# fdaPDE/fdaPDE-core

Hardware: AMD Instinct MI355X
Metric: DOF/s assemble+solve, 3D P1 Laplacian; SpMV achieved HBM GB/s vs peak (higher is better)
Workload: dtype f64

## Files before the change

fdapde-core_amd/capi.py:

```python
from __future__ import annotations

import ctypes as C
import os

import numpy as np

_HERE = os.path.dirname(os.path.abspath(__file__))
LIB_PATH = os.environ.get("FDAPDE_HIP_LIB") or os.path.join(_HERE, "lib", "libfdapde_hip.so")

OK, EINVAL, ENOMEM, ENODEVICE, EHIP, ENOTINIT, ENOCONV, EUNSUPPORTED, ERCCL = range(9)
LAPLACIAN, DIFFUSION, ADVECTION, REACTION, DT = range(5)
SOLVER_AUTO, SOLVER_CG, SOLVER_BICGSTAB, SOLVER_CG_SR, SOLVER_CG_FUSED, SOLVER_GMRES, SOLVER_DENSE, SOLVER_PMG, SOLVER_AMG = range(9)
ASSEMBLY_ROWS, ASSEMBLY_ATOMIC, ASSEMBLY_COLOURED, ASSEMBLY_PARTITIONED, ASSEMBLY_WAVE = range(5)
MAT_STIFF, MAT_MASS = 0, 1


class Term(C.Structure):
    _fields_ = [("kind", C.c_int32), ("space_varying", C.c_int32), ("coef", C.c_double), ("cst", C.c_double * 9),
                ("data", C.POINTER(C.c_double))]


class Options(C.Structure):
    _fields_ = [("method", C.c_int32), ("maxit", C.c_int32), ("rtol", C.c_double), ("assembly", C.c_int32),
                ("check_every", C.c_int32), ("time_spmv", C.c_int32)]


class Info(C.Structure):
    _fields_ = [("iters", C.c_int32), ("converged", C.c_int32), ("relres", C.c_double), ("t_assemble_ms", C.c_double),
                ("t_solve_ms", C.c_double), ("t_setup_ms", C.c_double), ("spmv_avg_ms", C.c_double), ("spmv_timed", C.c_int32),
                ("method_used", C.c_int32), ("persistent", C.c_int32), ("gather_avg_ms", C.c_double), ("update_avg_ms", C.c_double),
                ("spmv_mean_ms", C.c_double), ("launch_ms", C.c_double)]


SYMBOLS = [
    "fdapde_abi_version", "fdapde_device_count", "fdapde_ctx_create", "fdapde_ctx_destroy", "fdapde_last_error",
    "fdapde_status_string", "fdapde_mesh_upload", "fdapde_dofs_build", "fdapde_dofs_get", "fdapde_dofs_set_boundary", "fdapde_sizes",
    "fdapde_pattern_get", "fdapde_quadrature_nodes", "fdapde_set_operator", "fdapde_set_forcing", "fdapde_set_dirichlet",
    "fdapde_init", "fdapde_assemble_operator", "fdapde_solver_prepare", "fdapde_solve", "fdapde_matrix_values", "fdapde_lump", "fdapde_force", "fdapde_solution",
    "fdapde_info_get", "fdapde_spmv", "fdapde_bench_spmv", "fdapde_tune", "fdapde_stream", "fdapde_synchronize",
    "fdapde_comm_unique_id", "fdapde_comm_init", "fdapde_halo_setup", "fdapde_solve_parabolic",
    "fdapde_lin_compute", "fdapde_lin_solve", "fdapde_eval_pointwise", "fdapde_cell_integrals", "fdapde_comm_init_callback", "fdapde_comm_set_exchange_callback", "fdapde_halo_setup_peers",
    "fdapde_solver_layout", "fdapde_topology_build", "fdapde_topology_get", "fdapde_comm_allreduce", "fdapde_comm_library", "fdapde_solver_layout_kind", "fdapde_solver_layout_partition", "fdapde_rowdist_setup", "fdapde_ctx_clone", "fdapde_comm_count",
    "fdapde_ctx_create_multi", "fdapde_ctx_devices", "fdapde_partition_build", "fdapde_partition_sizes", "fdapde_partition_get", "fdapde_partition_whole",
    "fdapde_partition_peers",
]
PARTITION_ROWDIST, PARTITION_ELEMENTS = 0, 1

_lib = None


def load() -> C.CDLL:
    global _lib
    if _lib is None:
        if not os.path.exists(LIB_PATH):
            raise ImportError(f"{LIB_PATH} is missing: build it with __graft_entry__.build() or `make -C fdapde-core_amd/csrc`. "
                              "There is no CPU fallback.")
        lib = C.CDLL(LIB_PATH)
        lib.fdapde_last_error.restype = C.c_char_p
        lib.fdapde_status_string.restype = C.c_char_p
        lib.fdapde_stream.restype = C.c_void_p
        lib.fdapde_comm_library.restype = C.c_char_p
        lib.fdapde_ctx_destroy.restype = None
        _lib = lib
    return _lib


class FdapdeError(RuntimeError):
    def __init__(self, status, msg):
        super().__init__(f"[status {status}] {msg}")
        self.status = status


def _dp(a):
    return a.ctypes.data_as(C.POINTER(C.c_double))


def _ip(a):
    return a.ctypes.data_as(C.POINTER(C.c_int32))


def _bp(a):
    return a.ctypes.data_as(C.POINTER(C.c_uint8))


class Operator:

    def __init__(self, terms=None):
        self.terms = list(terms or [])

    def __neg__(self):
        return Operator([(k, -c, cst, d) for (k, c, cst, d) in self.terms])

    def __add__(self, o):
        return Operator(self.terms + o.terms)

    def __sub__(self, o):
        return Operator(self.terms + (-o).terms)

    def __rmul__(self, s):
        return Operator([(k, float(s) * c, cst, d) for (k, c, cst, d) in self.terms])

    @property
    def is_symmetric(self):
        return all(k != ADVECTION for (k, _, _, _) in self.terms)

    def c_terms(self):
        arr = (Term * len(self.terms))()
        keep = []
        for t, (k, c, cst, d) in zip(arr, self.terms):
            t.kind, t.coef, t.space_varying = k, c, 0 if d is None else 1
            if cst is not None:
                for i, v in enumerate(np.asarray(cst, dtype=float).reshape(-1)):
                    t.cst[i] = v
            if d is not None:
                dd = np.ascontiguousarray(d, dtype=float)
                keep.append(dd)
                t.data = _dp(dd)
        return arr, keep


def laplacian():
    return Operator([(LAPLACIAN, 1.0, None, None)])


def diffusion(K):
# ... 249 lines not shown
        flat = np.ascontiguousarray(locs.T).reshape(-1)
        cells = np.zeros(nl, dtype=np.int32)
        vals = np.zeros((nl, s["n_basis"]))
        self._check(self.lib.fdapde_eval_pointwise(self._ctx, C.c_int64(nl), _dp(flat), _ip(cells), _dp(vals)))
        dofs, _, _ = self.dofs_get()
        ok = cells >= 0
        rows = np.repeat(np.nonzero(ok)[0], s["n_basis"])
        cols = dofs[cells[ok]].reshape(-1)
        psi = sp.csr_matrix((vals[ok].reshape(-1), (rows, cols)), shape=(nl, s["n_dofs"]))
        return psi, np.ones(nl), cells

    def eval_areal(self, incidence):
        import scipy.sparse as sp

        inc = sp.csr_matrix(np.asarray(incidence) == 1, dtype=float)
        s = self.sizes()
        meas = np.zeros(self.n_cells)
        pint = np.zeros((self.n_cells, s["n_basis"]))
        self._check(self.lib.fdapde_cell_integrals(self._ctx, _dp(meas), _dp(pint)))
        dofs, _, _ = self.dofs_get()
        D = inc @ meas
        nb = s["n_basis"]
        cellmat = sp.csr_matrix((pint.reshape(-1), (np.repeat(np.arange(self.n_cells), nb), dofs.reshape(-1))),
                                shape=(self.n_cells, s["n_dofs"]))
        psi = sp.diags(1.0 / D) @ (inc @ cellmat)
        return psi.tocsr(), D

    def info(self):
        info = Info()
        self._check(self.lib.fdapde_info_get(self._ctx, C.byref(info)))
        return info

    def matrix_values(self, which=MAT_STIFF):
        out = np.zeros(self.sizes()["nnz"])
        self._check(self.lib.fdapde_matrix_values(self._ctx, which, _dp(out)))
        return out

    def lump(self, which=MAT_MASS):
        out = np.zeros(self.sizes()["n_dofs"])
        self._check(self.lib.fdapde_lump(self._ctx, which, _dp(out)))
        return out

    def force(self, ncols=None):
        have = getattr(self, "_force_cols", 1)
        if ncols is None:
            ncols = have
        if ncols < have:
            raise ValueError(f"force(): the context holds {have} forcing columns, a buffer for {ncols} was asked for")
        out = np.zeros(self.sizes()["n_dofs"] * ncols)
        self._check(self.lib.fdapde_force(self._ctx, _dp(out)))
        return out

    def solution(self):
        out = np.zeros(self.sizes()["n_dofs"])
        self._check(self.lib.fdapde_solution(self._ctx, _dp(out)))
        return out

    def spmv(self, which, x):
        x = np.ascontiguousarray(x, dtype=float)
        y = np.zeros_like(x)
        self._check(self.lib.fdapde_spmv(self._ctx, which, _dp(x), _dp(y)))
        return y

    def bench_spmv(self, reps=50):
        ms, by = C.c_double(), C.c_double()
        self._check(self.lib.fdapde_bench_spmv(self._ctx, reps, C.byref(ms), C.byref(by)))
        return ms.value, by.value

    def solver_layout(self, with_dirichlet=True):
        ni, nz, by = C.c_int64(), C.c_int64(), C.c_double()
        self._check(self.lib.fdapde_solver_layout(self._ctx, 1 if with_dirichlet else 0, C.byref(ni), C.byref(nz), C.byref(by)))
        return ni.value, nz.value, by.value

    def solver_layout_kind(self, with_dirichlet=True):
        k, sy, g, r = C.c_int32(), C.c_int32(), C.c_int32(), C.c_int32()
        self._check(self.lib.fdapde_solver_layout_kind(self._ctx, 1 if with_dirichlet else 0, C.byref(k), C.byref(sy), C.byref(g), C.byref(r)))
        return dict(kind=k.value, sym=sy.value, workgroups=g.value, rows_per_thread=r.value)

    def solver_layout_partition(self, with_dirichlet=True):
        p = C.c_int32()
        self._check(self.lib.fdapde_solver_layout_partition(self._ctx, 1 if with_dirichlet else 0, C.byref(p)))
        return p.value

    @staticmethod
    def comm_unique_id() -> bytes:
        buf = C.create_string_buffer(128)
        rc = load().fdapde_comm_unique_id(buf)
        if rc != OK:
            raise FdapdeError(rc, "fdapde_comm_unique_id failed (RCCL not loadable?)")
        return buf.raw

    def comm_init(self, world, rank, unique_id: bytes):
        self._check(self.lib.fdapde_comm_init(self._ctx, int(world), int(rank), C.c_char_p(unique_id)))

    def rowdist_setup(self, dof_key, dof_owner):
        k = np.ascontiguousarray(dof_key, dtype=np.int64)
        o = np.ascontiguousarray(dof_owner, dtype=np.int32)
        self._check(self.lib.fdapde_rowdist_setup(self._ctx, k.ctypes.data_as(C.POINTER(C.c_int64)), _ip(o)))

    def comm_allreduce(self, values, op="sum"):
        a = np.ascontiguousarray(np.asarray(values, dtype=float)).copy()
        self._check(self.lib.fdapde_comm_allreduce(self._ctx, _dp(a), int(a.size), 0 if op == "sum" else 1))
        return a

    def comm_count(self):
        n = C.c_int32(0)
        self._check(self.lib.fdapde_comm_count(self._ctx, C.byref(n)))
        return int(n.value)

    @staticmethod
    def comm_library():
        return (load().fdapde_comm_library() or b"").decode()

    def comm_init_callback(self, world, rank, allreduce):
        proto = C.CFUNCTYPE(C.c_int, C.c_void_p, C.POINTER(C.c_double), C.c_int64)

        def _cb(user, ptr, count):
            try:
                allreduce(np.ctypeslib.as_array(ptr, shape=(count,)))
                return 0
            except Exception:
                return 1

        self._ar_cb = proto(_cb)
        self._check(self.lib.fdapde_comm_init_callback(self._ctx, int(world), int(rank), self._ar_cb, None))

    def halo_setup(self, n_if_global, local_dof, if_index, owned):
        local_dof = np.ascontiguousarray(local_dof, dtype=np.int32)
        if_index = np.ascontiguousarray(if_index, dtype=np.int32)
        owned = np.ascontiguousarray(owned, dtype=np.uint8)
        self._check(self.lib.fdapde_halo_setup(self._ctx, C.c_int64(int(n_if_global)), C.c_int64(local_dof.size), _ip(local_dof),
                                               _ip(if_index), _bp(owned)))

    def comm_set_exchange_callback(self, exchange):
        proto = C.CFUNCTYPE(C.c_int, C.c_void_p, C.c_int32, C.POINTER(C.c_int32), C.POINTER(C.c_int64), C.POINTER(C.c_double), C.POINTER(C.c_double))

        def _cb(user, n_peers, ranks, offs, send, recv):
            try:
                off = np.ctypeslib.as_array(offs, shape=(n_peers + 1,))
                n = int(off[-1])
                exchange(np.ctypeslib.as_array(ranks, shape=(n_peers,)), off, np.ctypeslib.as_array(send, shape=(n,)),
                         np.ctypeslib.as_array(recv, shape=(n,)))
                return 0
            except Exception:
                return 1

        self._xchg_cb = proto(_cb)
        self._check(self.lib.fdapde_comm_set_exchange_callback(self._ctx, self._xchg_cb, None))

    def halo_setup_peers(self, peer_rank, peer_off, peer_dof, owned):
        peer_rank = np.ascontiguousarray(peer_rank, dtype=np.int32)
        peer_off = np.ascontiguousarray(peer_off, dtype=np.int64)
        peer_dof = np.ascontiguousarray(peer_dof, dtype=np.int32)
        owned = np.ascontiguousarray(owned, dtype=np.uint8)
        self._check(self.lib.fdapde_halo_setup_peers(self._ctx, C.c_int32(peer_rank.size), _ip(peer_rank),
                                                     peer_off.ctypes.data_as(C.POINTER(C.c_int64)), _ip(peer_dof), _bp(owned)))

    def tune(self, key, value):
        self._check(self.lib.fdapde_tune(self._ctx, key.encode(), int(value)))

    def stream(self):
        return self.lib.fdapde_stream(self._ctx)

    def synchronize(self):
        self._check(self.lib.fdapde_synchronize(self._ctx))
```

fdapde-core_amd/csrc/capi.hip:

```cpp
#include <algorithm>
#include <chrono>
#include <cmath>
#include <cstdio>
#include <cstdlib>
#include <cstring>
#include <new>

#include <dlfcn.h>
#include <hip/hip_ext.h>
#include <rccl/rccl.h>

#include "context.h"
#include "engine.h"

using namespace fdapde_engine;

extern "C" {

int fdapde_abi_version(void) { return FDAPDE_ABI_VERSION; }

int fdapde_device_count(void) {
    int n = 0;
    if (hipGetDeviceCount(&n) != hipSuccess) return 0;
    return n;
// ... 1 lines not shown

const char* fdapde_status_string(int s) {
    switch (s) {
    case FDAPDE_OK: return "ok";
    case FDAPDE_EINVAL: return "invalid argument";
    case FDAPDE_ENOMEM: return "out of memory";
    case FDAPDE_ENODEVICE: return "no HIP device";
    case FDAPDE_EHIP: return "HIP runtime error";
    case FDAPDE_ENOTINIT: return "solver must be initialized first!";
    case FDAPDE_ENOCONV: return "Krylov solve did not converge";
    case FDAPDE_EUNSUPPORTED: return "unsupported configuration";
    case FDAPDE_ERCCL: return "RCCL error";
    }
    return "unknown status";
}

int fdapde_ctx_create(int device, fdapde_ctx** out) {
    if (!out) return FDAPDE_EINVAL;
    *out = nullptr;
    fdapde_ctx* c = new (std::nothrow) fdapde_ctx();
    if (!c) return FDAPDE_ENOMEM;
    if (device >= 0) {
        int n = 0;
        if (hipGetDeviceCount(&n) != hipSuccess || device >= n) {
            delete c;
            return FDAPDE_ENODEVICE;
        }
        if (hipSetDevice(device) != hipSuccess || hipStreamCreateWithFlags(&c->stream, hipStreamNonBlocking) != hipSuccess ||
            hipEventCreate(&c->ev0) != hipSuccess || hipEventCreate(&c->ev1) != hipSuccess ||
            hipEventCreate(&c->ev_p0) != hipSuccess || hipEventCreate(&c->ev_p1) != hipSuccess ||
            hipHostMalloc(reinterpret_cast<void**>(&c->h_ctl), 8 * sizeof(int32_t)) != hipSuccess ||
            hipHostMalloc(reinterpret_cast<void**>(&c->h_sc), 16 * sizeof(double)) != hipSuccess) {
            delete c;
            return FDAPDE_EHIP;
        }
        c->device = device, c->has_device = true;
        preload_assembly(), preload_solve(), preload_dist(), preload_persist();
        preload_setup_async(device);
        if (hipDeviceGetAttribute(&c->n_cu, hipDeviceAttributeMultiprocessorCount, device) != hipSuccess) c->n_cu = 0;
    }
    *out = c;
    return FDAPDE_OK;
}

void fdapde_ctx_destroy(fdapde_ctx* c) {
    if (!c) return;
    if (c->group) fdapde_engine::g_destroy(c);
    fdapde_engine::pmg_release(c);
    fdapde_engine::amg_release(c);
    if (c->has_device) {
        (void)hipSetDevice(c->device);
        fdapde_engine::partition_free(c);
        (void)hipSetDevice(c->device);
        (void)hipStreamSynchronize(c->stream);
        drop_graph(c);
        for (DBuf<int32_t>* b : {&c->cverts, &c->cdofs, &c->adj, &c->rowptr, &c->colidx, &c->diag, &c->slot_i2e, &c->dof_i2e,
                                 &c->dof_e2i, &c->cell_i2e, &c->rb_row, &c->colour_cells, &c->ctl, &c->rowptr_e, &c->colidx_e, &c->dofs_e})
            b->release();
        for (DBuf<double>* b : {&c->vcoords, &c->vals[0], &c->vals[1], &c->force, &c->fq, &c->g, &c->sval, &c->scale, &c->gt,
                                &c->x, &c->r, &c->p, &c->y, &c->s, &c->t, &c->r0, &c->u, &c->part_a, &c->part_b, &c->sc,
                                &c->tmp_e, &c->tmp_i, &c->tmp_v, &c->lin_rhs, &c->cols_b, &c->cols_r, &c->cols_x, &c->cols_sc, &c->cols_part})
            b->release();
        c->cols_ctl.release(), c->eval_grid.release(), c->eval_locs.release(), c->eval_vals.release(), c->eval_out.release();
        for (auto& b : c->coef) b.release();
        c->slotw.release(), c->sl_off.release(), c->lane_row.release(), c->fq_blk.release(), c->bnd.release(), c->tables.release(), c->reftab.release(), c->reftab_sym.release(), c->lin_sq.release();
        c->bc_off.release(), c->bn_off.release(), c->bc_cell.release(), c->bn_node.release(), c->bc_vert.release();
        c->halo_dof.release(), c->halo_pos.release(), c->owned.release(), c->hbuf.release(), c->sbuf.release();
        c->halo_inv.release(), c->if_slot.release();
        c->peer_send_dof.release(), c->peer_src_off.release(), c->peer_src.release(), c->peer_sendbuf.release(), c->peer_recvbuf.release();
        c->xd.remote[0].release(), c->xd.remote[1].release(), c->xd.slots.release(), c->xd.slot_ptr.release();
        release_rowdist(c);
        if (c->comm) (void)g_rccl.CommDestroy(c->comm);
        c->mesh_nodes.release(), c->mesh_cells.release(), c->mesh_nbnd.release();
        c->gm_V.release(), c->gm_b.release(), c->gm_s.release(), c->gm_part.release();
        c->lin_dense.X.release(), c->step_dense.X.release(), c->solve_dense.X.release(), c->dn_b.release(), c->dn_x.release(), c->dn_r.release(), c->dn_cnt.release();
        c->lin_mat.release(), c->stiff_stat.release(), c->ar_dev.release(), c->persist_stats.release(), c->persist_x.release(), c->persist_xs.release(), c->coords_e.release();
        dev_topology_release(&c->topo);
        c->part_cells.release(), c->part_off.release(), c->part_slots.release(), c->wave_slots.release(), c->part_shared.release();
        for (auto& bk : c->bk)
            bk.slot_dof.release(), bk.sl_off.release(), bk.ell_src.release(), bk.imp_off.release(), bk.imp_dof.release(), bk.drop_dof.release(), bk.ell_off.release(),
              bk.ell_code.release(), bk.ell_val.release();
        for (auto& ps : c->ps)
            ps.slot_dof.release(), ps.sl_off.release(), ps.ell_src.release(), ps.exp_off.release(), ps.imp_off.release(),
              ps.imp_pos.release(), ps.ell_off.release(), ps.ell_code.release(), ps.exp_slot.release(), ps.ell_val.release(), ps.board.release(), ps.board_cols.release(), ps.amax.release(), ps.wg_late.release(), ps.ell_col.release();
        for (int v = 0; v < 2; ++v)
            c->sp_rowptr[v].release(), c->sp_colidx[v].release(), c->sp_map[v].release(), c->sp_tbase[v].release(), c->sp_col16[v].release(),
              c->sp_vrow[v].release();
        if (c->h_io) (void)hipHostFree(c->h_io);
        if (c->h_ctl) (void)hipHostFree(c->h_ctl);
        if (c->h_sc) (void)hipHostFree(c->h_sc);
        (void)hipEventDestroy(c->ev0), (void)hipEventDestroy(c->ev1), (void)hipEventDestroy(c->ev_p0), (void)hipEventDestroy(c->ev_p1);
        for (hipEvent_t e : c->ev_spmv) (void)hipEventDestroy(e);
        (void)hipStreamDestroy(c->stream);
    }
    delete c->lin_state;
    delete c;
}

int fdapde_ctx_clone(const fdapde_ctx* src, fdapde_ctx** out) {
    if (!src || !out) return FDAPDE_EINVAL;
    *out = nullptr;
    if (src->group) return fdapde_engine::g_clone(src, out);
    fdapde_ctx* c = nullptr;
    if (int rc = fdapde_ctx_create(src->has_device ? src->device : -1, &c)) return rc;
    const int rc = fdapde_engine::e_ctx_clone(src, c);
    if (rc != FDAPDE_OK) {
        const_cast<fdapde_ctx*>(src)->err = "fdapde_ctx_clone: " + c->err;
        fdapde_ctx_destroy(c);
        return rc;
    }
    *out = c;
    return FDAPDE_OK;
}

const char* fdapde_last_error(const fdapde_ctx* c) { return c ? c->err.c_str() : "null context"; }

int fdapde_mesh_upload(fdapde_ctx* c, int M, int N, int64_t n_nodes, const double* nodes, int64_t n_cells,
                       const int32_t* cells, const uint8_t* bnd) {
    if (!c) return FDAPDE_EINVAL;
    if (c->group && M == 2 && N == 3)
        return fail(c, FDAPDE_EUNSUPPORTED, "fdapde_mesh_upload: a surface mesh (Triangulation<2,3>) takes a one-GPU context; the multi-device partitioner "
                                            "and its ranks are built for planar and volume meshes");
    if (c->group && M == 1)
        return fail(c, FDAPDE_EUNSUPPORTED, "fdapde_mesh_upload: a 1-D mesh (interval or linear network, Triangulation<1,N>) takes a one-GPU context; the "
                                            "multi-device partitioner and its ranks are built for planar and volume meshes");
    c->space_ready = c->dev_ready = c->colour_ready = c->fq_blk_ready = c->fq_bc_ready = c->stiff_stat_valid = false;
    c->assembled[0] = c->assembled[1] = c->force_ready = c->solved = c->dirichlet_applied = false;
    c->op.clear(), c->coef_of_op = false, c->fq_i.clear(), c->fq_cols = 0, c->g_i.clear(), c->have_g = false;
    if (c->topo_ready) dev_topology_release(&c->topo), c->topo_ready = false;
    c->mesh_on_dev = false;
    if (int rc = host_set_mesh(c->hs, M, N, n_nodes, nodes, n_cells, cells, bnd, c->err)) return rc;
    if (c->has_device) {
        const HostSpace& hs = c->hs;
        if (hipSetDevice(c->device) != hipSuccess || c->mesh_nodes.upload(hs.nodes.data(), hs.nodes.size(), c->stream) != hipSuccess ||
            c->mesh_cells.upload(hs.cells.data(), hs.cells.size(), c->stream) != hipSuccess ||
            c->mesh_nbnd.upload(hs.node_bnd.data(), hs.node_bnd.size(), c->stream) != hipSuccess || hipStreamSynchronize(c->stream) != hipSuccess) {
            c->mesh_nodes.release(), c->mesh_cells.release(), c->mesh_nbnd.release();
            c->err = "fdapde_mesh_upload: copying the mesh to the device failed";
            return FDAPDE_EHIP;
        }
        c->mesh_on_dev = true;
    }
    fdapde_engine::partition_free(c);
    if (c->group) fdapde_engine::g_mesh_changed(c);
    return FDAPDE_OK;
}

int fdapde_sizes(const fdapde_ctx* c, int64_t* n_dofs, int64_t* nnz, int32_t* n_basis, int32_t* n_quadrature, int64_t* n_edges) {
    if (!c || !c->space_ready) return FDAPDE_ENOTINIT;
    if (n_dofs) *n_dofs = c->hs.n_dofs;
    if (nnz) *nnz = c->hs.nnz;
    if (n_basis) *n_basis = c->hs.nb;
    if (n_quadrature) *n_quadrature = c->hs.nq;
    if (n_edges) *n_edges = c->hs.n_edges;
    return FDAPDE_OK;
}

int fdapde_dofs_build(fdapde_ctx* c, int order, int64_t* n_dofs) {
    if (!c) return FDAPDE_EINVAL;
    if (c->group) return fdapde_engine::g_dofs_build(c, order, n_dofs);
    return fdapde_engine::e_dofs_build(c, order, n_dofs);
}
int fdapde_topology_build(fdapde_ctx* c, int64_t* n_facets, int64_t* n_edges) {
    if (!c) return FDAPDE_EINVAL;
    return fdapde_engine::e_topology_build(c, n_facets, n_edges);
}
int fdapde_topology_get(fdapde_ctx* c, int32_t* neighbors, int32_t* cell_facets, int32_t* facet_nodes, int32_t* facet_cells, uint8_t* facet_boundary, int32_t* edge_nodes, uint8_t* edge_boundary, int32_t* face_edges) {
    if (!c) return FDAPDE_EINVAL;
    return fdapde_engine::e_topology_get(c, neighbors, cell_facets, facet_nodes, facet_cells, facet_boundary, edge_nodes, edge_boundary, face_edges);
}
int fdapde_dofs_set_boundary(fdapde_ctx* c, const uint8_t* bnd) {
    if (!c) return FDAPDE_EINVAL;
    if (c->group) return fdapde_engine::g_dofs_set_boundary(c, bnd);
    return fdapde_engine::e_dofs_set_boundary(c, bnd);
}
int fdapde_dofs_get(const fdapde_ctx* c, int32_t* dofs, uint8_t* bnd, double* coords) {
    if (!c) return FDAPDE_EINVAL;
    return fdapde_engine::e_dofs_get(c, dofs, bnd, coords);
}
int fdapde_pattern_get(const fdapde_ctx* c, int32_t* rowptr, int32_t* colidx) {
    if (!c) return FDAPDE_EINVAL;
    return fdapde_engine::e_pattern_get(c, rowptr, colidx);
}
int fdapde_quadrature_nodes(fdapde_ctx* c, double* out) {
    if (!c) return FDAPDE_EINVAL;
    return fdapde_engine::e_quadrature_nodes(c, out);
}
int fdapde_set_operator(fdapde_ctx* c, int32_t n_terms, const fdapde_term* terms) {
    if (!c) return FDAPDE_EINVAL;
    if (c->group) return fdapde_engine::g_set_operator(c, n_terms, terms);
    return fdapde_engine::e_set_operator(c, n_terms, terms);
}
int fdapde_set_forcing(fdapde_ctx* c, const double* f_q, int32_t n_cols) {
    if (!c) return FDAPDE_EINVAL;
    if (c->group) return fdapde_engine::g_set_forcing(c, f_q, n_cols);
    return fdapde_engine::e_set_forcing(c, f_q, n_cols);
}
int fdapde_set_dirichlet(fdapde_ctx* c, const double* g) {
    if (!c) return FDAPDE_EINVAL;
    if (c->group) return fdapde_engine::g_set_dirichlet(c, g);
    return fdapde_engine::e_set_dirichlet(c, g);
}
int fdapde_assemble_operator(fdapde_ctx* c, int32_t which, int32_t n_terms, const fdapde_term* terms, int32_t assembly) {
    if (!c) return FDAPDE_EINVAL;
    if (c->group) return fdapde_engine::g_assemble_operator(c, which, n_terms, terms, assembly);
    return fdapde_engine::e_assemble_operator(c, which, n_terms, terms, assembly);
}
int fdapde_init(fdapde_ctx* c, const fdapde_options* opt) {
    if (!c) return FDAPDE_EINVAL;
    if (c->group) return fdapde_engine::g_init(c, opt);
    return fdapde_engine::e_init(c, opt);
}
int fdapde_eval_pointwise(fdapde_ctx* c, int64_t n_locs, const double* locs_colmajor, int32_t* cell_ids, double* values) {
    if (!c) return FDAPDE_EINVAL;
    return fdapde_engine::e_eval_pointwise(c, n_locs, locs_colmajor, cell_ids, values);
}
int fdapde_cell_integrals(fdapde_ctx* c, double* measure, double* psi_int) {
    if (!c) return FDAPDE_EINVAL;
    return fdapde_engine::e_cell_integrals(c, measure, psi_int);
}
int fdapde_solver_prepare(fdapde_ctx* c, int32_t with_dirichlet) {
    if (!c) return FDAPDE_EINVAL;
    if (c->group) return fdapde_engine::g_solver_prepare(c, with_dirichlet);
    return fdapde_engine::e_solver_prepare(c, with_dirichlet);
}
int fdapde_solver_layout(fdapde_ctx* c, int32_t with_dirichlet, int64_t* n_interior, int64_t* nnz_interior, double* streamed_bytes) {
    if (!c) return FDAPDE_EINVAL;
    if (c->group) return fdapde_engine::g_layout_kind(c, with_dirichlet, nullptr, nullptr, nullptr, nullptr);
    return fdapde_engine::e_solver_layout(c, with_dirichlet, n_interior, nnz_interior, streamed_bytes);
}
int fdapde_solver_layout_kind(fdapde_ctx* c, int32_t with_dirichlet, int32_t* kind, int32_t* symmetric_storage, int32_t* workgroups, int32_t* rows_per_thread) {
    if (!c) return FDAPDE_EINVAL;
    if (c->group) return fdapde_engine::g_layout_kind(c, with_dirichlet, kind, symmetric_storage, workgroups, rows_per_thread);
    return fdapde_engine::e_solver_layout_kind(c, with_dirichlet, kind, symmetric_storage, workgroups, rows_per_thread);
}
int fdapde_solver_layout_partition(fdapde_ctx* c, int32_t with_dirichlet, int32_t* partition) {
    int32_t kind = 0;
    if (int rc = fdapde_solver_layout_kind(c, with_dirichlet, &kind, nullptr, nullptr, nullptr)) return rc;
    const fdapde_ctx::Persist& ps = c->ps[with_dirichlet ? 1 : 0];
    if (partition) *partition = (kind == 2 || kind == 3) && ps.ok ? (ps.meta.bisect ? 1 : 0) : -1;
    return FDAPDE_OK;
}
int fdapde_solve(fdapde_ctx* c, const fdapde_options* opt, fdapde_info* info) {
    if (!c) return FDAPDE_EINVAL;
    if (c->group && opt && opt->method == FDAPDE_SOLVER_AMG) return fdapde_engine::fail(c, FDAPDE_EUNSUPPORTED, "FDAPDE_SOLVER_AMG takes one-GPU contexts, not a multi-device context");
    if (c->group) return fdapde_engine::g_solve(c, opt, info);
    return fdapde_engine::e_solve(c, opt, info);
}
int fdapde_solve_parabolic(fdapde_ctx* c, const fdapde_options* opt, int32_t n_times, double delta_t, const double* initial_condition, const double* dirichlet, double* solution, fdapde_info* info) {
    if (!c) return FDAPDE_EINVAL;
    if (c->group && opt && opt->method == FDAPDE_SOLVER_AMG) return fdapde_engine::fail(c, FDAPDE_EUNSUPPORTED, "FDAPDE_SOLVER_AMG takes one-GPU contexts, not a multi-device context");
    if (c->group) return fdapde_engine::g_solve_parabolic(c, opt, n_times, delta_t, initial_condition, dirichlet, solution, info);
    return fdapde_engine::e_solve_parabolic(c, opt, n_times, delta_t, initial_condition, dirichlet, solution, info);
}
int fdapde_lin_compute(fdapde_ctx* c, int32_t which, const double* values, int32_t symmetric) {
    if (!c) return FDAPDE_EINVAL;
    if (c->group) return fdapde_engine::g_lin_compute(c, which, values, symmetric);
    return fdapde_engine::e_lin_compute(c, which, values, symmetric);
}
int fdapde_lin_solve(fdapde_ctx* c, const fdapde_options* opt, const double* b, int32_t n_rhs, double* x, fdapde_info* info) {
    if (!c) return FDAPDE_EINVAL;
    if (c->group && opt && opt->method == FDAPDE_SOLVER_AMG) return fdapde_engine::fail(c, FDAPDE_EUNSUPPORTED, "FDAPDE_SOLVER_AMG takes one-GPU contexts, not a multi-device context");
    if (c->group) return fdapde_engine::g_lin_solve(c, opt, b, n_rhs, x, info);
    return fdapde_engine::e_lin_solve(c, opt, b, n_rhs, x, info);
}
int fdapde_matrix_values(fdapde_ctx* c, int32_t which, double* values) {
    if (!c) return FDAPDE_EINVAL;
    if (c->group) return fdapde_engine::g_matrix_values(c, which, values);
    return fdapde_engine::e_matrix_values(c, which, values);
}
int fdapde_lump(fdapde_ctx* c, int32_t which, double* diag) {
    if (!c) return FDAPDE_EINVAL;
    if (c->group) return fdapde_engine::g_lump(c, which, diag);
    return fdapde_engine::e_lump(c, which, diag);
}
int fdapde_force(fdapde_ctx* c, double* force) {
    if (!c) return FDAPDE_EINVAL;
    if (c->group) return fdapde_engine::g_force(c, force);
    return fdapde_engine::e_force(c, force);
}
int fdapde_solution(fdapde_ctx* c, double* solution) {
    if (!c) return FDAPDE_EINVAL;
    if (c->group) return fdapde_engine::g_solution(c, solution);
    return fdapde_engine::e_solution(c, solution);
}
int fdapde_spmv(fdapde_ctx* c, int32_t which, const double* x, double* y) {
    if (!c) return FDAPDE_EINVAL;
    if (c->group) return fdapde_engine::g_spmv(c, which, x, y);
    return fdapde_engine::e_spmv(c, which, x, y);
}
int fdapde_bench_spmv(fdapde_ctx* c, int32_t reps, double* avg_ms, double* algorithmic_bytes) {
    if (!c) return FDAPDE_EINVAL;
    if (c->group) return fail(c, FDAPDE_EUNSUPPORTED, "fdapde_bench_spmv: a multi-device context wires its own ranks");
    return fdapde_engine::e_bench_spmv(c, reps, avg_ms, algorithmic_bytes);
}
int fdapde_comm_unique_id(void* out128) {
    return fdapde_engine::e_comm_unique_id(out128);
}
int fdapde_comm_init(fdapde_ctx* c, int32_t world, int32_t rank, const void* unique_id128) {
    if (!c) return FDAPDE_EINVAL;
    if (c->group) return fail(c, FDAPDE_EUNSUPPORTED, "fdapde_comm_init: a multi-device context wires its own ranks");
    return fdapde_engine::e_comm_init(c, world, rank, unique_id128);
}
int fdapde_comm_allreduce(fdapde_ctx* c, double* host_inout, int32_t n, int32_t op) {
    if (!c) return FDAPDE_EINVAL;
    if (c->group) return fail(c, FDAPDE_EUNSUPPORTED, "fdapde_comm_allreduce: a multi-device context wires its own ranks");
    return fdapde_engine::e_comm_allreduce(c, host_inout, n, op);
}
int fdapde_comm_count(fdapde_ctx* c, int32_t* ranks) {
    if (!c) return FDAPDE_EINVAL;
    return fdapde_engine::e_comm_count(c, ranks);
}
int fdapde_comm_init_callback(fdapde_ctx* c, int32_t world, int32_t rank, fdapde_allreduce_fn fn, void* user) {
    if (!c) return FDAPDE_EINVAL;
    if (c->group) return fail(c, FDAPDE_EUNSUPPORTED, "fdapde_comm_init_callback: a multi-device context wires its own ranks");
    return fdapde_engine::e_comm_init_callback(c, world, rank, fn, user);
}
// ... 61 lines not shown
    if (c->group) return fdapde_engine::g_tune(c, key, value);
    const std::string k(key);
    drop_graph(c);
    if (k == "spmv_variant" && value >= 0 && value <= 2) c->spmv_variant = value;
    else if (k == "spmv_team" && (value == 2 || value == 4 || value == 8 || value == 16 || value == 32 || value == 64)) {
        if (value != c->spmv_team) c->sp_built[0] = c->sp_built[1] = false, c->sp_cur = -1, c->solved = false, c->scaled_owner = fdapde_ctx::kScaledNone;
        c->spmv_team = value;
    }
    else if (k == "spmv_unroll" && value >= 1 && value <= 8) c->spmv_unroll = value;
    else if (k == "spmv_ablate") c->spmv_ablate = value;
    else if (k == "spmv_c16" && (value == 0 || value == 1)) c->spmv_c16 = value;
    else if (k == "spmv_deep" && (value == 0 || value == 1)) c->spmv_deep = value;
    else if (k == "cgf_split" && (value == 0 || value == 1)) c->cgf_split = value;
    else if (k == "cgf_v" && (value == 1 || value == 2 || value == 4 || value == 8)) c->cgf_v = value;
    else if (k == "use_graph" && (value == 0 || value == 1)) c->use_graph = value;
    else if (k == "cgf_band" && (value == 0 || value == 1)) c->cgf_band = value;
    else if (k == "cgf_nt" && value >= 0 && value <= 15) c->cgf_nt = value;
    else if (k == "cgf_lazy" && (value == 0 || value == 1)) c->cgf_lazy = value;
    else if (k == "multi_rhs" && (value == 0 || value == 1)) c->multi_rhs = value;
    else if (k == "asm_fq_block" && (value == 0 || value == 1)) c->asm_fq_block = value;
    else if (k == "asm_fuse_mass" && value >= 0 && value <= 3) c->asm_fuse_mass = value;
    else if (k == "asm_items" && (value == 0 || value == 1)) c->asm_items = value;
    else if (k == "asm_items_fuse" && (value == 0 || value == 1)) c->asm_items_fuse = value;
    else if (k == "bicg_restart" && (value == 0 || value == 1)) c->bicg_restart = value;
    else if (k == "bicg_shadow" && value >= 0 && value <= 2) c->bicg_shadow = value;
    else if (k == "gmres_m" && value >= 2 && value <= 200) c->gmres_m = value;
    else if (k == "persist_exp_lds" && (value == 0 || value == 1)) {
        c->persist_exp_lds = value;
        c->ps[0].tried = c->ps[0].ok = c->ps[1].tried = c->ps[1].ok = false, c->scaled_owner = fdapde_ctx::kScaledNone;
        fdapde_engine::drop_graph(c);
    }
    else if (k == "dense_rows" && value >= 0 && value <= 8192) c->dense_rows = value, c->lin_dense.ready = false, c->lin_dense.failed = false;
    else if (k == "dense_after" && value >= 0) c->dense_after = value;
    else if (k == "dense_block" && (value == 0 || value == 1)) c->dense_block = value;
    else if (k == "dense_direct" && (value == 0 || value == 1)) c->dense_direct = value;
    else if (k == "dense_fold" && (value == 0 || value == 1)) c->dense_fold = value;
    else if (k == "dense_multi" && (value == 0 || value == 1)) c->dense_multi = value;
    else if (k == "pmg_inner_tol_exp" && value >= 1 && value <= 12) c->pmg_inner_rtol = std::pow(10.0, -(double)value);
    else if (k == "pmg_inner_maxit" && value >= 1) c->pmg_inner_maxit = value;
    else if (k == "pmg_auto" && (value == 0 || value == 1)) c->pmg_auto = value;
    else if (k == "pmg_blocked" && (value == 0 || value == 1)) c->pmg_blocked = value;
    else if (k == "pmg_smooth" && (value == 0 || value == 1)) c->pmg_smooth = value;
    else if (k == "pmg_setup_check" && (value == 0 || value == 1)) c->pmg_setup_check = value;
    else if (k == "amg_coarse_rows" && value >= 1 && value <= 8192) c->amg_coarse_rows = value;
    else if (k == "amg_setup_check" && (value == 0 || value == 1)) c->amg_setup_check = value;
    else if (k == "pmg_restart" && value >= 2 && value <= 50) c->pmg_restart = (int)value;
    else if (k == "pmg_outer" && (value == 0 || value == 1)) c->pmg_outer = value;
    else if (k == "pmg_auto_rows" && value >= 0) c->pmg_auto_rows = value;
    else if (k == "pmg_auto_first_rows" && value >= 0) c->pmg_auto_first_rows = value;
    else if (k == "dense_bulk" && (value == 0 || value == 1)) c->dense_bulk = value;
    else if (k == "dense_hostb" && (value == 0 || value == 1)) c->dense_hostb = value;
    else if (k == "small_rows" && value >= 0) c->small_rows = value;
    else if (k == "small_front_rows" && value >= 0) c->small_front_rows = value;
    else if (k == "auto_gmres" && (value == 0 || value == 1)) c->auto_gmres = value;
    else if (k == "asm_split_varying" && (value == 0 || value == 1)) c->asm_split_varying = value;
    else if (k == "asm_row_stat" && (value == 0 || value == 1)) c->asm_row_stat = value, c->stiff_stat_valid = false;
    else if (k == "asm_fq_bc" && (value == 0 || value == 1)) c->asm_fq_bc = value, c->fq_bc_ready = c->fq_bc_ready && value;
    else if (k == "persist" && (value == 0 || value == 1)) c->persist = value, c->persist_broken = false;
    else if (k == "persist_time" && (value == 0 || value == 1)) c->persist_time = value;
    else if (k == "persist_coop" && (value == 0 || value == 1)) c->persist_coop = value;
    else if (k == "persist_bicg" && (value == 0 || value == 1)) c->persist_bicg = value;
    else if (k == "persist_fill_fused" && (value == 0 || value == 1)) c->persist_fill_fused = value;
    else if (k == "persist_prefetch" && (value == 0 || value == 1)) c->persist_prefetch = value;
    else if (k == "persist_cols" && (value == 0 || value == 1)) c->persist_cols = value;
    else if (k == "persist_direct" && (value == 0 || value == 1)) c->persist_direct = value;
    else if (k == "persist_wide_gj" && (value == 4 || value == 6 || value == 12)) {
        c->persist_wide_gj = value;
        for (auto& ps : c->ps) ps.attr_set = nullptr;
    }
    else if ((k == "persist_wide" && (value == 0 || value == 1)) || (k == "persist_max_wg" && value >= 0)) {
        if (k == "persist_wide") c->persist_wide = value;
        else c->persist_max_wg = value;
        for (auto& ps : c->ps) ps.tried = ps.ok = ps.filled = false;
    }
    else if (k == "persist_direct_spin_us" && value >= 0 && value <= 1000000) c->persist_direct_spin_us = value;
    else if (k == "persist_single_rows" && value >= 0 && value <= 8192) {
        c->persist_single_rows = value;
        for (auto& ps : c->ps) ps.tried = ps.ok = ps.filled = false;
    }
    else if (k == "persist_partition" && value >= 0 && value <= 2) {
        c->persist_partition = value;
        for (auto& ps : c->ps) ps.tried = ps.ok = ps.filled = false;
    }
    else if (k == "persist_late" && (value == 0 || value == 1)) {
        c->persist_late = value;
        for (auto& ps : c->ps) ps.tried = ps.ok = ps.filled = false;
    }
    else if (k == "rowdist_max_wg" && value >= 0) {
        c->rd.max_wg = value;
        for (auto& L : c->rd.lay) L.tried = L.ok = false;
    } else if (k == "rowdist_share" && value >= 1) {
        c->rd.max_wg = std::max(1, c->n_cu / value);
        for (auto& L : c->rd.lay) L.tried = L.ok = false;
    } else if (k == "rowdist_timeout_first_ms" && value >= 1) c->rd.timeout_first_ms = value;
    else if (k == "rowdist_flat_gather" && value >= -1 && value <= 1) c->rd.flat_gather = value;
    else if (k == "persist_timeout_us" && value >= 100 && value <= 10000000) c->persist_timeout_us = value;
    else if (k == "persist_debug_stall" && value >= 0) c->persist_debug_stall = value;
    else if (k == "persist_retry" && value == 1) c->persist_broken = false, c->persist_retry_in = 0, c->persist_backoff = 8;
    else if (k == "blocked" && value >= 0 && value <= 2) c->blocked = value;
    else if (k == "persist_gather_waves" && (value == 1 || value == 4)) c->persist_gather_waves = value;
    else if (k == "persist_poll_sleep" && value >= 0 && value <= 3) c->persist_poll_sleep = value;
    else if (k == "persist_balance" && (value == 0 || value == 1)) {
        c->persist_balance = value;
        for (auto& ps : c->ps) ps.tried = ps.ok = ps.filled = false;
    } else if (k == "persist_sym" && value >= 0 && value <= 2) {
        c->persist_sym = value;
        for (auto& ps : c->ps) ps.tried = ps.ok = ps.filled = false;
    }
    else if (k == "spmv_ntv" && value >= -1 && value <= 1) c->spmv_ntv = value;
    else if (k == "spmv_bpx" && value >= 1 && value <= 1024) {
        c->spmv_grid = 8 * value;
        HIPCHK(c, hipSetDevice(c->device));
        HIPCHK(c, hipStreamSynchronize(c->stream));
        HIPCHK(c, c->part_a.alloc(2 * (size_t)c->spmv_grid));
    } else return fail(c, FDAPDE_EINVAL, "unknown tuning key or value out of range");
    return FDAPDE_OK;
}

void* fdapde_stream(fdapde_ctx* c) { return c ? (void*)c->stream : nullptr; }

int fdapde_synchronize(fdapde_ctx* c) {
    if (!c) return FDAPDE_EINVAL;
    if (int rc = need_device(c)) return rc;
    if (c->group)
        if (int rc = fdapde_engine::g_synchronize(c)) return rc;
    HIPCHK(c, hipSetDevice(c->device));
    HIPCHK(c, hipStreamSynchronize(c->stream));
    HIPCHK(c, hipDeviceSynchronize());
    return FDAPDE_OK;
}

}
```

fdapde-core_amd/csrc/context.h:

```cpp
#ifndef FDAPDE_CONTEXT_H
#define FDAPDE_CONTEXT_H

#include <cstdint>
#include <memory>
#include <functional>
#include <string>
#include <vector>

#include <dlfcn.h>
#include <hip/hip_ext.h>
#include <hip/hip_runtime.h>
#include <rccl/rccl.h>

#include "../../include/fdapde_hip.h"
#include "dev_persist.h"
#include "dev_setup.h"
#include "dev_topology.h"
#include "internal.h"

namespace fdapde_engine {
struct Group;
struct AmgHierarchy;
}
namespace fdapde_hip {
// ... 85 lines not shown
        GetUniqueId = reinterpret_cast<decltype(GetUniqueId)>(dlsym(handle, "ncclGetUniqueId"));
        CommInitRank = reinterpret_cast<decltype(CommInitRank)>(dlsym(handle, "ncclCommInitRank"));
        CommDestroy = reinterpret_cast<decltype(CommDestroy)>(dlsym(handle, "ncclCommDestroy"));
        CommCount = reinterpret_cast<decltype(CommCount)>(dlsym(handle, "ncclCommCount"));
        AllReduce = reinterpret_cast<decltype(AllReduce)>(dlsym(handle, "ncclAllReduce"));
        GetErrorString = reinterpret_cast<decltype(GetErrorString)>(dlsym(handle, "ncclGetErrorString"));
        Send = reinterpret_cast<decltype(Send)>(dlsym(handle, "ncclSend"));
        Recv = reinterpret_cast<decltype(Recv)>(dlsym(handle, "ncclRecv"));
        GroupStart = reinterpret_cast<decltype(GroupStart)>(dlsym(handle, "ncclGroupStart"));
        GroupEnd = reinterpret_cast<decltype(GroupEnd)>(dlsym(handle, "ncclGroupEnd"));
        if (!GetUniqueId || !CommInitRank || !CommDestroy || !AllReduce || !GetErrorString || !Send || !Recv || !GroupStart || !GroupEnd) {
            err = "librccl lacks a required symbol";
            return false;
        }
        return true;
    }
};
inline RcclApi g_rccl;

struct HostTerm {
    fdapde_term t;
    std::vector<double> data_i;
    std::shared_ptr<DBuf<double>> data_dev;
    bool field_nonsym = false;
};

}
using namespace fdapde_detail;

constexpr int64_t kNtValsRows = 2000000;
constexpr int kTimeStride = 8, kTimePhase = 3;

struct GraphKey {
    const void* sval;
    const void* rowptr;
    int64_t n;
    double tol2;
    int chunk, v, grid, team, ablate, c16, deep, unroll, sp_cur, bk_cur, bk_G;
    const void* bk_val;
};

struct SolveState {
    bool dist = false, diag_positive = true;
    bool symmetric = true;
    bool rowdist = false;
    const uint8_t* owned = nullptr;
    int use_bnd = 0;
    bool diag_deferred = false;
    mutable bool front_pending = false;
    const double* front_A = nullptr;
};
struct SolveStateHolder {
    SolveState ss;
};

struct fdapde_ctx {
    int device = -1;
    bool has_device = false;
    hipStream_t stream = nullptr;
    hipEvent_t ev0 = nullptr, ev1 = nullptr, ev_p0 = nullptr, ev_p1 = nullptr;
    std::vector<hipEvent_t> ev_spmv;
    std::string err;
    HostSpace hs;
    BasisTables tb;
    bool space_ready = false, dev_ready = false, colour_ready = false;
    bool assembled[2] = {false, false};
    bool force_ready = false, solved = false, dirichlet_applied = false;
    std::vector<HostTerm> op;
    bool op_symmetric = true;
    std::vector<double> fq_i;
    int fq_cols = 0;
    std::vector<double> g_i;
    bool have_g = false, g_zero = false;
    fdapde_info info{};
    DBuf<int32_t> cverts, cdofs, adj, rowptr, colidx, diag, slot_i2e, dof_i2e, dof_e2i, cell_i2e, rb_row, colour_cells;
    DBuf<int32_t> rowptr_e, colidx_e;
    DBuf<int32_t> dofs_e;
    DBuf<double> coords_e;
    DBuf<double> mesh_nodes;
    DBuf<int32_t> mesh_cells;
    DBuf<uint8_t> mesh_nbnd;
    bool mesh_on_dev = false;
    DBuf<double> gm_V, gm_b, gm_s, gm_part;
    int persist_exp_lds = 1;
    int gmres_m = 50;
    int auto_gmres = 1;
    bool dev_built = false;
    DBuf<uint32_t> slotw;
    DBuf<int64_t> bc_off, bn_off;
    DBuf<int32_t> bc_cell, bn_node;
    DBuf<uint16_t> bc_vert;
    DBuf<int64_t> sl_off;
    DBuf<int32_t> lane_row;
    DBuf<double> stiff_stat;
    bool stiff_stat_valid = false, asm_all_in_lds = false;
    int asm_row_stat = 1;
    DBuf<double> fq_blk;
    bool fq_blk_ready = false;
    DBuf<double> fq_bc;
    bool fq_bc_ready = false;
    bool cg_broke_down = false;
    int bicg_shadow = 0;
    int bicg_restart = 1;
    int asm_split_varying = 1;
    int asm_items = 1;
    int32_t asm_max_visits = -1;
    int asm_fuse_mass = 1;
    int asm_items_fuse = 1;
    int asm_fq_bc = 1;
    int asm_fq_block = 0;
    DBuf<double> vcoords, vals[2], force, fq, g, sval, scale, gt, x, r, p, y, s, t, r0, u, part_a, part_b, sc, tmp_e,
      tmp_i, tmp_v, restart_u, lin_rhs;
    DBuf<uint8_t> bnd;
    DBuf<DevTables> tables;
    DBuf<DevRefTensors> reftab;
    DBuf<DevRefTensorsSym> reftab_sym;
    DBuf<int32_t> ctl;
    DBuf<double> coef[kMaxTerms];
    bool coef_of_op = false;
    double* h_io = nullptr;
    size_t h_io_cap = 0;
    int persist_direct = 1;
    int persist_direct_spin_us = 2000;
    int32_t* h_ctl = nullptr;
    double* h_sc = nullptr;
    int spmv_grid = 0, rb_per_band = 0, vec_grid = 0, n_rb = 0, cg_grid = 0;
    int spmv_variant = 2;
    int spmv_team = 16, spmv_unroll = 4, spmv_ablate = 0;
    int lds_limit = 96 * 1024;
    DBuf<int32_t> sp_rowptr[2], sp_colidx[2], sp_map[2], sp_tbase[2], sp_vrow[2];
    int64_t sp_nv[2] = {0, 0};
    int sval_layout = -2;
    DBuf<uint16_t> sp_col16[2];
    int64_t sp_wide[2] = {0, 0};
    int spmv_ntv = -1;
    int sp_team = 0;
    int spmv_c16 = 1;
    int use_graph = 0;
    hipGraphExec_t cg_graph_exec = nullptr;
    GraphKey cg_graph_key{};
    int cgf_lazy = 1;
    int cgf_nt = 7;
    int cgf_band = 1;
    int cgf_split = 0;
    int cgf_v = 8;
    int spmv_deep = 0;
    int64_t sp_nnz[2] = {0, 0};
    bool sp_built[2] = {false, false};
    int sp_cur = -1;
    bool sval_stale = false;
    const double* sval_A = nullptr;
    int persist_fill_fused = 0;
    enum { kScaledNone = 0, kScaledSolve, kScaledParabolic, kScaledLin, kScaledPmg };
    int scaled_owner = kScaledNone;
    ncclComm_t comm = nullptr;
    fdapde_allreduce_fn ar_fn = nullptr;
    void* ar_user = nullptr;
    std::vector<double> ar_host;
    DBuf<double> ar_dev;
    int world = 1, rank = 0;
    bool halo_ready = false;
    int64_t n_if = 0, n_loc_if = 0;
    DBuf<int32_t> halo_dof, halo_pos;
    DBuf<int32_t> halo_inv, if_slot;
    DBuf<uint8_t> owned;
    DBuf<double> hbuf, sbuf;
    bool peer_mode = false;
    fdapde_exchange_fn xchg_fn = nullptr;
    void* xchg_user = nullptr;
    std::vector<int32_t> peer_rank;
    std::vector<int64_t> peer_off;
    DBuf<int32_t> peer_send_dof;
    DBuf<int32_t> peer_src_off, peer_src;
    DBuf<double> peer_sendbuf, peer_recvbuf;
    std::vector<double> xchg_send_h, xchg_recv_h;
    struct PeerDirect {
        bool on = false;
        int (*arrive)(void*) = nullptr;
        void* user = nullptr;
        int parity = 0, ar_parity = 0;
        int64_t n_send = 0;
        DBuf<const double*> remote[2];
        DBuf<double> slots;
        DBuf<const double*> slot_ptr;
    } xd;
    static constexpr int kSlotDoubles = 64;
    DBuf<double> lin_mat;
    bool lin_ready = false, lin_symmetric = false;
    DBuf<double> lin_sq;
    bool lin_sq_ready = false;
    int multi_rhs = 1;
    SolveStateHolder* lin_state = nullptr;
    int n_cu = 0;
    int persist = 1;
    int persist_time = 1;
    int persist_balance = 1;
    int persist_sym = 2;
    int persist_gather_waves = 4, persist_poll_sleep = 2;
    bool persist_broken = false;
    int persist_retry_in = 0, persist_backoff = 8;
    struct Persist {
        bool tried = false, ok = false;
        PersistLayout meta;
        int32_t lds_cap = 0, imp_cap = 0;
        size_t lds_bytes = 0;
        DBuf<int32_t> slot_dof, sl_off, ell_src, exp_off, imp_off, imp_pos;
        DBuf<int32_t> ell_col;
        bool stream = false;
        bool exp_lds = false;
        DBuf<int64_t> ell_off;
        DBuf<uint16_t> ell_code, exp_slot;
        DBuf<double> ell_val;
        DBuf<unsigned long long> amax;
        DBuf<uint8_t> wg_late;
        DBuf<unsigned long long> board;
        DBuf<unsigned long long> board_cols;
        int per_cu = 0;
        bool filled = false;
        uint32_t epoch_next = 0;
        const void* attr_set = nullptr;
        bool built_plain = false;
    } ps[2];
    struct RowDist {
        bool ready = false;
        std::vector<int32_t> owner_i;
        std::vector<int64_t> key_i;
        DBuf<uint8_t> owned;
        int max_wg = 0;
        int flat_gather = -1;
        int timeout_first_ms = 2000;
        struct Layout {
            bool tried = false, ok = false;
            Persist ps;
            int32_t n_ghost = 0, G_tot = 0, g_base = 0;
            DBuf<int32_t> rexp_off, rexp_peer, rexp_pos;
            DBuf<uint16_t> rexp_slot;
            DBuf<uint8_t> wg_late;
            DBuf<unsigned long long> rboard;
            DBuf<unsigned long long*> peer_pboard, peer_dboard;
            std::vector<void*> ipc_opened;
            std::vector<int32_t> x_rank;
            std::vector<int64_t> x_soff, x_roff;
            DBuf<int32_t> x_send_dof, x_recv_dof;
            DBuf<double> x_sendbuf, x_recvbuf;
        } lay[2];
    } rd;
    DBuf<double> persist_stats;
    DBuf<double> persist_x;
    DBuf<double> persist_xs;
    int persist_wide_gj = 12;
    int persist_wide = 1;
    int persist_max_wg = 0;
    double persist_launch_ms = 0;
    int persist_host_below = 32768;
    int persist_cols = 1;
    DBuf<double> cols_b, cols_r, cols_x, cols_sc, cols_part;
    DBuf<int32_t> cols_ctl;
    struct EvalGrid {
        bool ready = false;
        DBuf<int32_t> ptr, cells, dims;
        DBuf<double> lo, invh;
        void release() { ptr.release(), cells.release(), dims.release(), lo.release(), invh.release(), ready = false; }
    } eval_grid;
    DBuf<double> eval_locs, eval_vals;
    DBuf<int32_t> eval_out;
    std::function<int()> persist_tail;
    int h_ctl_seen = 4;
    bool ev1_at_end = false;
    int64_t small_rows = 8192;
    int64_t small_front_rows = 2048;
    bool front_used = false;
    bool tail_in_launch = false;
    bool defer_end_sync = false;
    int persist_single_rows = 2048;
    int persist_prefetch = 1;
    int persist_partition = 2;
    int persist_late = 0;
    int persist_plain = 0;
    int persist_bicg = 1;
    int persist_coop = 0;
    int persist_timeout_us = 5000;
    int persist_debug_stall = 0;
    struct Blocked {
        bool tried = false, ok = false, filled = false;
        PersistLayout meta;
        int32_t imp_cap = 0;
        size_t lds_bytes = 0;
        DBuf<int32_t> slot_dof, sl_off, ell_src, imp_off, imp_dof, drop_dof;
        DBuf<int64_t> ell_off;
        DBuf<uint16_t> ell_code;
        DBuf<double> ell_val;
    } bk[2];
    int bk_cur = -1;
    int blocked = 1;
    DevTopology topo;
    bool topo_ready = false;
// ... 78 lines not shown
```

fdapde-core_amd/csrc/eng_solve.hip:

```cpp
#include <algorithm>
#include <chrono>
#include <cmath>
#include <cstdio>
#include <cstdlib>
#include <cstring>
#include <new>

#include <dlfcn.h>
#include <hip/hip_ext.h>
#include <rccl/rccl.h>

#include "context.h"
#include "engine.h"
#include "kernels.h"

namespace fdapde_engine {

constexpr int64_t kBlockedShortRowsAbove = 3200000;

void drop_graph(fdapde_ctx* c) {
    if (c->cg_graph_exec) (void)hipGraphExecDestroy(c->cg_graph_exec);
    c->cg_graph_exec = nullptr;
}

// ... 794 lines not shown
    int rc = solve_run(c, ss, A, f_dev, g_dev, u0_dev, method, rtol, maxit, check_every, n_timed);
    int total = c->info.iters;
    const bool may_restart = method == FDAPDE_SOLVER_BICGSTAB || method == FDAPDE_SOLVER_AUTO;
    for (int k = 0; k < kBicgRestarts && may_restart && rc == FDAPDE_ENOCONV && c->h_ctl[2] != 0 && c->info.method_used == FDAPDE_SOLVER_BICGSTAB &&
                    total < maxit && std::isfinite(c->info.relres) && c->info.relres < 1e3 && c->bicg_restart;
         ++k) {
        if (ss.rowdist)
            if (int rc2 = rowdist_import_ghosts(c, ss.use_bnd ? 1 : 0, c->u.p)) return rc2;
        HIPCHK(c, c->restart_u.alloc((size_t)n));
        HIPCHK(c, hipMemcpyAsync(c->restart_u.p, c->u.p, sizeof(double) * (size_t)n, hipMemcpyDeviceToDevice, c->stream));
        rc = solve_run(c, ss, A, f_dev, g_dev, c->restart_u.p, FDAPDE_SOLVER_BICGSTAB, rtol, maxit - total, check_every, 0);
        total += c->info.iters;
    }
    c->info.iters = total;
    if (gmres_budget >= 0 && (gmres_budget > 0 || maxit - total > 0) && rc == FDAPDE_ENOCONV && c->info.method_used == FDAPDE_SOLVER_BICGSTAB && !ss.dist && !ss.rowdist &&
        dense_eligible(c)) {
        bool solved = false;
        if (int rc2 = dense_direct(c, A, ss.use_bnd, f_dev, g_dev, &solved)) return rc2;
        if (solved) {
            c->info.method_used = FDAPDE_SOLVER_DENSE, c->info.converged = 1, c->info.relres = c->solve_dense.check, c->info.persistent = 0;
            c->h_ctl[0] = 1, c->h_ctl[2] = 0;
            c->err.clear();
            if (c->ev1_at_end) HIPCHK(c, hipEventRecord(c->ev1, c->stream));
            return FDAPDE_OK;
        }
    }
    const int gm_maxit = gmres_budget > 0 ? gmres_budget : maxit - total;
    if (gmres_budget >= 0 && gm_maxit > 0 && c->auto_gmres && rc == FDAPDE_ENOCONV && c->info.method_used == FDAPDE_SOLVER_BICGSTAB && !ss.dist && !ss.rowdist) {
        const bool warm = std::isfinite(c->info.relres) && c->info.relres < 1.0;
        if (warm) {
            HIPCHK(c, c->restart_u.alloc((size_t)n));
            HIPCHK(c, hipMemcpyAsync(c->restart_u.p, c->u.p, sizeof(double) * (size_t)n, hipMemcpyDeviceToDevice, c->stream));
        }
        rc = solve_run(c, ss, A, f_dev, g_dev, warm ? c->restart_u.p : u0_dev, FDAPDE_SOLVER_GMRES, rtol, gm_maxit, check_every, 0);
        c->info.iters += total;
    }
    return rc;
}

int e_solver_prepare(fdapde_ctx* c, int32_t with_dirichlet) {
    if (!c) return FDAPDE_EINVAL;
    if (int rc = need_device(c)) return rc;
    if (!c->dev_ready) return fail(c, FDAPDE_ENOTINIT, "call fdapde_dofs_build first");
    HIPCHK(c, hipSetDevice(c->device));
    if (c->spmv_variant != 2) return FDAPDE_OK;
    const int v = with_dirichlet ? 1 : 0;
    if (c->persist && !c->persist_broken && c->comm == nullptr && c->ar_fn == nullptr && (c->op_symmetric || c->persist_bicg)) {
        c->persist_plain = c->op_symmetric ? 0 : 1;
        if (int rc = build_persist(c, v)) return rc;
        if (c->ps[v].ok && (c->op_symmetric || (!c->ps[v].meta.sym && c->ps[v].meta.R <= 8))) return FDAPDE_OK;
    }
    if (c->blocked && c->comm == nullptr && c->ar_fn == nullptr &&
        ((double)c->hs.nnz >= 20.0 * (double)c->hs.n_dofs || c->blocked == 2 || c->hs.n_dofs > kBlockedShortRowsAbove)) {
        if (int rc = build_blocked(c, v)) return rc;
        if (c->bk[v].ok) return FDAPDE_OK;
    }
    return build_solver_pattern(c, v);
}

int e_solver_layout(fdapde_ctx* c, int32_t with_dirichlet, int64_t* n_interior, int64_t* nnz_interior, double* streamed_bytes) {
    if (!c) return FDAPDE_EINVAL;
    if (int rc = need_device(c)) return rc;
    if (!c->dev_ready) return fail(c, FDAPDE_ENOTINIT, "call fdapde_dofs_build first");
    HIPCHK(c, hipSetDevice(c->device));
    const int v = with_dirichlet ? 1 : 0;
    const bool persist = c->persist && !c->persist_broken && c->ps[v].tried && c->ps[v].ok;
    const bool blocked = !persist && c->bk[v].tried && c->bk[v].ok;
    if (c->spmv_variant == 2 && !persist && !blocked)
        if (int rc = build_solver_pattern(c, v)) return rc;
    if (int rc = ensure_host(c, kHostPattern)) return rc;
    const HostSpace& hs = c->hs;
    int64_t ni = 0, nz = 0;
    for (int64_t i = 0; i < hs.n_dofs; ++i) {
        if (v && hs.dof_bnd_i[(size_t)i]) continue;
        ++ni;
        for (int32_t k = hs.rowptr_i[(size_t)i]; k < hs.rowptr_i[(size_t)i + 1]; ++k)
            if (!(v && hs.dof_bnd_i[(size_t)hs.colidx_i[(size_t)k]])) ++nz;
    }
    if (n_interior) *n_interior = ni;
    if (nnz_interior) *nnz_interior = nz;
    if (streamed_bytes) {
        if (persist) {
            *streamed_bytes = 10.0 * (double)c->ps[v].meta.n_entries + 32.0 * (double)c->ps[v].meta.n_board +
                              (c->ps[v].meta.R > kPersistRmax ? 16.0 * (double)c->ps[v].meta.n_int : 0.0);
        } else if (blocked) {
            *streamed_bytes = 10.0 * (double)c->bk[v].meta.n_entries + 8.0 * (double)(c->bk[v].meta.n_int + c->bk[v].meta.n_imp) + 8.0 * (double)c->bk[v].meta.n_int;
        } else if (c->spmv_variant == 2 && c->sp_built[v]) {
            const int64_t n_csr = c->sp_nv[v] > 0 ? c->sp_nv[v] : hs.n_dofs;
            *streamed_bytes = 10.0 * (double)c->sp_nnz[v] + 4.0 * (double)(n_csr + 1) + 16.0 * (double)((n_csr + kCodeRows - 1) / kCodeRows) +
                              (c->sp_nv[v] > 0 ? 8.0 * (double)n_csr : 0.0) + 16.0 * (double)hs.n_dofs +
                              4.0 * (double)c->sp_wide[v] * kCodeRows * ((double)c->sp_nnz[v] / (double)(n_csr > 0 ? n_csr : 1));
        } else
            *streamed_bytes = 12.0 * (double)hs.nnz + 4.0 * (double)(hs.n_dofs + 1) + 16.0 * (double)hs.n_dofs;
    }
    return FDAPDE_OK;
}

int e_solver_layout_kind(fdapde_ctx* c, int32_t with_dirichlet, int32_t* kind, int32_t* symmetric_storage, int32_t* workgroups,
                              int32_t* rows_per_thread) {
    if (!c) return FDAPDE_EINVAL;
    if (!c->dev_ready) return fail(c, FDAPDE_ENOTINIT, "call fdapde_dofs_build first");
    const int v = with_dirichlet ? 1 : 0;
    const bool persist = c->persist && !c->persist_broken && c->ps[v].tried && c->ps[v].ok;
    const bool blocked = !persist && c->bk[v].tried && c->bk[v].ok;
    if (kind) *kind = persist ? (c->ps[v].stream ? 2 : 3) : blocked ? 1 : 0;
    if (symmetric_storage) *symmetric_storage = persist && c->ps[v].meta.sym ? 1 : 0;
    if (workgroups) *workgroups = persist ? c->ps[v].meta.G : blocked ? c->bk[v].meta.G : 0;
    if (rows_per_thread) *rows_per_thread = persist ? c->ps[v].meta.R : blocked ? c->bk[v].meta.R : 0;
    return FDAPDE_OK;
}

int e_solve(fdapde_ctx* c, const fdapde_options* opt, fdapde_info* info) {
    if (!c) return FDAPDE_EINVAL;
    if (int rc = need_device(c)) return rc;
    if (!c->dev_ready || !c->assembled[0] || !c->force_ready)
        return fail(c, FDAPDE_ENOTINIT, "solver must be initialized first!");
    HIPCHK(c, hipSetDevice(c->device));
    const int64_t n = c->hs.n_dofs;
    const double rtol = (opt && opt->rtol > 0) ? opt->rtol : 1e-10;
    const int maxit = (opt && opt->maxit > 0) ? opt->maxit : default_maxit(c, n);
    const int check_every = (opt && opt->check_every > 0) ? opt->check_every : 32;
    const double* A = c->vals[FDAPDE_MAT_STIFF].p;
    HIPCHK(c, hipEventRecord(c->ev0, c->stream));
    if (opt && opt->method == FDAPDE_SOLVER_PMG) return e_solve_pmg(c, opt, info);
    if (opt && opt->method == FDAPDE_SOLVER_AMG) return e_solve_amg(c, opt, info);
    if (opt && opt->method == FDAPDE_SOLVER_DENSE) {
        if (!dense_eligible(c))
            return fail(c, FDAPDE_EUNSUPPORTED, "FDAPDE_SOLVER_DENSE takes one-GPU systems of up to `dense_rows` (at most 8192) DOFs");
        bool solved = false;
        c->scaled_owner = fdapde_ctx::kScaledNone;
        if (int rc = dense_direct(c, A, c->have_g ? 1 : 0, c->force.p, c->g.p, &solved)) return rc;
        HIPCHK(c, hipEventRecord(c->ev1, c->stream));
        HIPCHK(c, hipEventSynchronize(c->ev1));
        float ms = 0;
        HIPCHK(c, hipEventElapsedTime(&ms, c->ev0, c->ev1));
        const double t_asm = c->info.t_assemble_ms;
        c->info = fdapde_info{};
        c->info.t_assemble_ms = t_asm;
        c->info.method_used = FDAPDE_SOLVER_DENSE, c->info.converged = solved ? 1 : 0, c->info.relres = c->solve_dense.check, c->info.t_solve_ms = ms;
        c->solved = solved, c->dirichlet_applied = c->have_g;
        if (info) *info = c->info;
        if (!solved) {
            c->err = "FDAPDE_SOLVER_DENSE: the matrix is singular to working precision (no usable pivot, or max |I - A X| beyond 1e-6)";
            return FDAPDE_ENOCONV;
        }
        return FDAPDE_OK;
    }
    if ((!opt || opt->method == FDAPDE_SOLVER_AUTO) && c->pmg_auto && n >= c->pmg_auto_rows &&
        (n >= c->pmg_auto_first_rows || c->pmg.ready || c->open_solves >= 1) && pmg_eligible(c)) {
        fdapde_options po{};
        po.method = FDAPDE_SOLVER_PMG, po.rtol = rtol, po.maxit = (opt && opt->maxit > 0) ? std::min(opt->maxit, 60) : 60;
        const int rc = e_solve_pmg(c, &po, info);
        if (rc == FDAPDE_OK) {
            ++c->open_solves;
            return rc;
        }
        if (rc != FDAPDE_ENOCONV && rc != FDAPDE_EUNSUPPORTED) return rc;
        c->err.clear();
        HIPCHK(c, hipEventRecord(c->ev0, c->stream));
    }
    SolveState ss;
    c->scaled_owner = fdapde_ctx::kScaledSolve;
    DebugClock clk;
    const bool open_method = !opt || opt->method == FDAPDE_SOLVER_AUTO;
    const bool skip_cg = open_method && c->cg_broke_down;
    const int gm_budget = !open_method ? -1 : ((opt && opt->maxit > 0) ? 0 : default_maxit(c, n));
    if (int rc = solve_prepare(c, A, c->have_g ? 1 : 0, &ss, c->op_symmetric && !skip_cg, true)) return rc;
// ... 436 lines not shown
    struct KrylovClock {
        fdapde_ctx* c;
        std::chrono::steady_clock::time_point t0 = std::chrono::steady_clock::now();
        ~KrylovClock() { c->lin_krylov_ms += std::chrono::duration<double, std::milli>(std::chrono::steady_clock::now() - t0).count(); }
    } krylov_clock{c};
    if (c->scaled_owner != fdapde_ctx::kScaledLin) {
        c->scaled_owner = fdapde_ctx::kScaledNone;
        if (int rc = solve_prepare(c, c->lin_mat.p, 0, &c->lin_state->ss, c->lin_symmetric)) return rc;
        c->scaled_owner = fdapde_ctx::kScaledLin;
    }
    c->solved = false;
    DBuf<double>& rhs = c->lin_rhs;
    HIPCHK(c, rhs.alloc((size_t)n));
    DebugClock clk;
    HIPCHK(c, hipEventRecord(c->ev0, st));
    int total = 0, rc_all = FDAPDE_OK;
    double worst = 0;
    int32_t j0 = 0;
    bool breakdown = false;
    auto retry_as_bicgstab = [&]() -> int {
        c->lin_symmetric = false, c->scaled_owner = fdapde_ctx::kScaledNone;
        if (int rc = solve_prepare(c, c->lin_mat.p, 0, &c->lin_state->ss, false)) return rc;
        c->scaled_owner = fdapde_ctx::kScaledLin, c->lin_sq_ready = false;
        const int spent = total;
        c->lin_cols -= n_rhs;
        const int rc = e_lin_solve(c, opt, b, n_rhs, x, info);
        c->info.iters += spent;
        if (info) info->iters = c->info.iters;
        return rc;
    };
    const bool may_retry = c->lin_symmetric && (!opt || opt->method == FDAPDE_SOLVER_AUTO) && method == FDAPDE_SOLVER_CG_FUSED &&
                           !c->lin_state->ss.dist && !c->lin_state->ss.rowdist;
    const bool persist_cols = c->persist && !c->persist_broken && c->ps[0].ok && c->ps[0].filled && c->ps[0].meta.R <= kPersistRmax;
    const bool batched = c->multi_rhs && n_rhs >= 4 && method == FDAPDE_SOLVER_CG_FUSED && !c->lin_state->ss.dist && !c->lin_state->ss.rowdist && !persist_cols;
    if (batched) {
        if (!c->lin_sq_ready) {
            HIPCHK(c, c->lin_sq.alloc((size_t)hs.nnz + 2));
            hipLaunchKernelGGL(k_scale_matrix, dim3(g1(n * 16)), dim3(256), 0, st, n, c->rowptr.p, c->colidx.p, c->lin_mat.p, c->scale.p,
                               c->lin_sq.p);
            c->lin_sq_ready = true;
        }
        while (n_rhs - j0 >= 4) {
            const int q = n_rhs - j0 >= 8 ? 8 : 4;
            int its = 0, rc = FDAPDE_OK;
            double rel = 0;
            bool ok = true;
            if (q == 8) rc = lin_solve_batch<8>(c, b + (size_t)j0 * n, x + (size_t)j0 * n, rtol, maxit, check_every, &its, &rel, &ok);
            else rc = lin_solve_batch<4>(c, b + (size_t)j0 * n, x + (size_t)j0 * n, rtol, maxit, check_every, &its, &rel, &ok);
            if (rc != FDAPDE_OK) return rc;
            if (!ok) rc_all = FDAPDE_ENOCONV, breakdown = breakdown || c->h_ctl[2] != 0;
            total += its, worst = rel > worst ? rel : worst;
            c->info.method_used = method;
            j0 += q;
        }
    }
    if (n_rhs == 1 && persist_cols && c->persist_cols && c->persist_direct && method == FDAPDE_SOLVER_CG_FUSED && !c->lin_state->ss.dist &&
        !c->lin_state->ss.rowdist && !c->lin_state->ss.use_bnd && c->ps[0].meta.G == 1) {
        bool ran = false;
        const double tol2 = rtol * rtol;
        if (int rc = run_persist_direct(c, 0, tol2, maxit, b, x, &ran)) return rc;
        if (ran) {
            const double bb = c->h_sc[0], rr = c->h_sc[3];
            c->info.iters = c->h_ctl[1], c->info.relres = bb > 0 ? sqrt(rr / bb) : 0.0;
            c->info.converged = (rr <= tol2 * bb && c->h_ctl[2] == 0) ? 1 : 0;
            c->info.method_used = method, c->info.persistent = 1, c->info.launch_ms = 0.0, c->info.t_solve_ms = 0.0;
            c->info.spmv_avg_ms = 0, c->info.spmv_timed = 0;
            if (info) *info = c->info;
            if (!c->info.converged) {
                if (c->h_ctl[2] && may_retry) {
                    total = c->info.iters;
                    return retry_as_bicgstab();
                }
                c->err = c->h_ctl[2] ? "Krylov breakdown (operator not SPD for CG)" : "maxit reached";
                return FDAPDE_ENOCONV;
            }
            return FDAPDE_OK;
        }
    }
    const bool cols_bicg = method == FDAPDE_SOLVER_BICGSTAB && c->persist_bicg && !c->ps[0].meta.sym && c->ps[0].meta.R <= 8;
    if (persist_cols && c->persist_cols && (method == FDAPDE_SOLVER_CG_FUSED || cols_bicg) && !c->lin_state->ss.dist && !c->lin_state->ss.rowdist &&
        !c->lin_state->ss.use_bnd) {
        fdapde_ctx::Persist& ps = c->ps[0];
        const int G = ps.meta.G;
        const int cap = (ps.per_cu > 0 ? ps.per_cu : 1) * c->n_cu / (G > 0 ? G : 1);
        const double tol2 = rtol * rtol;
        const int np = c->vec_grid;
        while (n_rhs - j0 >= 1 && cap >= 1) {
            const int Q = std::min(std::min<int>(n_rhs - j0, cap), 64);
            const size_t qn = (size_t)Q * (size_t)n;
            HIPCHK(c, c->cols_b.alloc(qn));
            HIPCHK(c, c->cols_r.alloc(qn));
            HIPCHK(c, c->cols_x.alloc(qn));
            HIPCHK(c, c->cols_sc.alloc(4 * (size_t)Q));
            HIPCHK(c, c->cols_ctl.alloc(4 * (size_t)Q));
            HIPCHK(c, c->cols_part.alloc(2 * (size_t)np * Q));
            HIPCHK(c, hipMemcpyAsync(c->cols_b.p, b + (size_t)j0 * n, sizeof(double) * qn, hipMemcpyHostToDevice, st));
            hipLaunchKernelGGL(k_cols_init, dim3(np, Q), dim3(256), 0, st, n, c->cols_b.p, c->dof_i2e.p, c->scale.p, c->cols_r.p, c->cols_part.p);
            hipLaunchKernelGGL(k_cols_init_fin, dim3(Q), dim3(256), 0, st, c->cols_part.p, np, c->cols_sc.p, c->cols_ctl.p);
            HIPCHK(c, hipGetLastError());
            std::vector<int32_t> h_ctl(4 * (size_t)Q);
            std::vector<double> h_sc(4 * (size_t)Q);
            bool ran = false;
            if (int rc = run_persist_cols(c, 0, tol2, maxit, Q, c->cols_r.p, c->cols_x.p, c->cols_sc.p, c->cols_ctl.p, h_ctl.data(), h_sc.data(), &ran, cols_bicg))
                return rc;
            if (!ran) break;
            if (cols_bicg && c->bicg_restart) {
                bool broke = false;
                for (int k = 0; k < Q; ++k) broke = broke || h_ctl[4 * (size_t)k + 2] != 0;
                if (broke) break;
            }
            hipLaunchKernelGGL(k_cols_finish, dim3(g1(n), Q), dim3(256), 0, st, n, c->cols_x.p, c->scale.p, c->dof_i2e.p, c->cols_b.p);
            HIPCHK(c, hipGetLastError());
            HIPCHK(c, hipMemcpyAsync(x + (size_t)j0 * n, c->cols_b.p, sizeof(double) * qn, hipMemcpyDeviceToHost, st));
            for (int k = 0; k < Q; ++k) {
                const double bb = h_sc[4 * (size_t)k], rr = h_sc[4 * (size_t)k + 3];
                const double rel = bb > 0 ? sqrt(rr / bb) : 0.0;
                if (!(rr <= tol2 * bb && h_ctl[4 * (size_t)k + 2] == 0)) rc_all = FDAPDE_ENOCONV;
                breakdown = breakdown || h_ctl[4 * (size_t)k + 2] != 0;
                total += h_ctl[4 * (size_t)k + 1], worst = rel > worst ? rel : worst;
            }
            c->info.method_used = method, c->info.persistent = 1, c->info.launch_ms = c->persist_launch_ms;
            j0 += Q;
        }
    }
    for (int32_t j = j0; j < n_rhs; ++j) {
        HIPCHK(c, hipMemcpyAsync(c->tmp_e.p, b + (size_t)j * n, sizeof(double) * (size_t)n, hipMemcpyHostToDevice, st));
        hipLaunchKernelGGL(k_gather_f64, dim3(g1(n)), dim3(256), 0, st, n, c->dof_i2e.p, c->tmp_e.p, rhs.p);
        clk.mark("lin_solve: upload + gather issued");
        c->defer_end_sync = true;
        const int rc = solve_run_restarting(c, c->lin_state->ss, c->lin_mat.p, rhs.p, c->g.p, nullptr, method, rtol, maxit, check_every, 0,
                                            !(!opt || opt->method == FDAPDE_SOLVER_AUTO) ? -1 : ((opt && opt->maxit > 0) ? 0 : default_maxit(c, n)));
        c->defer_end_sync = false;
        clk.mark("lin_solve: solve_run");
        if (rc != FDAPDE_OK && rc != FDAPDE_ENOCONV) return rc;
        if (rc == FDAPDE_ENOCONV) rc_all = rc, breakdown = breakdown || (c->h_ctl[2] != 0 && is_cg_method(c->info.method_used));
        total += c->info.iters, worst = c->info.relres > worst ? c->info.relres : worst;
        hipLaunchKernelGGL(k_scatter_f64, dim3(g1(n)), dim3(256), 0, st, n, c->dof_i2e.p, c->u.p, c->tmp_e.p);
        HIPCHK(c, hipMemcpyAsync(x + (size_t)j * n, c->tmp_e.p, sizeof(double) * (size_t)n, hipMemcpyDeviceToHost, st));
        clk.mark("lin_solve: solution download issued");
    }
    HIPCHK(c, hipEventRecord(c->ev1, st));
    HIPCHK(c, hipEventSynchronize(c->ev1));
    if (rc_all == FDAPDE_ENOCONV && breakdown && may_retry) return retry_as_bicgstab();
    float ms = 0;
    HIPCHK(c, hipEventElapsedTime(&ms, c->ev0, c->ev1));
    c->info.t_solve_ms = ms, c->info.iters = total, c->info.relres = worst, c->info.converged = rc_all == FDAPDE_OK ? 1 : 0;
    if (rc_all == FDAPDE_ENOCONV)
        c->err = breakdown ? "Krylov breakdown in at least one column (matrix not positive definite for CG, or BiCGStab rho / omega = 0)" : "maxit reached in at least one column";
    if (info) *info = c->info;
    return rc_all;
}

int e_matrix_values(fdapde_ctx* c, int32_t which, double* values) {
    if (!c || !values || which < 0 || which > 1) return FDAPDE_EINVAL;
    if (int rc = need_device(c)) return rc;
    if (!c->dev_ready || !c->assembled[which]) return fail(c, FDAPDE_ENOTINIT, "matrix not assembled");
    HIPCHK(c, hipSetDevice(c->device));
    const HostSpace& hs = c->hs;
    const int zero_rows = (which == FDAPDE_MAT_STIFF && c->dirichlet_applied) ? 1 : 0;
    hipLaunchKernelGGL(k_export_values, dim3(g1(hs.n_dofs * 16)), dim3(256), 0, c->stream, hs.n_dofs, c->rowptr.p, c->colidx.p,
                       c->vals[which].p, c->slot_i2e.p, c->bnd.p, zero_rows, c->tmp_v.p);
    HIPCHK(c, hipGetLastError());
    HIPCHK(c, hipMemcpyAsync(values, c->tmp_v.p, sizeof(double) * (size_t)hs.nnz, hipMemcpyDeviceToHost, c->stream));
    HIPCHK(c, hipStreamSynchronize(c->stream));
    return FDAPDE_OK;
}

// ... 145 lines not shown
```

fdapde-core_amd/csrc/host_persist.cpp:

```cpp
#include <algorithm>
#include <cstddef>
#include <cstdint>
#include <numeric>
#include <thread>
#include <vector>

#include "internal.h"

namespace fdapde_hip {

namespace {

template <typename F> void for_each_wg(int G, F&& fn) {
    unsigned nt = std::thread::hardware_concurrency();
    nt = nt < 1 ? 1 : (nt > 16 ? 16 : nt);
    if ((unsigned)G < nt) nt = (unsigned)G;
    if (nt <= 1) {
        for (int g = 0; g < G; ++g) fn(g);
        return;
    }
    std::vector<std::thread> th;
    for (unsigned t = 0; t < nt; ++t)
        th.emplace_back([&, t] {
            for (int g = (int)t; g < G; g += (int)nt) fn(g);
// ... 177 lines not shown
    if (ghost_order != nullptr) {
        for (int64_t d = 0; d < nd; ++d)
            if (ghost(d) && is_exp[(size_t)d]) pl.ghost_needed.push_back((int32_t)d);
        std::sort(pl.ghost_needed.begin(), pl.ghost_needed.end(), [&](int32_t a, int32_t b) { return ghost_order[(size_t)a] < ghost_order[(size_t)b]; });
        for (size_t k = 0; k < pl.ghost_needed.size(); ++k) board_of[(size_t)pl.ghost_needed[k]] = (int32_t)(pl.n_board + (int64_t)k);
    }
    pl.imp_off.assign((size_t)G + 1, 0);
    pl.max_imp = 0;
    for (int g = 0; g < G; ++g) {
        std::vector<int32_t>& imp = imports[(size_t)g];
        std::sort(imp.begin(), imp.end(), [&](int32_t a, int32_t b) { return board_of[(size_t)a] < board_of[(size_t)b]; });
        pl.imp_off[(size_t)g + 1] = pl.imp_off[(size_t)g] + (int32_t)imp.size();
        pl.max_imp = std::max(pl.max_imp, (int32_t)imp.size());
    }
    if (S + pl.max_imp > 65535) return FDAPDE_EUNSUPPORTED;
    pl.imp_pos.resize((size_t)pl.imp_off[(size_t)G]);
    pl.n_imp = pl.imp_off[(size_t)G];
    for (int g = 0; g < G; ++g)
        for (size_t h = 0; h < imports[(size_t)g].size(); ++h)
            pl.imp_pos[(size_t)pl.imp_off[(size_t)g] + h] = board_of[(size_t)imports[(size_t)g][h]];

    pl.sl_off.assign((size_t)G * (nsl + 1), 0);
    pl.ell_off.assign((size_t)G + 1, 0);
    for (int g = 0; g < G; ++g) {
        int32_t off = 0;
        for (int q = 0; q < nsl; ++q) {
            int32_t w = 0;
            for (int l = 0; l < 64; ++l) {
                const int32_t d = pl.slot_dof[(size_t)g * S + (size_t)q * 64 + l];
                if (d >= 0) w = std::max(w, row_len[(size_t)d]);
            }
            pl.sl_off[(size_t)g * (nsl + 1) + q] = off;
            off += (w + 1) / 2;
        }
        pl.sl_off[(size_t)g * (nsl + 1) + nsl] = off;
        pl.ell_off[(size_t)g + 1] = pl.ell_off[(size_t)g] + (int64_t)off * 128;
    }
    pl.n_entries = pl.ell_off[(size_t)G];
    pl.ell_code.assign((size_t)pl.n_entries, 0);
    pl.ell_src.assign((size_t)pl.n_entries, -1);
    std::vector<int64_t> nnz_wg((size_t)G, 0);
    for_each_wg(G, [&](int g) {
        const std::vector<int32_t>& imp = imports[(size_t)g];
        std::vector<int32_t> by_dof(imp.size());
        std::iota(by_dof.begin(), by_dof.end(), 0);
        std::sort(by_dof.begin(), by_dof.end(), [&](int32_t a, int32_t b) { return imp[(size_t)a] < imp[(size_t)b]; });
        auto import_index = [&](int32_t dof) {
            size_t lo = 0, hi = by_dof.size();
            while (lo < hi) {
                const size_t mid = (lo + hi) / 2;
                if (imp[(size_t)by_dof[mid]] < dof) lo = mid + 1;
                else hi = mid;
            }
            return by_dof[lo];
        };
        int64_t nz = 0;
        for (int s = 0; s < S; ++s) {
            const int32_t d = pl.slot_dof[(size_t)g * S + s];
            if (d < 0 && !sym) continue;
            const int q = s / 64, l = s % 64;
            const int64_t base = pl.ell_off[(size_t)g] + (int64_t)pl.sl_off[(size_t)g * (nsl + 1) + q] * 128 + 2 * l;
            int32_t e = 0;
            for (int32_t k = d < 0 ? 0 : hs.rowptr_i[(size_t)d]; k < (d < 0 ? 0 : hs.rowptr_i[(size_t)d + 1]); ++k) {
                const int32_t c = hs.colidx_i[(size_t)k];
                if (!kept(d, c)) continue;
                if (sym && wg_of[(size_t)c] == g && !own[(size_t)k]) continue;
                const int64_t at = base + (int64_t)(e / 2) * 128 + (e & 1);
                pl.ell_src[(size_t)at] = k;
                pl.ell_code[(size_t)at] = (uint16_t)(wg_of[(size_t)c] == g ? slot_of[(size_t)c] : S + import_index(c));
                ++e, ++nz;
            }
            if (sym) {
                const int32_t e1 = 2 * (pl.sl_off[(size_t)g * (nsl + 1) + q + 1] - pl.sl_off[(size_t)g * (nsl + 1) + q]);
                for (; e < e1; ++e) pl.ell_code[(size_t)(base + (int64_t)(e / 2) * 128 + (e & 1))] = (uint16_t)s;
            }
        }
        nnz_wg[(size_t)g] = nz;
    });
    pl.nnz = std::accumulate(nnz_wg.begin(), nnz_wg.end(), (int64_t)0);
    if (ghost_order != nullptr) pl.wg_of = std::move(wg_of), pl.slot_of = std::move(slot_of);
    return FDAPDE_OK;
}

}
```

fdapde-core_amd/csrc/internal.h:

```cpp
#ifndef FDAPDE_INTERNAL_H
#define FDAPDE_INTERNAL_H

#include <cmath>
#include <cstdint>
#include <memory>
#include <new>
#include <string>
#include <utility>
#include <vector>

#include "../../include/fdapde_hip.h"

namespace fdapde_hip {

template <class T> struct NoInitAlloc : std::allocator<T> {
    template <class U> struct rebind { using other = NoInitAlloc<U>; };
    NoInitAlloc() = default;
    template <class U> NoInitAlloc(const NoInitAlloc<U>&) noexcept {}
    template <class U> void construct(U* p) noexcept { ::new (static_cast<void*>(p)) U; }
    template <class U, class... A> void construct(U* p, A&&... a) { ::new (static_cast<void*>(p)) U(std::forward<A>(a)...); }
};
template <class T> using hvec = std::vector<T, NoInitAlloc<T>>;

constexpr int kMaxBasis = 10;
// ... 64 lines not shown
int host_build_colouring(HostSpace& hs, std::string& err);
int host_build_solver_pattern_seg(const HostSpace& hs, bool use_bnd, int seg, int wrows, std::vector<int32_t>& rowptr_v,
                                  std::vector<int32_t>& colidx_s, std::vector<int32_t>& full2s, std::vector<int32_t>& vrow);
constexpr int kCodeRows = 32, kCodeWindow = 1 << 14;
int host_build_col16(int64_t n, const std::vector<int32_t>& rowptr, const std::vector<int32_t>& colidx, std::vector<uint16_t>& code,
                     std::vector<int32_t>& tbase, int64_t* n_wide);
int host_build_solver_pattern(const HostSpace& hs, bool use_bnd, std::vector<int32_t>& rowptr_s, std::vector<int32_t>& colidx_s,
                              std::vector<int32_t>& full2s);


struct CellPartitions {
    int32_t cells_per_part = 0, max_colours = 0;
    int64_t n_parts = 0;
    std::vector<int32_t> cell_list;
    std::vector<int32_t> colour_off;
    std::vector<uint8_t> dof_shared;
    std::vector<int32_t> slot_map;
};
int host_build_cell_partitions(const HostSpace& hs, int cells_per_part, CellPartitions& cp, std::string& err);
void host_build_slot_map(const HostSpace& hs, const int32_t* list, int64_t n, std::vector<int32_t>& out);

constexpr int kPersistT = 512;
constexpr int kPersistRmax = 16;
constexpr int kPersistRwide = 24;
inline int persist_rows_per_thread(int64_t rpw, int64_t max_halo, bool halo_free, bool sym) {
    constexpr int64_t T = kPersistT;
    int R = 2;
    while (R <= kPersistRmax && ((int64_t)R * T < rpw || (!halo_free && (int64_t)(R / 2) * T < max_halo))) R *= 2;
    if (R <= kPersistRmax) return R;
    if (!sym && (int64_t)kPersistRwide * T >= rpw && (halo_free || (int64_t)(kPersistRwide / 2) * T >= max_halo)) return kPersistRwide;
    return 0;
}
#ifdef __HIPCC__
__host__ __device__
#endif
inline bool persist_sym_owner(int32_t row, int32_t col) {
    const uint32_t lo = (uint32_t)(row < col ? row : col), hi = (uint32_t)(row < col ? col : row);
    const bool low_owns = ((((lo * 2654435761u) ^ (hi * 2246822519u)) >> 16) & 1u) != 0;
    return (low_owns ? lo : hi) == (uint32_t)row;
}
inline int64_t persist_want_workgroups(int64_t n_int, int64_t nnz_kept, int lds_entries, int32_t single_rows) {
    if (n_int <= single_rows) return 1;
    int64_t want = (n_int + 2047) / 2048;
    if (lds_entries > 0) {
        const int64_t fit = (nnz_kept + nnz_kept / 16 + lds_entries - 1) / lds_entries;
        if (fit > want) want = fit;
    }
    return want;
}
inline bool persist_want_sym(int sym_mode, int64_t nnz_kept, int G, int64_t rows_per_wg) {
    const bool plain_streams = 10.6 * (double)nnz_kept / (double)G + 16.0 * (double)rows_per_wg > 150e3;
    return sym_mode == 1 || (sym_mode == 2 && rows_per_wg > 2048 && plain_streams) || (sym_mode == 3 && plain_streams);
}
struct PersistLayout {
    int32_t single_rows = 2048;
    bool sym = false;
    bool bisect = false;
    int G = 0, R = 0, nsl = 0;
    int64_t n_int = 0;
    int64_t n_entries = 0;
    int64_t nnz = 0;
    int64_t nnz_full = 0;
    int64_t n_board = 0;
    int64_t n_imp = 0;
    int64_t n_drop = 0;
    int32_t max_imp = 0, max_exp = 0;
    int64_t max_block = 0;
    std::vector<int32_t> slot_dof;
    std::vector<int64_t> ell_off;
    std::vector<int32_t> sl_off;
    std::vector<uint16_t> ell_code;
    std::vector<int32_t> ell_src;
    std::vector<int32_t> exp_off;
    std::vector<uint16_t> exp_slot;
    std::vector<int32_t> imp_off;
    std::vector<int32_t> imp_pos;
    std::vector<int32_t> ghost_needed;
    std::vector<int32_t> wg_of, slot_of;
    std::vector<uint8_t> wg_late;
};
int host_build_persist_layout(const HostSpace& hs, bool use_bnd, int n_wg, int lds_entries, PersistLayout& pl, const int32_t* block_rows = nullptr,
                              int sym_mode = 0, bool balance = false, const int32_t* ghost_order = nullptr, bool allow_late = false);

inline double persist_bisect_span(int M, int N, int64_t n) {
    const double key_span = (double)((uint64_t(1) << (N == 3 ? 21 : 31)) - 1);
    double levels = std::floor(std::pow((double)(n > 1 ? n : 1), 1.0 / (double)(M >= 1 ? M : 1)) + 0.5) - 1.0;
    return levels < 1.0 ? 1.0 : (levels > key_span ? key_span : levels);
}
void host_bisect_quantise(int N, int64_t n, const double* pts_colmajor, const int32_t* i2e, double span, std::vector<uint32_t>& q);
int host_bisect_partition(int64_t n_int, const int32_t* cost, const uint32_t* qx, const uint32_t* qy, const uint32_t* qz, int G, std::vector<int32_t>& perm,
                          std::vector<int32_t>& block_rows);
int host_build_persist_layout_bisect(const HostSpace& hs, bool use_bnd, int G, int lds_entries, PersistLayout& pl, int sym_mode, const uint32_t* q,
                                     std::vector<int32_t>* perm_out = nullptr, std::vector<int32_t>* rows_out = nullptr);

}
#endif
```

fdapde-core_amd/csrc/kernels_persist.h:

```cpp
#ifndef FDAPDE_KERNELS_PERSIST_H
#define FDAPDE_KERNELS_PERSIST_H

#include <hip/hip_runtime.h>

#include <type_traits>

#include "internal.h"

#ifndef FDAPDE_SYM_U8
#define FDAPDE_SYM_U8 1
#endif
#ifndef FDAPDE_SYM_NT_V
#define FDAPDE_SYM_NT_V 0
#endif
#ifndef FDAPDE_SYM_NT_C
#define FDAPDE_SYM_NT_C 0
#endif
#ifndef FDAPDE_SYM_U
#define FDAPDE_SYM_U 1
#endif

namespace fdapde_hip {

#ifdef FDAPDE_DOT_STRIDE6
constexpr int kDotStride = 6;
#else
constexpr int kDotStride = 8;
#endif
#ifdef FDAPDE_GATHER_3BAR
constexpr bool kGather3 = true;
#else
constexpr bool kGather3 = false;
#endif

struct PersistArgs {
    int32_t G, nsl, maxit, imp_cap;
    int32_t lds_cap;
    int32_t time_phases;
    int32_t gather_waves, poll_sleep;
    uint32_t epoch0;
    int32_t timeout_ticks;
    int32_t debug_stall_it;
    int32_t n_cols;
    int64_t col_stride, board_stride;
    int32_t direct;
    const double* b_ext;
    double* x_ext;
    double* rec;
    int32_t exp_lds;
    double* hrec;
    double* u_out;
    const int32_t* i2e;
    const double* scale;
    int32_t pf_steps;
    double tol2;
    const int32_t* slot_dof;
    const int64_t* ell_off;
    const int32_t* sl_off;
    const uint16_t* ell_code;
    const double* ell_val;
    const int32_t* exp_off;
    const uint16_t* exp_slot;
    const int32_t* imp_off;
    const int32_t* imp_pos;
    unsigned long long* pboard;
    unsigned long long* dboard;
    const unsigned long long* amax_bits;
    int32_t max_len;
    const double* r_in;
    const double* x;
    double* x_slots;
    double* x_out;
    double* sc;
    int32_t* ctl;
    double* stats;
    int32_t world, rank, n_board_local;
    int32_t flat_gather, g_base, G_tot;
    int32_t timeout_first_ticks;
    const int32_t* rexp_off;
    const uint16_t* rexp_slot;
    const int32_t* rexp_peer;
    const int32_t* rexp_pos;
    const uint8_t* wg_late;
    unsigned long long* rboard;
    unsigned long long* const* peer_pboard;
    unsigned long long* const* peer_dboard;
};

typedef __attribute__((address_space(1))) unsigned long long pg_u64;

__device__ __forceinline__ void granule_store(unsigned long long* p, unsigned epoch, unsigned payload) {
    __hip_atomic_store((pg_u64*)p, ((unsigned long long)epoch << 32) | payload, __ATOMIC_RELAXED,
                       __HIP_MEMORY_SCOPE_AGENT);
}
__device__ __forceinline__ unsigned long long granule_load(const unsigned long long* p) {
    return __hip_atomic_load((const pg_u64*)p, __ATOMIC_RELAXED, __HIP_MEMORY_SCOPE_AGENT);
}
typedef unsigned long long pg_v2u64 __attribute__((ext_vector_type(2)));
typedef unsigned int pg_u32x4 __attribute__((ext_vector_type(4)));
__device__ __forceinline__ pg_v2u64 granule_load2(const unsigned long long* p) {
    pg_v2u64 v;
    asm volatile("global_load_dwordx4 %0, %1, off sc1\n\ts_waitcnt vmcnt(0)" : "=v"(v) : "v"(p) : "memory");
    return v;
}
__device__ __forceinline__ void granule_load6(const unsigned long long* p, pg_v2u64& a, pg_v2u64& b, pg_v2u64& c) {
    asm volatile("global_load_dwordx4 %0, %3, off sc1\n\tglobal_load_dwordx4 %1, %3, off offset:16 sc1\n\t"
                 "global_load_dwordx4 %2, %3, off offset:32 sc1\n\ts_waitcnt vmcnt(0)"
                 : "=&v"(a), "=&v"(b), "=&v"(c) : "v"(p) : "memory");
}
__device__ __forceinline__ bool granule_pair_ok(pg_v2u64 v, unsigned epoch) {
    return (unsigned)(v.x >> 32) == epoch && (unsigned)(v.y >> 32) == epoch;
}
__device__ __forceinline__ double granule_pair_f64(pg_v2u64 v) {
    return __longlong_as_double((long long)((v.y << 32) | (v.x & 0xffffffffull)));
}
__device__ __forceinline__ void publish_f64(unsigned long long* g2, unsigned epoch, double v) {
    const unsigned long long b = (unsigned long long)__double_as_longlong(v);
    granule_store(g2, epoch, (unsigned)b);
    granule_store(g2 + 1, epoch, (unsigned)(b >> 32));
}
__device__ __forceinline__ void publish_f64_x4(unsigned long long* g2, unsigned epoch, double v) {
    const unsigned long long b = (unsigned long long)__double_as_longlong(v);
    pg_u32x4 q;
    q.x = (unsigned)b, q.y = epoch, q.z = (unsigned)(b >> 32), q.w = epoch;
    asm volatile("global_store_dwordx4 %0, %1, off sc1" ::"v"(g2), "v"(q) : "memory");
}
__device__ __forceinline__ void granule_load2x4(const unsigned long long* p0, const unsigned long long* p1, const unsigned long long* p2,
                                                const unsigned long long* p3, pg_v2u64& a, pg_v2u64& b, pg_v2u64& c, pg_v2u64& d) {
    asm volatile("global_load_dwordx4 %0, %4, off sc1\n\tglobal_load_dwordx4 %1, %5, off sc1\n\t"
                 "global_load_dwordx4 %2, %6, off sc1\n\tglobal_load_dwordx4 %3, %7, off sc1\n\ts_waitcnt vmcnt(0)"
                 : "=&v"(a), "=&v"(b), "=&v"(c), "=&v"(d) : "v"(p0), "v"(p1), "v"(p2), "v"(p3) : "memory");
}
__device__ __forceinline__ void publish_f64_x4_sys(unsigned long long* g2, unsigned epoch, double v) {
    const unsigned long long b = (unsigned long long)__double_as_longlong(v);
    pg_u32x4 q;
    q.x = (unsigned)b, q.y = epoch, q.z = (unsigned)(b >> 32), q.w = epoch;
    asm volatile("global_store_dwordx4 %0, %1, off sc0 sc1" ::"v"(g2), "v"(q) : "memory");
}
__device__ __forceinline__ pg_v2u64 granule_load2_sys(const unsigned long long* p) {
    pg_v2u64 v;
    asm volatile("global_load_dwordx4 %0, %1, off sc0 sc1\n\ts_waitcnt vmcnt(0)" : "=v"(v) : "v"(p) : "memory");
    return v;
}
__device__ __forceinline__ void granule_load6_sys(const unsigned long long* p, pg_v2u64& a, pg_v2u64& b, pg_v2u64& c) {
    asm volatile("global_load_dwordx4 %0, %3, off sc0 sc1\n\tglobal_load_dwordx4 %1, %3, off offset:16 sc0 sc1\n\t"
                 "global_load_dwordx4 %2, %3, off offset:32 sc0 sc1\n\ts_waitcnt vmcnt(0)"
                 : "=&v"(a), "=&v"(b), "=&v"(c) : "v"(p) : "memory");
}
__device__ __forceinline__ void granule_load2x4_sys(const unsigned long long* p0, const unsigned long long* p1, const unsigned long long* p2,
                                                    const unsigned long long* p3, pg_v2u64& a, pg_v2u64& b, pg_v2u64& c, pg_v2u64& d) {
    asm volatile("global_load_dwordx4 %0, %4, off sc0 sc1\n\tglobal_load_dwordx4 %1, %5, off sc0 sc1\n\t"
                 "global_load_dwordx4 %2, %6, off sc0 sc1\n\tglobal_load_dwordx4 %3, %7, off sc0 sc1\n\ts_waitcnt vmcnt(0)"
                 : "=&v"(a), "=&v"(b), "=&v"(c), "=&v"(d) : "v"(p0), "v"(p1), "v"(p2), "v"(p3) : "memory");
}
__device__ __forceinline__ void touch_line(const void* p, unsigned lds_dump) {
    unsigned m0_saved;
    asm volatile("s_mov_b32 %0, m0\n\ts_mov_b32 m0, %2\n\tglobal_load_lds_dword %1, off\n\ts_mov_b32 m0, %0" : "=&s"(m0_saved) : "v"(p), "s"(lds_dump) : "memory");
}
template <int RI, int W>
__device__ __forceinline__ void touch_first_step(const int32_t* slo, const void* gv, const void* gc, int wave, int lane, unsigned lds_dump) {
    constexpr int per_wave = RI * 10, total = 2 * per_wave;
    if (wave < W / 2) return;
#pragma unroll
    for (int t = 0; t * 64 < total; ++t) {
        int idx = min(t * 64 + lane, total - 1);
        asm volatile("" : "+v"(idx));
        const int half = idx / per_wave, rem = idx - half * per_wave;
        const int j = rem / 10, k = rem - j * 10;
        const int tw = (wave - W / 2) + half * (W / 2);
        const int o = slo[j * W + tw], wj = slo[j * W + tw + 1] - o;
        const char* line = k < 8 ? static_cast<const char*>(gv) + (size_t)o * 1024 + k * 128 : static_cast<const char*>(gc) + (size_t)o * 256 + (k - 8) * 128;
        if (t * 64 + lane < total && wj > 0) touch_line(line, lds_dump);
    }
}
template <int CTRL> __device__ __forceinline__ double persist_dpp_f64(double v) {
    const long long b = __double_as_longlong(v);
    const int lo = __builtin_amdgcn_update_dpp(0, (int)(b & 0xffffffffll), CTRL, 0xf, 0xf, false);
    const int hi = __builtin_amdgcn_update_dpp(0, (int)(b >> 32), CTRL, 0xf, 0xf, false);
    return __longlong_as_double(((long long)hi << 32) | (unsigned int)lo);
}
template <int O> __device__ __forceinline__ double persist_swap_sum(double v) {
    const long long b = __double_as_longlong(v);
    const unsigned l = (unsigned)(b & 0xffffffffll), h = (unsigned)(b >> 32);
    const auto lo = O == 32 ? __builtin_amdgcn_permlane32_swap(l, l, false, false) : __builtin_amdgcn_permlane16_swap(l, l, false, false);
    const auto hi = O == 32 ? __builtin_amdgcn_permlane32_swap(h, h, false, false) : __builtin_amdgcn_permlane16_swap(h, h, false, false);
    return __longlong_as_double(((long long)hi[0] << 32) | lo[0]) + __longlong_as_double(((long long)hi[1] << 32) | lo[1]);
}
__device__ __forceinline__ double wave_max64(double v) {
#ifdef FDAPDE_WAVE_SUM_SHFL
#pragma unroll
    for (int o = 32; o > 0; o >>= 1) v = fmax(v, __shfl_xor(v, o));
    return v;
#endif
    const long long b = __double_as_longlong(v);
    const unsigned l = (unsigned)(b & 0xffffffffll), h = (unsigned)(b >> 32);
    const auto lo = __builtin_amdgcn_permlane32_swap(l, l, false, false), hi = __builtin_amdgcn_permlane32_swap(h, h, false, false);
    v = fmax(__longlong_as_double(((long long)hi[0] << 32) | lo[0]), __longlong_as_double(((long long)hi[1] << 32) | lo[1]));
    const long long b2 = __double_as_longlong(v);
    const unsigned l2 = (unsigned)(b2 & 0xffffffffll), h2 = (unsigned)(b2 >> 32);
    const auto lo2 = __builtin_amdgcn_permlane16_swap(l2, l2, false, false), hi2 = __builtin_amdgcn_permlane16_swap(h2, h2, false, false);
    v = fmax(__longlong_as_double(((long long)hi2[0] << 32) | lo2[0]), __longlong_as_double(((long long)hi2[1] << 32) | lo2[1]));
    v = fmax(v, persist_dpp_f64<0x128>(v));
    v = fmax(v, persist_dpp_f64<0x124>(v));
    v = fmax(v, persist_dpp_f64<0x4E>(v));
    v = fmax(v, persist_dpp_f64<0xB1>(v));
    return v;
}
__device__ __forceinline__ double wave_sum64(double v) {
#ifdef FDAPDE_WAVE_SUM_SHFL
#pragma unroll
    for (int o = 32; o > 0; o >>= 1) v += __shfl_xor(v, o);
    return v;
#endif
    v = persist_swap_sum<32>(v);
    v = persist_swap_sum<16>(v);
    v += persist_dpp_f64<0x128>(v);
    v += persist_dpp_f64<0x124>(v);
    v += persist_dpp_f64<0x4E>(v);
    v += persist_dpp_f64<0xB1>(v);
    return v;
}


template <int R, bool STREAM, bool SYM, bool DIST = false, int WIDE_GJ = 12>
static __global__ __launch_bounds__(kPersistT) void k_cg_persist(PersistArgs a) {
    constexpr int T = kPersistT, W = T / 64, S = R * T, RI = R / 2;
    constexpr bool WIDE = R > kPersistRmax;
    constexpr bool PLDS = SYM || WIDE;
    static_assert(!WIDE || (STREAM && !SYM && !DIST), "the wide form is the plain streaming storage on one GPU");
    extern __shared__ __attribute__((aligned(128))) double lds[];
    __shared__ double red[W][3], red2[W][3];
    __shared__ double tot[3];
    __shared__ double pmax_w[W];
    __shared__ int32_t fail_flag;
    const int g = blockIdx.x, tid = threadIdx.x, lane = tid & 63, wave = tid >> 6;
    if constexpr (!DIST) {
        if (a.n_cols > 1) {
            const size_t col = blockIdx.y;
            a.r_in += col * a.col_stride, a.x_out += col * a.col_stride, a.sc += 4 * col, a.ctl += 4 * col;
            if (a.x != nullptr) a.x += col * a.col_stride;
            a.pboard += col * a.board_stride, a.dboard += col * a.board_stride;
        }
    }
    const int nsl = a.nsl;
    const int H = a.imp_off[g + 1] - a.imp_off[g], exp0 = a.exp_off[g], E = a.exp_off[g + 1] - exp0;
    unsigned long long* const exp_board = a.pboard + 2 * (size_t)exp0;
    double* p_tab = lds;
    long long* y_tab = reinterpret_cast<long long*>(p_tab + (S + a.imp_cap));
    double2* ev = reinterpret_cast<double2*>(y_tab + (SYM ? S : 0));
    uint32_t* ec = reinterpret_cast<uint32_t*>(ev + a.lds_cap / 2);
    int32_t* impl_l = reinterpret_cast<int32_t*>(ec + a.lds_cap / 2);
    uint16_t* expl_l = reinterpret_cast<uint16_t*>(impl_l + a.imp_cap);
    const int64_t e0 = a.ell_off[g];
    const double2* gv = reinterpret_cast<const double2*>(a.ell_val + e0);
    const uint32_t* gc = reinterpret_cast<const uint32_t*>(a.ell_code + e0);
    const int64_t e_left = a.ell_off[a.G] + 256 - e0;
    const __amdgpu_buffer_rsrc_t rs_v = __builtin_amdgcn_make_buffer_rsrc(const_cast<double2*>(gv), 0, (int)min(e_left * 8, (int64_t)0x7fffffff), 0x00020000);
    const __amdgpu_buffer_rsrc_t rs_c = __builtin_amdgcn_make_buffer_rsrc(const_cast<uint32_t*>(gc), 0, (int)min(e_left * 2, (int64_t)0x7fffffff), 0x00020000);
    const int lane16 = lane * 16, lane4 = lane * 4;
    const int32_t* impl = PLDS ? a.imp_pos + a.imp_off[g] : impl_l;
    const uint16_t* expl = PLDS ? a.exp_slot + a.exp_off[g] : expl_l;
    bool expl_in_lds = !PLDS;
    if constexpr (SYM && STREAM && !DIST) {
        if (a.exp_lds) {
            uint16_t* expl_s = reinterpret_cast<uint16_t*>(y_tab + S);
            for (int i = tid; i < E; i += T) expl_s[i] = a.exp_slot[exp0 + i];
            expl = expl_s;
            expl_in_lds = true;
        }
    }
    if constexpr (!PLDS) {
        for (int i = tid; i < H; i += T) impl_l[i] = a.imp_pos[a.imp_off[g] + i];
        for (int i = tid; i < E; i += T) expl_l[i] = a.exp_slot[a.exp_off[g] + i];
    } else if constexpr (SYM) {
#pragma unroll
        for (int j = 0; j < R; ++j) y_tab[j * T + tid] = 0;
    }
    int bexp = 0;
    if constexpr (SYM) {
        const double amax = __longlong_as_double((long long)*a.amax_bits);
        bexp = amax > 0.0 && amax < 1.7e308 ? ilogb(amax * (double)a.max_len) + 1 : 0;
    }
    if (tid == 0) fail_flag = 0;
    const int32_t* slo = a.sl_off + (size_t)g * (nsl + 1);
    if constexpr (!STREAM) {
        const int n_pairs = slo[nsl] * 64;
        for (int i = tid; i < n_pairs; i += T) ev[i] = gv[i], ec[i] = gc[i];
    }
    int o0[R], w[R];
#pragma unroll
    for (int j = 0; j < R; ++j) {
        o0[j] = __builtin_amdgcn_readfirstlane(slo[j * W + wave]);
        w[j] = __builtin_amdgcn_readfirstlane(slo[j * W + wave + 1]) - o0[j];
    }
    double xv[WIDE ? 1 : R], rv[R], pv[PLDS ? 1 : R];
    int32_t dof[PLDS ? 1 : R];
    double* const xs = WIDE ? a.x_slots + (size_t)g * S + tid : nullptr;
    double rr_part = 0;
    auto P = [&](int j) -> double {
        if constexpr (PLDS) return p_tab[j * T + tid];
        else return pv[j];
    };
#pragma unroll
    for (int j = 0; j < R; ++j) {
        const int32_t d = a.slot_dof[(size_t)g * S + j * T + tid];
        const bool on = d >= 0;
        if (!DIST && a.direct) rv[j] = on ? a.scale[d] * (a.b_ext[a.i2e[d]] - 0.0) : 0.0;
        else rv[j] = on ? a.r_in[d] : 0.0;
        const double x0 = on && a.x != nullptr ? a.x[d] : 0.0;
        if constexpr (WIDE) xs[j * T] = x0;
        else xv[j] = x0;
        if constexpr (PLDS) p_tab[j * T + tid] = rv[j];
        else pv[j] = rv[j], dof[j] = d;
        rr_part += rv[j] * rv[j];
    }
    double bb = (!DIST && a.direct) ? 0.0 : a.sc[0];
    const bool stamper = a.time_phases && tid == 0;
    long long t_spmv = 0, t_gather = 0, t_update = 0, n_stamped = 0;
    int it = 0, status = 0;
    double rr = 0;
    __shared__ unsigned pf_dump[64];
    [[maybe_unused]] auto prefetch_next = [&]() {
        if constexpr (STREAM)
            if (a.pf_steps != 0) touch_first_step<RI, W>(slo, gv, gc, wave, lane, (unsigned)(size_t)(__attribute__((address_space(3))) unsigned*)pf_dump);
    };
    __syncthreads();
    for (;;) {
        const unsigned epoch = a.epoch0 + (unsigned)it + 1u;
        const long long tmo = (DIST && it == 0) ? (long long)a.timeout_first_ticks : (long long)a.timeout_ticks;
        if (a.debug_stall_it > 0 && it == a.debug_stall_it && g == a.G - 1) {
            status = 3;
            break;
        }
        long long c0 = 0, c1 = 0, c2 = 0;
        if (stamper) c0 = wall_clock64();
        if constexpr (!PLDS) {
#pragma unroll
            for (int j = 0; j < R; ++j) p_tab[j * T + tid] = pv[j];
        }
        double tscale = 0, tinv = 0;
        if constexpr (SYM) {
            double m = 0;
#pragma unroll
            for (int j = 0; j < R; ++j) m = fmax(m, fabs(P(j)));
            m = wave_max64(m);
            if (lane == 0) pmax_w[wave] = m;
        }
        __syncthreads();
        if constexpr (SYM) {
            double m = 0;
#pragma unroll
            for (int ww = 0; ww < W; ++ww) m = fmax(m, pmax_w[ww]);
            const int ex = m > 0.0 && m < 1.7e308 ? min(max(61 - bexp - ilogb(m), -1000), 1000) : 0;
            tscale = ldexp(1.0, ex), tinv = ldexp(1.0, -ex);
        }
        constexpr bool PS_REG = SYM && R <= 8;
        double psj[PS_REG ? R : 1];
        if constexpr (PS_REG) {
#pragma unroll
            for (int j = 0; j < R; ++j) psj[j] = P(j) * tscale;
        }
        [[maybe_unused]] long long c_exp = 0, c_first = 0;
        {
            auto publish = [&](auto codes) {
                for (int i0 = tid; i0 < E; i0 += 4 * T) {
                    unsigned code[4];
                    double pe[4];
#pragma unroll
                    for (int k = 0; k < 4; ++k) code[k] = codes[min(i0 + k * T, E - 1)];
#pragma unroll
                    for (int k = 0; k < 4; ++k) pe[k] = p_tab[code[k]];
#pragma unroll
                    for (int k = 0; k < 4; ++k)
                        if (i0 + k * T < E) publish_f64_x4(exp_board + 2 * (size_t)(i0 + k * T), epoch, pe[k]);
                }
            };
            if (expl_in_lds) publish((const __attribute__((address_space(3))) uint16_t*)expl);
            else publish(expl);
            if constexpr (DIST) {
                const int re0 = a.rexp_off[g], RE = a.rexp_off[g + 1] - re0;
                for (int i = tid; i < RE; i += T) {
                    const unsigned slot = a.rexp_slot[re0 + i];
                    publish_f64_x4_sys(a.peer_pboard[a.rexp_peer[re0 + i]] + 2 * (size_t)a.rexp_pos[re0 + i], epoch, p_tab[slot]);
                }
            }
#ifdef FDAPDE_STAMP_EXPORT
            if (stamper) c_exp = wall_clock64();
#endif
        }
        double yv[R];
#pragma unroll
        for (int j = 0; j < R; ++j) yv[j] = P(j);
        auto product = [&](auto phase) {
            constexpr int J0 = decltype(phase)::value ? RI : 0, J1 = decltype(phase)::value ? R : RI, NJ = J1 - J0;
            int mw = 0;
#pragma unroll
            for (int j = J0; j < J1; ++j) mw = max(mw, w[j]);
            if constexpr (!SYM && STREAM) {
                constexpr int U = NJ >= 4 ? 1 : 8 / NJ;
                constexpr int GJ = NJ > 8 ? WIDE_GJ : NJ;
                static_assert(NJ % GJ == 0, "the passes of a phase in equal groups");
                for (int e = 0; e < mw; e += U) {
#pragma unroll
                    for (int jg = J0; jg < J1; jg += GJ) {
                        pg_u32x4 v[U][GJ];
                        uint32_t c[U][GJ];
#pragma unroll
                        for (int u = 0; u < U; ++u)
#pragma unroll
                            for (int j = jg; j < jg + GJ; ++j) {
                                if (e + u < w[j]) {
                                    const int row = o0[j] + e + u;
                                    v[u][j - jg] = __builtin_amdgcn_raw_buffer_load_b128(rs_v, lane16, row * 1024, 0);
                                    c[u][j - jg] = __builtin_amdgcn_raw_buffer_load_b32(rs_c, lane4, row * 256, 0);
                                }
                            }
#pragma unroll
                        for (int u = 0; u < U; ++u)
#pragma unroll
                            for (int j = jg; j < jg + GJ; ++j) {
                                if (e + u < w[j]) {
                                    const pg_u32x4 q = v[u][j - jg];
                                    const double vx = __hiloint2double((int)q.y, (int)q.x), vy = __hiloint2double((int)q.w, (int)q.z);
                                    yv[j] += vx * p_tab[c[u][j - jg] & 0xffffu] + vy * p_tab[c[u][j - jg] >> 16];
                                }
                            }
                    }
                }
            } else if constexpr (!SYM) {
                double2 vn[NJ];
                uint32_t cn[NJ];
                auto fetch = [&](int e) {
#pragma unroll
                    for (int j = J0; j < J1; ++j) {
                        const int ee = min(e, max(w[j] - 1, 0));
                        const int idx = (o0[j] + ee) * 64 + lane;
                        if constexpr (STREAM) vn[j - J0] = gv[idx], cn[j - J0] = gc[idx];
                        else vn[j - J0] = ev[idx], cn[j - J0] = ec[idx];
                    }
                };
                if (mw > 0) fetch(0);
                for (int e = 0; e < mw; ++e) {
                    double2 v[NJ];
                    double pa[NJ], pb[NJ];
#pragma unroll
                    for (int j = J0; j < J1; ++j) {
                        v[j - J0] = vn[j - J0];
                        pa[j - J0] = p_tab[cn[j - J0] & 0xffffu], pb[j - J0] = p_tab[cn[j - J0] >> 16];
                    }
                    if (e + 1 < mw) fetch(e + 1);
#pragma unroll
                    for (int j = J0; j < J1; ++j) {
                        const double t = v[j - J0].x * pa[j - J0] + v[j - J0].y * pb[j - J0];
                        yv[j] += e < w[j] ? t : 0.0;
                    }
                }
            } else {
                auto load = [&](auto& v, auto& c, int jg, int e) {
                    constexpr int GS = sizeof(c) / sizeof(c[0]);
#pragma unroll
                    for (int j = jg; j < jg + GS; ++j) {
                        if (e < w[j]) {
                            const int row = o0[j] + e;
                            if constexpr (STREAM) {
                                v[j - jg] = __builtin_amdgcn_raw_buffer_load_b128(rs_v, lane16, row * 1024, FDAPDE_SYM_NT_V);
                                c[j - jg] = __builtin_amdgcn_raw_buffer_load_b32(rs_c, lane4, row * 256, FDAPDE_SYM_NT_C);
                            } else v[j - jg] = reinterpret_cast<const pg_u32x4*>(ev)[row * 64 + lane], c[j - jg] = ec[row * 64 + lane];
                        }
                    }
                };
                auto compute = [&](const auto& v, const auto& c, int jg, int e) {
                    constexpr int GS = sizeof(c) / sizeof(c[0]);
#pragma unroll
                    for (int j = jg; j < jg + GS; ++j) {
                        if (e < w[j]) {
                            const unsigned c_lo = c[j - jg] & 0xffffu, c_hi = c[j - jg] >> 16;
                            const double vx = __hiloint2double((int)v[j - jg].y, (int)v[j - jg].x), vy = __hiloint2double((int)v[j - jg].w, (int)v[j - jg].z);
                            yv[j] += vx * p_tab[c_lo] + vy * p_tab[c_hi];
                            double ps;
                            if constexpr (PS_REG) ps = psj[j];
                            else ps = P(j) * tscale;
                            const long long q_lo = (long long)(vx * ps), q_hi = (long long)(vy * ps);
                            const bool t_lo = c_lo < (unsigned)S, t_hi = c_hi < (unsigned)S;
                            __hip_atomic_fetch_add(&y_tab[t_lo ? c_lo : (unsigned)(j * T + tid)], t_lo ? q_lo : 0ll, __ATOMIC_RELAXED, __HIP_MEMORY_SCOPE_WORKGROUP);
                            __hip_atomic_fetch_add(&y_tab[t_hi ? c_hi : (unsigned)(j * T + tid)], t_hi ? q_hi : 0ll, __ATOMIC_RELAXED, __HIP_MEMORY_SCOPE_WORKGROUP);
                        }
                    }
                };
                constexpr int U = !STREAM ? 1 : (NJ <= 4 ? FDAPDE_SYM_U : (NJ == 8 ? FDAPDE_SYM_U8 : 1));
                if constexpr (U == 1) {
                    for (int e = 0; e < mw; ++e) {
                        pg_u32x4 v[NJ];
                        uint32_t c[NJ];
                        load(v, c, J0, e);
                        compute(v, c, J0, e);
#ifdef FDAPDE_STAMP_EXPORT
                        if (stamper && e == 0 && J0 == 0) c_first = wall_clock64();
#endif
                    }
                } else {
                    for (int e = 0; e < mw; e += U) {
                        pg_u32x4 v[U][NJ];
                        uint32_t c[U][NJ];
#pragma unroll
                        for (int u = 0; u < U; ++u) load(v[u], c[u], J0, e + u);
#pragma unroll
                        for (int u = 0; u < U; ++u) compute(v[u], c[u], J0, e + u);
                    }
                }
            }
        };
        const bool late = a.wg_late != nullptr && a.wg_late[g] != 0;
        if (!late) product(std::integral_constant<int, 0>{});
        {
            bool fail = false;
            for (int hb = wave * 64; hb < H; hb += 4 * T) {
                const unsigned long long* gp[4];
                pg_v2u64 v[4];
                bool done[4];
                [[maybe_unused]] bool far[4];
#pragma unroll
                for (int k = 0; k < 4; ++k) {
                    const int h = hb + k * T + lane;
                    done[k] = h >= H;
                    const int32_t pos = impl[done[k] ? 0 : h];
                    if constexpr (DIST) {
                        far[k] = pos >= a.n_board_local;
                        gp[k] = far[k] ? a.rboard + 2 * (size_t)(pos - a.n_board_local) : a.pboard + 2 * (size_t)pos;
                    } else
                        gp[k] = a.pboard + 2 * (size_t)pos;
                }
                if constexpr (DIST) {
                    granule_load2x4(gp[0], gp[1], gp[2], gp[3], v[0], v[1], v[2], v[3]);
#pragma unroll
                    for (int k = 0; k < 4; ++k)
                        if (far[k]) v[k] = granule_load2_sys(gp[k]);
                } else
                    granule_load2x4(gp[0], gp[1], gp[2], gp[3], v[0], v[1], v[2], v[3]);
#pragma unroll
                for (int k = 0; k < 4; ++k) done[k] = done[k] || granule_pair_ok(v[k], epoch);
                long long t_wait = 0;
                for (unsigned spins = 0; !__all(done[0] && done[1] && done[2] && done[3]); ++spins) {
                    if ((spins & 63u) == 63u) {
                        const long long now = wall_clock64();
                        if (t_wait == 0) t_wait = now;
                        else if (now - t_wait > tmo) {
                            fail = true;
                            break;
                        }
                    }
                    __builtin_amdgcn_s_sleep(2);
#pragma unroll
                    for (int k = 0; k < 4; ++k)
                        if (!done[k]) {
                            if constexpr (DIST) v[k] = far[k] ? granule_load2_sys(gp[k]) : granule_load2(gp[k]);
                            else v[k] = granule_load2(gp[k]);
                            done[k] = granule_pair_ok(v[k], epoch);
                        }
                }
#pragma unroll
                for (int k = 0; k < 4; ++k) {
                    const int h = hb + k * T + lane;
                    if (h < H) p_tab[S + h] = granule_pair_f64(v[k]);
                }
                if (fail) break;
            }
            if (fail && lane == 0) fail_flag = 1;
        }
        const bool solo = !DIST && a.G == 1;
        if (!solo) {
            __syncthreads();
            if (fail_flag) {
                status = 3;
                break;
            }
        }
        if (late) product(std::integral_constant<int, 0>{});
        product(std::integral_constant<int, 1>{});
        if constexpr (SYM) {
            __syncthreads();
#pragma unroll
            for (int j = 0; j < R; ++j) {
                yv[j] += (double)y_tab[j * T + tid] * tinv;
                y_tab[j * T + tid] = 0;
            }
        }
        if (stamper) c1 = wall_clock64();
        double s0 = 0, s1 = 0;
#pragma unroll
        for (int j = 0; j < R; ++j) s0 += P(j) * yv[j], s1 += yv[j] * yv[j];
        s0 = wave_sum64(s0), s1 = wave_sum64(s1);
        const double s2 = wave_sum64(rr_part);
        if (lane == 0) red[wave][0] = s0, red[wave][1] = s1, red[wave][2] = s2;
        __syncthreads();
        double solo_tot[3] = {0.0, 0.0, 0.0};
        const bool flat = DIST && a.flat_gather != 0;
        if (flat) {
            if (tid < 3) {
                double v = 0;
#pragma unroll
                for (int ww = 0; ww < W; ++ww) v += red[ww][tid];
                tot[tid] = v;
            }
            __syncthreads();
            const size_t fbuf = (size_t)2 * a.world * 8 + (size_t)(it & 1) * a.G_tot * 8;
            if (tid < 3 * a.world) {
                const int k = tid % 3, q = tid / 3;
                publish_f64_x4_sys(a.peer_dboard[q] + fbuf + (size_t)(a.g_base + g) * 8 + 2 * k, epoch, tot[k]);
            }
            if (a.G_tot <= (W / 2) * 64) prefetch_next();
            double v0 = 0, v1 = 0, v2 = 0;
            bool fail = false;
            const int per_lane = (a.G_tot + T - 1) / T;
            if (wave * 64 < a.G_tot) {
                for (int rsel = 0; rsel < per_lane; ++rsel) {
                    const int w = rsel * T + tid;
                    const unsigned long long* gp = a.peer_dboard[a.rank] + fbuf + (size_t)(w < a.G_tot ? w : 0) * 8;
                    pg_v2u64 q0 = {0, 0}, q1 = {0, 0}, q2 = {0, 0};
                    bool done = w >= a.G_tot;
                    long long t_wait = 0;
                    for (unsigned spins = 0;; ++spins) {
                        if (!done) {
                            granule_load6_sys(gp, q0, q1, q2);
                            done = granule_pair_ok(q0, epoch) && granule_pair_ok(q1, epoch) && granule_pair_ok(q2, epoch);
                        }
                        if (__all(done)) break;
                        if ((spins & 63u) == 63u) {
                            const long long now = wall_clock64();
                            if (t_wait == 0) t_wait = now;
                            else if (now - t_wait > tmo) {
                                fail = true;
                                break;
                            }
                        }
                        __builtin_amdgcn_s_sleep(2);
                    }
                    if (w < a.G_tot && !fail) v0 += granule_pair_f64(q0), v1 += granule_pair_f64(q1), v2 += granule_pair_f64(q2);
                    if (fail) break;
                }
            }
            if (fail && lane == 0) fail_flag = 1;
            v0 = wave_sum64(v0), v1 = wave_sum64(v1), v2 = wave_sum64(v2);
            __syncthreads();
            if (lane == 0) red[wave][0] = v0, red[wave][1] = v1, red[wave][2] = v2;
            __syncthreads();
            if (tid < 3) {
                double v = 0;
#pragma unroll
                for (int ww = 0; ww < W; ++ww) v += red[ww][tid];
                tot[tid] = v;
            }
        } else if (!DIST && a.G == 1) {
#pragma unroll
            for (int ww = 0; ww < W; ++ww) solo_tot[0] += red[ww][0], solo_tot[1] += red[ww][1], solo_tot[2] += red[ww][2];
            prefetch_next();
        } else {
        unsigned long long* dslot = a.dboard + (size_t)(it & 1) * a.G * kDotStride;
        if (tid < 3) {
            double v = 0;
#pragma unroll
            for (int ww = 0; ww < W; ++ww) v += red[ww][tid];
            publish_f64_x4(dslot + (size_t)g * kDotStride + 2 * tid, epoch, v);
        }
        prefetch_next();
        {
            double v0 = 0, v1 = 0, v2 = 0;
            bool fail = false;
            const int per_lane = a.gather_waves == 1 ? (a.G + 63) / 64 : 1;
            if (a.gather_waves == 1 ? wave == 0 : wave * 64 < a.G) {
                for (int rsel = 0; rsel < per_lane; ++rsel) {
                    const int w = a.gather_waves == 1 ? rsel * 64 + lane : tid;
                    const unsigned long long* gp = dslot + (size_t)(w < a.G ? w : 0) * kDotStride;
                    pg_v2u64 q0 = {0, 0}, q1 = {0, 0}, q2 = {0, 0};
// ... 39 lines not shown
        if constexpr (DIST) {
            __syncthreads();
            const bool lfail = fail_flag != 0;
            const size_t rbuf = (size_t)(it & 1) * a.world * 8;
            if (g == 0 && !lfail && tid < 3 * a.world) {
                const int k = tid % 3, q = tid / 3;
                publish_f64_x4_sys(a.peer_dboard[q] + rbuf + (size_t)a.rank * 8 + 2 * k, epoch, tot[k]);
            }
            __syncthreads();
            if (wave == 0 && !lfail) {
                const unsigned long long* gp = a.peer_dboard[a.rank] + rbuf + (size_t)(lane < a.world ? lane : 0) * 8;
                pg_v2u64 q0 = {0, 0}, q1 = {0, 0}, q2 = {0, 0};
                bool done = lane >= a.world, fail = false;
                long long t_wait = 0;
                for (unsigned spins = 0;; ++spins) {
                    if (!done) {
                        granule_load6_sys(gp, q0, q1, q2);
                        done = granule_pair_ok(q0, epoch) && granule_pair_ok(q1, epoch) && granule_pair_ok(q2, epoch);
                    }
                    if (__all(done)) break;
                    if ((spins & 63u) == 63u) {
                        const long long now = wall_clock64();
                        if (t_wait == 0) t_wait = now;
                        else if (now - t_wait > tmo) {
                            fail = true;
                            break;
                        }
                    }
                    __builtin_amdgcn_s_sleep(1);
                }
                const bool on = lane < a.world && !fail;
                const double w0 = wave_sum64(on ? granule_pair_f64(q0) : 0.0), w1 = wave_sum64(on ? granule_pair_f64(q1) : 0.0),
                             w2 = wave_sum64(on ? granule_pair_f64(q2) : 0.0);
                if (lane == 0) {
                    tot[0] = w0, tot[1] = w1, tot[2] = w2;
                    if (fail) fail_flag = 1;
                }
            }
        }
        }
        if (!solo) {
            __syncthreads();
            if (fail_flag) {
                status = 3;
                break;
            }
            if constexpr (!DIST && !kGather3) {
#pragma unroll
                for (int ww = 0; ww < W; ++ww) solo_tot[0] += red2[ww][0], solo_tot[1] += red2[ww][1], solo_tot[2] += red2[ww][2];
            }
        }
        const bool own_tot = !DIST && (!kGather3 || solo);
        const double pAp = own_tot ? solo_tot[0] : tot[0], yy = own_tot ? solo_tot[1] : tot[1];
        rr = own_tot ? solo_tot[2] : tot[2];
        if (!DIST && a.direct && it == 0) bb = rr;
        if (stamper) c2 = wall_clock64();
        if (rr <= a.tol2 * bb) {
            status = 1;
            break;
        }
        if (!(pAp > 0.0)) {
            status = 2;
            break;
        }
        if (it >= a.maxit) break;
        const double alpha = rr / pAp;
        const double est = alpha * alpha * yy - rr;
        const double beta = (est > 0.0 && rr > 0.0) ? est / rr : 0.0;
        rr_part = 0;
        if constexpr (WIDE) {
#pragma unroll
            for (int j = 0; j < R; ++j) rv[j] -= alpha * yv[j], rr_part += rv[j] * rv[j];
#pragma unroll
            for (int j = 0; j < R; ++j) yv[j] = xs[j * T];
#pragma unroll
            for (int j = 0; j < R; ++j) {
                const double pj = P(j);
                xs[j * T] = yv[j] + alpha * pj;
                p_tab[j * T + tid] = rv[j] + beta * pj;
            }
        } else {
#pragma unroll
        for (int j = 0; j < R; ++j) {
            const double pj = P(j);
            xv[j] += alpha * pj;
            rv[j] -= alpha * yv[j];
            if constexpr (PLDS) p_tab[j * T + tid] = rv[j] + beta * pj;
            else pv[j] = rv[j] + beta * pj;
            rr_part += rv[j] * rv[j];
        }
        }
        ++it;
        if (stamper) {
            const long long c3 = wall_clock64();
#ifdef FDAPDE_STAMP_EXPORT
            t_spmv += c1 - c0, t_gather += c_exp - c0, t_update += (c_first > 0 ? c_first : c_exp) - c0, ++n_stamped;
            (void)c2, (void)c3;
#else
            t_spmv += c1 - c0, t_gather += c2 - c1, t_update += c3 - c2, ++n_stamped;
#endif
        }
    }
    if constexpr (STREAM) asm volatile("s_waitcnt vmcnt(0)" ::: "memory");
    if (status != 3) {
#pragma unroll
        for (int j = 0; j < R; ++j) {
            int32_t d;
            if constexpr (PLDS) d = a.slot_dof[(size_t)g * S + j * T + tid];
            else d = dof[j];
            double xj;
            if constexpr (WIDE) xj = xs[j * T];
            else xj = xv[j];
            if (!DIST && a.direct) {
                if (d >= 0) a.x_ext[a.i2e[d]] = a.scale[d] * xj + 0.0;
            } else if (d >= 0) {
                a.x_out[d] = xj;
                if (!DIST && a.u_out != nullptr) a.u_out[d] = a.scale[d] * xj + 0.0;
            }
        }
    }
    if (!DIST && a.direct) {
        asm volatile("s_waitcnt vmcnt(0)" ::: "memory");
        __syncthreads();
        if (tid == 0) {
            a.rec[0] = (double)it, a.rec[1] = rr, a.rec[2] = bb;
            __atomic_store_n(reinterpret_cast<volatile long long*>(a.rec + 3), (long long)(status + 1), __ATOMIC_RELEASE);
        }
    } else if (g == 0 && tid == 0 && status != 3) {
        a.sc[3] = rr;
        a.ctl[0] = status == 1 ? 1 : 0, a.ctl[1] = it, a.ctl[2] = status == 2 ? 1 : 0;
    }
    if constexpr (!DIST) {
        if (a.hrec != nullptr && g == 0 && tid == 0) {
            a.hrec[0] = status == 1 ? 1.0 : 0.0, a.hrec[1] = (double)it, a.hrec[2] = status == 2 ? 1.0 : 0.0, a.hrec[3] = status == 3 ? 1.0 : 0.0;
            a.hrec[4] = (double)a.ctl[4], a.hrec[5] = bb, a.hrec[6] = rr;
        }
    }
    if (stamper) {
        double* st = a.stats + 4 * (size_t)g;
        st[0] = (double)n_stamped, st[1] = (double)t_spmv, st[2] = (double)t_gather, st[3] = (double)t_update;
    }
    if (status == 3 && tid == 0 && !(!DIST && a.direct)) atomicExch(a.ctl + 3, 1);
}

struct BlockedSpmvArgs {
    int32_t G, nsl, imp_cap, dot2_ww;
    const int32_t* slot_dof;
    const int64_t* ell_off;
    const int32_t* sl_off;
    const uint16_t* ell_code;
    const double* ell_val;
    const int32_t* imp_off;
    const int32_t* imp_dof;
    const int32_t* drop_dof;
    int32_t n_drop;
    const double* x;
    double* y;
    const double* w;
    double* partial;
    const int32_t* stop;
};
template <int R>
static __global__ __launch_bounds__(kPersistT) void k_spmv_blocked(BlockedSpmvArgs a) {
    constexpr int T = kPersistT, W = T / 64, S = R * T;
    extern __shared__ __attribute__((aligned(128))) double lds[];
    __shared__ double red[W][2];
    if (a.stop && __syncthreads_or(*a.stop != 0)) return;
    const int g = blockIdx.x, tid = threadIdx.x, lane = tid & 63, wave = tid >> 6;
    const int nsl = a.nsl;
    double* p_tab = lds;
    const int H = a.imp_off[g + 1] - a.imp_off[g];
    const int64_t e0 = a.ell_off[g];
    const double2* gv = reinterpret_cast<const double2*>(a.ell_val + e0);
    const uint32_t* gc = reinterpret_cast<const uint32_t*>(a.ell_code + e0);
    const int64_t e_left = a.ell_off[a.G] + 256 - e0;
    const __amdgpu_buffer_rsrc_t rs_v = __builtin_amdgcn_make_buffer_rsrc(const_cast<double2*>(gv), 0, (int)min(e_left * 8, (int64_t)0x7fffffff), 0x00020000);
    const __amdgpu_buffer_rsrc_t rs_c = __builtin_amdgcn_make_buffer_rsrc(const_cast<uint32_t*>(gc), 0, (int)min(e_left * 2, (int64_t)0x7fffffff), 0x00020000);
    const int lane16 = lane * 16, lane4 = lane * 4;
    const int32_t* slo = a.sl_off + (size_t)g * (nsl + 1);
    int o0[R], w[R];
#pragma unroll
    for (int j = 0; j < R; ++j) {
        o0[j] = __builtin_amdgcn_readfirstlane(slo[j * W + wave]);
        w[j] = __builtin_amdgcn_readfirstlane(slo[j * W + wave + 1]) - o0[j];
    }
    double yv[R];
    int32_t dof[R];
#pragma unroll
    for (int j = 0; j < R; ++j) {
        dof[j] = a.slot_dof[(size_t)g * S + j * T + tid];
        yv[j] = dof[j] >= 0 ? a.x[dof[j]] : 0.0;
        p_tab[j * T + tid] = yv[j];
    }
    for (int h = tid; h < H; h += T) p_tab[S + h] = a.x[a.imp_dof[a.imp_off[g] + h]];
    __syncthreads();
    double wy = 0, second = 0;
    if (a.w != nullptr && a.dot2_ww) {
#pragma unroll
        for (int j = 0; j < R; ++j) {
            const double wv = (a.w == a.x) ? yv[j] : (dof[j] >= 0 ? a.w[dof[j]] : 0.0);
            second += wv * wv;
        }
    }
    auto product = [&](auto) {
        constexpr int J0 = 0, J1 = R;
        int mw = 0;
#pragma unroll
        for (int j = J0; j < J1; ++j) mw = max(mw, w[j]);
        constexpr int U = 2;
        for (int e = 0; e < mw; e += U) {
            pg_u32x4 v[U][J1 - J0];
            uint32_t c[U][J1 - J0];
#pragma unroll
            for (int u = 0; u < U; ++u)
#pragma unroll
                for (int j = J0; j < J1; ++j) {
                    if (e + u < w[j]) {
                        const int row = o0[j] + e + u;
                        v[u][j - J0] = __builtin_amdgcn_raw_buffer_load_b128(rs_v, lane16, row * 1024, 0);
                        c[u][j - J0] = __builtin_amdgcn_raw_buffer_load_b32(rs_c, lane4, row * 256, 0);
                    }
                }
#pragma unroll
            for (int u = 0; u < U; ++u)
#pragma unroll
// ... 118 lines not shown
```

fdapde-core_amd/csrc/persist_engine.hip:

```cpp
#include <algorithm>
#include <atomic>
#include <cstring>
#include <utility>

#include <unistd.h>

#include "engine.h"
#include "kernels_persist.h"
#include "kernels_persist_bicg.h"

static inline size_t dboard_offset(int64_t n_board) { return (2 * (size_t)n_board + 7) & ~(size_t)7; }

namespace fdapde_engine {

static int compare_dev_persist(fdapde_ctx* c, const PersistLayout& pl, const DevPersist& dp, const PersistLayout& ref);
int check_dev_persist(fdapde_ctx* c, int v, const PersistLayout& pl, const DevPersist& dp, const std::vector<int32_t>* block_rows, bool balance, int n_wg) {
    if (int rc = ensure_host(c, kHostPattern)) return rc;
    PersistLayout ref;
    ref.single_rows = pl.single_rows;
    if (host_build_persist_layout(c->hs, v == 1, n_wg, 12000, ref, block_rows ? block_rows->data() : nullptr,
                                  pl.sym ? 1 : 0, balance) != FDAPDE_OK) return fail(c, FDAPDE_EHIP, "set-up check: host persistent layout failed");
    return compare_dev_persist(c, pl, dp, ref);
}
int check_dev_persist_bisect(fdapde_ctx* c, int v, const PersistLayout& pl, const DevPersist& dp, const std::vector<int32_t>& perm, const std::vector<int32_t>& rows) {
    if (int rc = ensure_host(c, kHostPattern | kHostDofs)) return rc;
    std::vector<uint32_t> q;
    host_bisect_quantise(c->hs.N, c->hs.n_dofs, c->hs.dof_coords.data(), c->hs.dof_i2e.data(), persist_bisect_span(c->hs.M, c->hs.N, c->hs.n_dofs), q);
    PersistLayout ref;
    ref.single_rows = pl.single_rows;
    std::vector<int32_t> perm_h, rows_h;
    if (host_build_persist_layout_bisect(c->hs, v == 1, pl.G, 12000, ref, pl.sym ? 1 : 0, q.data(), &perm_h, &rows_h) != FDAPDE_OK)
        return fail(c, FDAPDE_EHIP, "set-up check: host bisection layout failed");
    const bool same_perm = perm == perm_h, same_rows = rows == rows_h;
    std::fprintf(stderr, "persist check %-9s: %s (%zu elements)\n", "bis_perm", same_perm ? "ok" : "MISMATCH", perm_h.size());
    std::fprintf(stderr, "persist check %-9s: %s (%zu elements)\n", "bis_rows", same_rows ? "ok" : "MISMATCH", rows_h.size());
    if (!same_perm || !same_rows) return fail(c, FDAPDE_EHIP, "FDAPDE_SETUP_CHECK: the device-built bisection differs from the host's (see stderr)");
    return compare_dev_persist(c, pl, dp, ref);
}
static int compare_dev_persist(fdapde_ctx* c, const PersistLayout& pl, const DevPersist& dp, const PersistLayout& ref) {
    int bad = 0;
    auto scalar = [&](const char* name, int64_t a, int64_t b) {
        if (a != b) std::fprintf(stderr, "persist check %-9s: MISMATCH %lld vs %lld\n", name, (long long)a, (long long)b), ++bad;
    };
    scalar("G", pl.G, ref.G), scalar("R", pl.R, ref.R), scalar("n_int", pl.n_int, ref.n_int), scalar("n_entries", pl.n_entries, ref.n_entries);
    scalar("nnz", pl.nnz, ref.nnz), scalar("n_board", pl.n_board, ref.n_board), scalar("max_imp", pl.max_imp, ref.max_imp), scalar("max_exp", pl.max_exp, ref.max_exp);
    auto cmp = [&](const char* name, const void* dev, const void* host, size_t bytes, size_t elem) {
        std::vector<unsigned char> tmp(bytes ? bytes : 1);
        if (bytes && hipMemcpy(tmp.data(), dev, bytes, hipMemcpyDeviceToHost) != hipSuccess) {
            ++bad;
            return;
        }
        size_t at = 0;
        while (at < bytes && tmp[at] == static_cast<const unsigned char*>(host)[at]) ++at;
        if (at < bytes) std::fprintf(stderr, "persist check %-9s: MISMATCH at element %zu of %zu\n", name, at / elem, bytes / elem), ++bad;
        else std::fprintf(stderr, "persist check %-9s: ok (%zu elements)\n", name, bytes / elem);
    };
    if (bad == 0) {
#define CMP(name, dptr, hvec_) cmp(name, dptr, (hvec_).data(), (hvec_).size() * sizeof((hvec_)[0]), sizeof((hvec_)[0]))
        CMP("slot_dof", dp.slot_dof, ref.slot_dof), CMP("ell_off", dp.ell_off, ref.ell_off), CMP("sl_off", dp.sl_off, ref.sl_off);
        CMP("ell_code", dp.ell_code, ref.ell_code), CMP("ell_src", dp.ell_src, ref.ell_src), CMP("exp_off", dp.exp_off, ref.exp_off);
        CMP("exp_slot", dp.exp_slot, ref.exp_slot), CMP("imp_off", dp.imp_off, ref.imp_off), CMP("imp_pos", dp.imp_pos, ref.imp_pos);
#undef CMP
    }
    if (bad) return fail(c, FDAPDE_EHIP, "FDAPDE_SETUP_CHECK: the device-built persistent layout differs from the host builder's (see stderr)");
    return FDAPDE_OK;
}

struct PersistNeeds {
    int S = 0, imp_cap = 0, exp_cap = 0;
    size_t fixed = 0;
    int64_t need = 0;
};
static PersistNeeds persist_needs(const PersistLayout& pl, bool host_built) {
    PersistNeeds n;
    n.S = pl.R * kPersistT;
    n.imp_cap = (pl.max_imp + 63) & ~63, n.exp_cap = (pl.max_exp + 63) & ~63;
    n.fixed = pl.sym ? 8 * (size_t)(n.S + n.imp_cap) + 8 * (size_t)n.S + 64 : 8 * (size_t)(n.S + n.imp_cap) + 4 * (size_t)n.imp_cap + 2 * (size_t)n.exp_cap + 64;
    if (pl.R > kPersistRmax) n.fixed = 8 * (size_t)(n.S + n.imp_cap) + 64;
    n.need = pl.max_block;
    for (int g = 0; g < pl.G && host_built; ++g) n.need = std::max<int64_t>(n.need, pl.ell_off[(size_t)g + 1] - pl.ell_off[(size_t)g]);
    n.need += 128;
    return n;
}

int build_persist_once(fdapde_ctx* c, int v, const std::vector<int32_t>* block_rows, bool balance) {
    fdapde_ctx::Persist& ps = c->ps[v];
    ps.ok = false;
    ps.ell_col.release();
    if (c->n_cu < 1) return FDAPDE_OK;
    const int32_t* brows = block_rows ? block_rows->data() : nullptr;
    const int n_wg = block_rows ? (int)block_rows->size() : (c->persist_max_wg > 0 ? std::min(c->persist_max_wg, c->n_cu) : c->n_cu);
    PersistLayout pl;
    DevPersist dp;
    DebugClock clk;
    const char* mode = std::getenv("FDAPDE_SETUP");
    bool on_device = !(mode && std::strcmp(mode, "host") == 0);
    if (c->hs.n_dofs <= c->persist_host_below && !(mode && std::strcmp(mode, "device") == 0)) on_device = false;
    double max_mb = 1024.0;
    if (const char* e = std::getenv("FDAPDE_PERSIST_MAX_MB")) max_mb = std::atof(e);
    const size_t lds_total = 160 * 1024 - 1024;
    size_t fixed = 0;
    int64_t need = 0;
    int imp_cap = 0, exp_cap = 0, S = 0;
    bool late_ok = c->persist_late != 0 && block_rows == nullptr;
    if (late_ok) on_device = false;
    int sym_mode = c->persist_sym == 2 ? 3 : c->persist_sym;
    if (c->persist_plain) sym_mode = 0;
    for (int attempt = 0; attempt < 2; ++attempt) {
        pl = PersistLayout{};
        pl.single_rows = c->persist_single_rows;
        int rc = FDAPDE_EUNSUPPORTED;
        if (on_device) {
            preload_wait(2);
            rc = dev_build_persist_layout(c->hs.n_dofs, c->hs.max_row, c->rowptr.p, c->colidx.p, c->bnd.p, v == 1, n_wg, 12000, 0, brows, sym_mode,
                                          balance, c->stream, pl, &dp, c->err);
            if (rc == FDAPDE_EUNSUPPORTED && c->hs.max_row > 255) on_device = false;
        }
        if (!on_device) {
            clk.mark("build_persist: (before ensure_host)");
            if (int rc2 = ensure_host(c, kHostPattern)) return rc2;
            clk.mark("build_persist: ensure_host");
            rc = host_build_persist_layout(c->hs, v == 1, n_wg, 12000, pl, brows, sym_mode, balance, nullptr, late_ok);
        }
        if (c->persist_plain && !late_ok && block_rows == nullptr && (rc == FDAPDE_EUNSUPPORTED || (rc == FDAPDE_OK && pl.R > 8)) &&
            (rc == FDAPDE_EUNSUPPORTED ? (c->hs.n_dofs + n_wg - 1) / n_wg <= 8 * kPersistT : (pl.n_int + pl.G - 1) / pl.G <= 8 * kPersistT) && attempt == 0) {
            dev_persist_release(&dp);
            late_ok = true, on_device = false;
            --attempt;
            continue;
        }
        if (rc == FDAPDE_EUNSUPPORTED && sym_mode != 0 && attempt == 0) {
            dev_persist_release(&dp);
            sym_mode = 0;
            continue;
        }
        if (rc == FDAPDE_EUNSUPPORTED) return FDAPDE_OK;
        if (rc) return rc;
        if (10.0 * (double)pl.n_entries > max_mb * 1e6) {
            dev_persist_release(&dp);
            return FDAPDE_OK;
        }
        {
            const PersistNeeds pn = persist_needs(pl, !on_device);
            S = pn.S, imp_cap = pn.imp_cap, exp_cap = pn.exp_cap, fixed = pn.fixed, need = pn.need;
        }
        if (pl.sym && fixed > lds_total && attempt == 0) {
            dev_persist_release(&dp);
            sym_mode = 0;
            continue;
        }
        if (c->persist_sym == 2 && pl.sym && attempt == 0 && pl.G == 1) {
            dev_persist_release(&dp);
            sym_mode = 0;
            continue;
        }
        if (c->persist_sym == 2 && pl.sym && attempt == 0) {
            const size_t fixed_plain = 8 * (size_t)(S + imp_cap) + 4 * (size_t)imp_cap + 2 * (size_t)exp_cap + 64;
            const size_t block_plain = (size_t)(1.03 * (double)pl.nnz_full / (double)pl.G) + 256;
            const bool plain_resident = pl.R < 16 && fixed_plain + 10 * block_plain <= lds_total;
            const bool sym_resident = fixed + 10 * (size_t)need <= lds_total;
            if (plain_resident || ((pl.n_int + pl.G - 1) / pl.G <= 2048 && !sym_resident)) {
                dev_persist_release(&dp);
                sym_mode = 0;
                continue;
            }
        }
        break;
    }
    clk.mark("build_persist: layout");
    ps.stream = fixed + 10 * (size_t)need > lds_total;
    if (fixed > lds_total || (pl.R >= 16 && !ps.stream) || (pl.R > kPersistRmax && (c->persist_plain || !c->persist_wide))) {
        dev_persist_release(&dp);
        return FDAPDE_OK;
    }
    const int part = c->persist_partition;
    const bool check = on_device && std::getenv("FDAPDE_SETUP_CHECK") != nullptr;
    if (check) {
        if (int rc2 = check_dev_persist(c, v, pl, dp, block_rows, balance, n_wg)) {
            dev_persist_release(&dp);
            return rc2;
        }
    }
    if (part != 0 && block_rows == nullptr && !late_ok && pl.G >= 2) {
        PersistLayout pl2;
        DevPersist dp2;
        pl2.single_rows = c->persist_single_rows;
        std::vector<int32_t> perm2, rows2;
        int rc2 = FDAPDE_EUNSUPPORTED;
        const size_t n_co = (size_t)c->hs.n_dofs * c->hs.N;
        if (on_device) {
            DBuf<double> coords_tmp;
            const double* coords = nullptr;
            if (c->hs.order == 1 && c->mesh_on_dev && c->mesh_nodes.n == n_co) coords = c->mesh_nodes.p;
            else if (c->coords_e.p && c->coords_e.n == n_co) coords = c->coords_e.p;
            else if (ensure_host(c, kHostDofs) == FDAPDE_OK && c->hs.dof_coords.size() == n_co &&
                     coords_tmp.upload(c->hs.dof_coords.data(), n_co, c->stream) == hipSuccess)
                coords = coords_tmp.p;
            if (coords)
                rc2 = dev_build_persist_layout_bisect(c->hs.n_dofs, c->hs.max_row, c->rowptr.p, c->colidx.p, c->bnd.p, v == 1, c->hs.M, c->hs.N, coords, c->dof_i2e.p, pl.G, 12000,
                                                      pl.sym ? 1 : 0, c->stream, pl2, &dp2, check ? &perm2 : nullptr, check ? &rows2 : nullptr, c->err);
            if (coords_tmp.p) (void)hipStreamSynchronize(c->stream);
        } else if (ensure_host(c, kHostPattern | kHostDofs) == FDAPDE_OK && c->hs.dof_coords.size() == n_co) {
            std::vector<uint32_t> q;
            host_bisect_quantise(c->hs.N, c->hs.n_dofs, c->hs.dof_coords.data(), c->hs.dof_i2e.data(), persist_bisect_span(c->hs.M, c->hs.N, c->hs.n_dofs), q);
            rc2 = host_build_persist_layout_bisect(c->hs, v == 1, pl.G, 12000, pl2, pl.sym ? 1 : 0, q.data());
        }
        if (rc2 != FDAPDE_OK) {
            (void)hipGetLastError();
            c->err.clear();
        }
        if (rc2 == FDAPDE_OK && check)
            if (int rc3 = check_dev_persist_bisect(c, v, pl2, dp2, perm2, rows2)) {
                dev_persist_release(&dp), dev_persist_release(&dp2);
                return rc3;
            }
        bool take = false;
        PersistNeeds pn2;
        bool stream2 = false;
        if (rc2 == FDAPDE_OK) {
            pn2 = persist_needs(pl2, !on_device);
            stream2 = pn2.fixed + 10 * (size_t)pn2.need > lds_total;
            auto bytes = [](const PersistLayout& l) {
                return 10.0 * (double)l.n_entries + 32.0 * (double)l.n_board + (l.R > kPersistRmax ? 16.0 * (double)l.n_int : 0.0);
            };
            const bool fits = 10.0 * (double)pl2.n_entries <= max_mb * 1e6 && pn2.fixed <= lds_total && !(pl2.R >= 16 && !stream2) &&
                              !(pl2.R > kPersistRmax && (c->persist_plain || !c->persist_wide));
            const bool same_form = pl2.sym == pl.sym && pl2.R <= pl.R && (!stream2 || ps.stream);
            take = fits && same_form && (part == 1 || bytes(pl2) < bytes(pl));
            if (std::getenv("FDAPDE_DEBUG_SETUP"))
                std::fprintf(stderr, "persistent CG layout %d: bisection %s: %.0f bytes per iteration against %.0f (entries %lld / %lld, board %lld / %lld, imports <= %d / %d, R %d / %d)\n",
                             v, take ? "taken" : "not taken", bytes(pl2), bytes(pl), (long long)pl2.n_entries, (long long)pl.n_entries, (long long)pl2.n_board,
                             (long long)pl.n_board, pl2.max_imp, pl.max_imp, pl2.R, pl.R);
        }
        if (take) {
            dev_persist_release(&dp);
            pl = std::move(pl2), dp = dp2;
            S = pn2.S, imp_cap = pn2.imp_cap, exp_cap = pn2.exp_cap, fixed = pn2.fixed, need = pn2.need, ps.stream = stream2;
            pl.bisect = true;
        } else
            dev_persist_release(&dp2);
        clk.mark("build_persist: bisection layout");
    }
    ps.lds_cap = ps.stream ? 0 : (int32_t)need, ps.imp_cap = imp_cap;
    ps.lds_bytes = fixed + (ps.stream ? 0 : 10 * (size_t)need);
    ps.exp_lds = pl.sym && ps.stream && pl.R <= kPersistRmax && ps.lds_bytes + 2 * (size_t)exp_cap + 1024 <= 160 * 1024 && c->persist_exp_lds;
    if (ps.exp_lds) ps.lds_bytes += 2 * (size_t)exp_cap;
    hipStream_t st = c->stream;
    if (on_device) {
        const size_t GS = (size_t)pl.G * S, n_alloc = (size_t)pl.n_entries + 256;
        adopt(ps.slot_dof, dp.slot_dof, GS), adopt(ps.ell_off, dp.ell_off, (size_t)pl.G + 1), adopt(ps.sl_off, dp.sl_off, (size_t)pl.G * (pl.nsl + 1));
        adopt(ps.ell_code, dp.ell_code, n_alloc), adopt(ps.ell_src, dp.ell_src, n_alloc), adopt(ps.exp_off, dp.exp_off, (size_t)pl.G + 1);
        adopt(ps.exp_slot, dp.exp_slot, (size_t)(pl.n_board ? pl.n_board : 1)), adopt(ps.imp_off, dp.imp_off, (size_t)pl.G + 1);
        adopt(ps.imp_pos, dp.imp_pos, (size_t)(pl.n_imp ? pl.n_imp : 1));
    } else {
        HIPCHK(c, ps.slot_dof.upload(pl.slot_dof.data(), pl.slot_dof.size(), st));
        HIPCHK(c, ps.ell_off.upload(pl.ell_off.data(), pl.ell_off.size(), st));
        HIPCHK(c, ps.sl_off.upload(pl.sl_off.data(), pl.sl_off.size(), st));
        HIPCHK(c, ps.ell_code.alloc(pl.ell_code.size() + 256));
        HIPCHK(c, hipMemsetAsync(ps.ell_code.p, 0, sizeof(uint16_t) * (pl.ell_code.size() + 256), st));
        HIPCHK(c, hipMemcpyAsync(ps.ell_code.p, pl.ell_code.data(), sizeof(uint16_t) * pl.ell_code.size(), hipMemcpyHostToDevice, st));
        HIPCHK(c, ps.ell_src.upload(pl.ell_src.data(), pl.ell_src.size(), st));
        HIPCHK(c, ps.exp_off.upload(pl.exp_off.data(), pl.exp_off.size(), st));
        HIPCHK(c, ps.exp_slot.upload(pl.exp_slot.data(), pl.exp_slot.size(), st));
        HIPCHK(c, ps.imp_off.upload(pl.imp_off.data(), pl.imp_off.size(), st));
        HIPCHK(c, ps.imp_pos.upload(pl.imp_pos.data(), pl.imp_pos.size(), st));
    }
    if (late_ok && !pl.wg_late.empty()) HIPCHK(c, ps.wg_late.upload(pl.wg_late.data(), pl.wg_late.size(), st));
    else ps.wg_late.release();
    HIPCHK(c, ps.ell_val.alloc((size_t)pl.n_entries + 256));
    HIPCHK(c, hipMemsetAsync(ps.ell_val.p, 0, sizeof(double) * ((size_t)pl.n_entries + 256), st));
    HIPCHK(c, ps.board.alloc(dboard_offset(pl.n_board) + 2 * (size_t)pl.G * 8 + 8));
    HIPCHK(c, hipMemsetAsync(ps.board.p, 0, sizeof(unsigned long long) * ps.board.n, st));
    ps.epoch_next = 0, ps.attr_set = nullptr;
    ps.board_cols.release();
    HIPCHK(c, ps.amax.alloc(1));
    HIPCHK(c, c->persist_stats.alloc(4 * 1024));
    HIPCHK(c, hipStreamSynchronize(st));
    clk.mark("build_persist: uploads + allocs");
    if (std::getenv("FDAPDE_DEBUG_SETUP"))
        std::fprintf(stderr, "persistent CG layout %d (%s-built): %d workgroups x %d rows/thread, %lld interior rows, %lld entries (%lld stored, %.1f %% padding), "
                     "LDS %zu B (%s%s, largest block %lld), imports <= %d, exports <= %d, board %lld\n", v, on_device ? "device" : "host", pl.G, pl.R,
                     (long long)pl.n_int, (long long)pl.n_entries, (long long)pl.nnz,
                     100.0 * (double)(pl.n_entries - pl.nnz) / (double)(pl.n_entries > 0 ? pl.n_entries : 1), ps.lds_bytes,
                     ps.stream ? "blocks stream" : "blocks resident", pl.sym ? (pl.bisect ? ", symmetric storage, bisection blocks" : ", symmetric storage") : (pl.bisect ? ", bisection blocks" : ""), (long long)need, pl.max_imp, pl.max_exp, (long long)pl.n_board);
    pl.slot_dof = {}, pl.ell_code = {}, pl.ell_src = {}, pl.exp_slot = {}, pl.imp_pos = {}, pl.sl_off = {}, pl.ell_off = {};
    ps.meta = std::move(pl);
    ps.filled = false, ps.ok = true;
    return FDAPDE_OK;
}

int launch_persist(fdapde_ctx* c, fdapde_ctx::Persist& ps, PersistArgs& a, bool dist = false, bool bicg = false) {
    hipStream_t st = c->stream;
    a.G = ps.meta.G, a.nsl = ps.meta.nsl, a.imp_cap = ps.imp_cap, a.lds_cap = ps.lds_cap;
    a.gather_waves = c->persist_gather_waves, a.poll_sleep = c->persist_poll_sleep;
    a.slot_dof = ps.slot_dof.p, a.ell_off = ps.ell_off.p, a.sl_off = ps.sl_off.p, a.ell_code = ps.ell_code.p;
    a.ell_val = ps.ell_val.p, a.exp_off = ps.exp_off.p, a.exp_slot = ps.exp_slot.p, a.imp_off = ps.imp_off.p, a.imp_pos = ps.imp_pos.p;
    if (!dist && a.n_cols <= 1) a.pboard = ps.board.p, a.dboard = ps.board.p + dboard_offset(ps.meta.n_board);
    if (!dist) a.wg_late = ps.wg_late.p;
    a.exp_lds = (!dist && !bicg && ps.exp_lds) ? 1 : 0;
    a.amax_bits = ps.amax.p, a.max_len = c->hs.max_row, a.stats = c->persist_stats.p;
    a.timeout_ticks = c->persist_timeout_us * 100, a.debug_stall_it = c->persist_debug_stall, a.pf_steps = c->persist_prefetch;
    if (!dist && ps.epoch_next > 0xC0000000u - 2u * (uint32_t)a.maxit) {
        HIPCHK(c, hipMemsetAsync(ps.board.p, 0, sizeof(unsigned long long) * ps.board.n, st));
        if (ps.board_cols.p) HIPCHK(c, hipMemsetAsync(ps.board_cols.p, 0, sizeof(unsigned long long) * ps.board_cols.n, st));
        ps.epoch_next = 0;
    }
    a.epoch0 = ps.epoch_next;
    if (a.time_phases) HIPCHK(c, hipMemsetAsync(c->persist_stats.p, 0, 4 * (size_t)a.G * sizeof(double), st));
    HIPCHK(c, hipEventRecord(c->ev_p0, st));
    void* kargs[] = {&a};
#define PERSIST_GO(R_, ST_, SY_) PERSIST_GO_D(R_, ST_, SY_, false)
#define PERSIST_GO_D(R_, ST_, SY_, DI_)                                                                                         \
    do {                                                                                                                        \
        const void* fn = reinterpret_cast<const void*>(&k_cg_persist<R_, ST_, SY_, DI_>);                                       \
        if (ps.attr_set != fn) {                                                                                                \
            DebugClock clk2;                                                                                                    \
            HIPCHK(c, hipFuncSetAttribute(fn, hipFuncAttributeMaxDynamicSharedMemorySize, (int)ps.lds_bytes));                  \
            clk2.mark("launch_persist: hipFuncSetAttribute");                                                                   \
            int per_cu = 0;                                                                                                     \
            HIPCHK(c, hipOccupancyMaxActiveBlocksPerMultiprocessor(&per_cu, fn, kPersistT, ps.lds_bytes));                      \
            clk2.mark("launch_persist: occupancy query");                                                                       \
            if ((int64_t)per_cu * c->n_cu < (int64_t)a.G) return FDAPDE_EUNSUPPORTED;    \
            ps.attr_set = fn, ps.per_cu = per_cu;                                                                               \
        }                                                                                                                       \
        const unsigned ncol = a.n_cols > 1 ? (unsigned)a.n_cols : 1u;                                                           \
        if ((int64_t)ps.per_cu * c->n_cu < (int64_t)a.G * ncol) return FDAPDE_EUNSUPPORTED;                                     \
        if (c->persist_coop) HIPCHK(c, hipLaunchCooperativeKernel(fn, dim3(a.G, ncol), dim3(kPersistT), kargs, (unsigned)ps.lds_bytes, st)); \
        else hipLaunchKernelGGL((k_cg_persist<R_, ST_, SY_, DI_>), dim3(a.G, ncol), dim3(kPersistT), ps.lds_bytes, st, a);      \
    } while (0)
#define PERSIST_GO2(R_, ST_)                                                                                                    \
    do {                                                                                                                        \
        if (ps.meta.sym) PERSIST_GO(R_, ST_, true);                                                                             \
        else PERSIST_GO(R_, ST_, false);                                                                                        \
    } while (0)
#define PERSIST_GOD(R_, ST_)                                                                                                    \
    do {                                                                                                                        \
        if (ps.meta.sym) PERSIST_GO_D(R_, ST_, true, true);                                                                     \
        else PERSIST_GO_D(R_, ST_, false, true);                                                                                \
    } while (0)
#define BICG_GO(R_, ST_, DI_)                                                                                                   \
    do {                                                                                                                        \
        const void* fn = reinterpret_cast<const void*>(&k_bicg_persist<R_, ST_, DI_>);                                          \
        if (ps.attr_set != fn) {                                                                                                \
            HIPCHK(c, hipFuncSetAttribute(fn, hipFuncAttributeMaxDynamicSharedMemorySize, (int)ps.lds_bytes));                  \
            int per_cu = 0;                                                                                                     \
            HIPCHK(c, hipOccupancyMaxActiveBlocksPerMultiprocessor(&per_cu, fn, kPersistT, ps.lds_bytes));                      \
            if ((int64_t)per_cu * c->n_cu < (int64_t)a.G) return FDAPDE_EUNSUPPORTED;                                           \
            ps.attr_set = fn, ps.per_cu = per_cu;                                                                               \
        }                                                                                                                       \
        const unsigned ncol = a.n_cols > 1 ? (unsigned)a.n_cols : 1u;                                                           \
        if ((int64_t)ps.per_cu * c->n_cu < (int64_t)a.G * ncol) return FDAPDE_EUNSUPPORTED;                                     \
        hipLaunchKernelGGL((k_bicg_persist<R_, ST_, DI_>), dim3(a.G, ncol), dim3(kPersistT), ps.lds_bytes, st, a);              \
    } while (0)
#define BICG_GO2(R_, ST_)                                                                                                       \
    do {                                                                                                                        \
        if (dist) BICG_GO(R_, ST_, true);                                                                                       \
        else BICG_GO(R_, ST_, false);                                                                                           \
    } while (0)
    if (bicg) {
        if (ps.meta.sym) return FDAPDE_EUNSUPPORTED;
        if (ps.stream) switch (ps.meta.R) {
            case 2: BICG_GO2(2, true); break;
            case 4: BICG_GO2(4, true); break;
            case 8: BICG_GO2(8, true); break;
            default: return FDAPDE_EUNSUPPORTED;
            }
        else switch (ps.meta.R) {
            case 2: BICG_GO2(2, false); break;
            case 4: BICG_GO2(4, false); break;
            case 8: BICG_GO2(8, false); break;
            default: return FDAPDE_EUNSUPPORTED;
            }
    } else if (dist) {
        if (ps.stream) switch (ps.meta.R) {
            case 2: PERSIST_GOD(2, true); break;
            case 4: PERSIST_GOD(4, true); break;
            case 8: PERSIST_GOD(8, true); break;
            case 16: PERSIST_GOD(16, true); break;
            default: return FDAPDE_EUNSUPPORTED;
            }
        else switch (ps.meta.R) {
            case 2: PERSIST_GOD(2, false); break;
            case 4: PERSIST_GOD(4, false); break;
            case 8: PERSIST_GOD(8, false); break;
            default: return FDAPDE_EUNSUPPORTED;
            }
    } else if (ps.stream) switch (ps.meta.R) {
        case 2: PERSIST_GO2(2, true); break;
        case 4: PERSIST_GO2(4, true); break;
        case 8: PERSIST_GO2(8, true); break;
        case 16: PERSIST_GO2(16, true); break;
        case kPersistRwide:
            if (ps.meta.sym || a.n_cols > 1 || a.direct) return FDAPDE_EUNSUPPORTED;
            if (c->persist_xs.n < (size_t)ps.meta.G * kPersistRwide * kPersistT) HIPCHK(c, c->persist_xs.alloc((size_t)ps.meta.G * kPersistRwide * kPersistT));
            a.x_slots = c->persist_xs.p;
            {
                const void* fn = c->persist_wide_gj == 12 ? reinterpret_cast<const void*>(&k_cg_persist<kPersistRwide, true, false, false, 12>)
                               : c->persist_wide_gj == 4  ? reinterpret_cast<const void*>(&k_cg_persist<kPersistRwide, true, false, false, 4>)
                                                          : reinterpret_cast<const void*>(&k_cg_persist<kPersistRwide, true, false, false, 6>);
                if (ps.attr_set != fn) {
                    HIPCHK(c, hipFuncSetAttribute(fn, hipFuncAttributeMaxDynamicSharedMemorySize, (int)ps.lds_bytes));
                    int per_cu = 0;
                    HIPCHK(c, hipOccupancyMaxActiveBlocksPerMultiprocessor(&per_cu, fn, kPersistT, ps.lds_bytes));
                    if ((int64_t)per_cu * c->n_cu < (int64_t)a.G) return FDAPDE_EUNSUPPORTED;
                    ps.attr_set = fn, ps.per_cu = per_cu;
                }
                if (c->persist_wide_gj == 12) hipLaunchKernelGGL((k_cg_persist<kPersistRwide, true, false, false, 12>), dim3(a.G), dim3(kPersistT), ps.lds_bytes, st, a);
                else if (c->persist_wide_gj == 4) hipLaunchKernelGGL((k_cg_persist<kPersistRwide, true, false, false, 4>), dim3(a.G), dim3(kPersistT), ps.lds_bytes, st, a);
                else hipLaunchKernelGGL((k_cg_persist<kPersistRwide, true, false, false, 6>), dim3(a.G), dim3(kPersistT), ps.lds_bytes, st, a);
            }
            break;
// ... 675 lines not shown
```

include/fdapde_hip.h:

```cpp
#ifndef FDAPDE_HIP_H
#define FDAPDE_HIP_H

#include <stdint.h>

#ifdef __cplusplus
extern "C" {
#endif

#define FDAPDE_ABI_VERSION 5

enum {
    FDAPDE_OK = 0,
    FDAPDE_EINVAL = 1,
    FDAPDE_ENOMEM = 2,
    FDAPDE_ENODEVICE = 3,
    FDAPDE_EHIP = 4,
    FDAPDE_ENOTINIT = 5,
    FDAPDE_ENOCONV = 6,
    FDAPDE_EUNSUPPORTED = 7,
    FDAPDE_ERCCL = 8
};

enum { FDAPDE_LAPLACIAN = 0, FDAPDE_DIFFUSION = 1, FDAPDE_ADVECTION = 2, FDAPDE_REACTION = 3, FDAPDE_DT = 4 };

// ... 20 lines not shown
    double rtol;
    int32_t assembly;
    int32_t check_every;
    int32_t time_spmv;
} fdapde_options;

typedef struct {
    int32_t iters;
    int32_t converged;
    double relres;
    double t_assemble_ms;
    double t_solve_ms;
    double t_setup_ms;
    double spmv_avg_ms;
    int32_t spmv_timed;
    int32_t method_used;
    int32_t persistent;
    double gather_avg_ms;
    double update_avg_ms;
    double spmv_mean_ms;
    double launch_ms;
} fdapde_info;

typedef struct fdapde_ctx fdapde_ctx;

int fdapde_abi_version(void);
int fdapde_device_count(void);
int fdapde_ctx_create(int device, fdapde_ctx **ctx);
void fdapde_ctx_destroy(fdapde_ctx *ctx);
int fdapde_ctx_clone(const fdapde_ctx *src, fdapde_ctx **out);
int fdapde_ctx_create_multi(const int32_t *devices, int32_t n_devices, fdapde_ctx **ctx);
int fdapde_ctx_devices(const fdapde_ctx *ctx, int32_t *n_devices, int32_t *devices, int32_t *form, double *t_partition_ms,
                       double *t_rank_setup_ms);
const char *fdapde_last_error(const fdapde_ctx *ctx);
const char *fdapde_status_string(int status);

int fdapde_mesh_upload(fdapde_ctx *ctx, int M, int N, int64_t n_nodes, const double *nodes_colmajor, int64_t n_cells,
                       const int32_t *cells_rowmajor, const uint8_t *boundary_nodes);

int fdapde_topology_build(fdapde_ctx *ctx, int64_t *n_facets, int64_t *n_edges);
int fdapde_topology_get(fdapde_ctx *ctx, int32_t *neighbors, int32_t *cell_facets, int32_t *facet_nodes, int32_t *facet_cells,
                        uint8_t *facet_boundary, int32_t *edge_nodes, uint8_t *edge_boundary, int32_t *face_edges);

int fdapde_dofs_build(fdapde_ctx *ctx, int order, int64_t *n_dofs);
int fdapde_dofs_get(const fdapde_ctx *ctx, int32_t *dofs_rowmajor, uint8_t *boundary_dofs, double *dof_coords_colmajor);
int fdapde_dofs_set_boundary(fdapde_ctx *ctx, const uint8_t *boundary_dofs);
int fdapde_sizes(const fdapde_ctx *ctx, int64_t *n_dofs, int64_t *nnz, int32_t *n_basis, int32_t *n_quadrature,
                 int64_t *n_edges);
int fdapde_pattern_get(const fdapde_ctx *ctx, int32_t *rowptr, int32_t *colidx);
int fdapde_quadrature_nodes(fdapde_ctx *ctx, double *out_colmajor);

int fdapde_set_operator(fdapde_ctx *ctx, int32_t n_terms, const fdapde_term *terms);
int fdapde_set_forcing(fdapde_ctx *ctx, const double *f_q, int32_t n_cols);
int fdapde_set_dirichlet(fdapde_ctx *ctx, const double *g);

int fdapde_init(fdapde_ctx *ctx, const fdapde_options *opt);
int fdapde_assemble_operator(fdapde_ctx *ctx, int32_t which, int32_t n_terms, const fdapde_term *terms, int32_t assembly);

int fdapde_solver_prepare(fdapde_ctx *ctx, int32_t with_dirichlet);
int fdapde_solve(fdapde_ctx *ctx, const fdapde_options *opt, fdapde_info *info);

int fdapde_solve_parabolic(fdapde_ctx *ctx, const fdapde_options *opt, int32_t n_times, double delta_t,
                           const double *initial_condition, const double *dirichlet, double *solution, fdapde_info *info);

int fdapde_lin_compute(fdapde_ctx *ctx, int32_t which, const double *values, int32_t symmetric);
int fdapde_lin_solve(fdapde_ctx *ctx, const fdapde_options *opt, const double *b, int32_t n_rhs, double *x, fdapde_info *info);

int fdapde_eval_pointwise(fdapde_ctx *ctx, int64_t n_locs, const double *locs_colmajor, int32_t *cell_ids, double *values);
int fdapde_cell_integrals(fdapde_ctx *ctx, double *measure, double *psi_int);

int fdapde_matrix_values(fdapde_ctx *ctx, int32_t which, double *values);
int fdapde_lump(fdapde_ctx *ctx, int32_t which, double *diag);
int fdapde_force(fdapde_ctx *ctx, double *force);
int fdapde_solution(fdapde_ctx *ctx, double *solution);
int fdapde_info_get(const fdapde_ctx *ctx, fdapde_info *info);

int fdapde_spmv(fdapde_ctx *ctx, int32_t which, const double *x, double *y);
int fdapde_bench_spmv(fdapde_ctx *ctx, int32_t reps, double *avg_ms, double *algorithmic_bytes);
int fdapde_solver_layout(fdapde_ctx *ctx, int32_t with_dirichlet, int64_t *n_interior, int64_t *nnz_interior,
                         double *streamed_bytes);
int fdapde_solver_layout_kind(fdapde_ctx *ctx, int32_t with_dirichlet, int32_t *kind, int32_t *symmetric_storage,
                              int32_t *workgroups, int32_t *rows_per_thread);
int fdapde_solver_layout_partition(fdapde_ctx *ctx, int32_t with_dirichlet, int32_t *partition);
typedef int (*fdapde_allreduce_fn)(void *user, double *host_buf, int64_t count);
int fdapde_comm_init_callback(fdapde_ctx *ctx, int32_t world, int32_t rank, fdapde_allreduce_fn fn, void *user);
int fdapde_comm_unique_id(void *out128);
int fdapde_comm_init(fdapde_ctx *ctx, int32_t world, int32_t rank, const void *unique_id128);
int fdapde_comm_allreduce(fdapde_ctx *ctx, double *host_inout, int32_t n, int32_t op);
int fdapde_comm_count(fdapde_ctx *ctx, int32_t *ranks);
const char *fdapde_comm_library(void);
int fdapde_halo_setup(fdapde_ctx *ctx, int64_t n_if_global, int64_t n_if_local, const int32_t *local_dof,
                      const int32_t *if_index, const uint8_t *owned);
typedef int (*fdapde_exchange_fn)(void *user, int32_t n_peers, const int32_t *peer_rank, const int64_t *peer_off, const double *send,
                                  double *recv);
int fdapde_comm_set_exchange_callback(fdapde_ctx *ctx, fdapde_exchange_fn fn, void *user);
int fdapde_halo_setup_peers(fdapde_ctx *ctx, int32_t n_peers, const int32_t *peer_rank, const int64_t *peer_off,
                            const int32_t *peer_dof, const uint8_t *owned);

int fdapde_rowdist_setup(fdapde_ctx *ctx, const int64_t *dof_key, const int32_t *dof_owner);

int fdapde_partition_build(fdapde_ctx *ctx, int32_t world, int32_t form);
int fdapde_partition_sizes(const fdapde_ctx *ctx, int32_t rank, int64_t *n_nodes, int64_t *n_cells);
int fdapde_partition_get(fdapde_ctx *ctx, int32_t rank, double *nodes_colmajor, int32_t *cells_rowmajor, uint8_t *boundary_nodes,
                         int64_t *node_ids, int64_t *cell_ids, int32_t *node_owner);
int fdapde_partition_whole(fdapde_ctx *ctx, int32_t *cell_rank, int32_t *node_owner, uint64_t *node_ranks);
int fdapde_partition_peers(fdapde_ctx *ctx, int32_t rank, int32_t *n_peers, int32_t *peer_rank, int64_t *peer_off, int32_t *peer_node,
                           uint8_t *owned, int64_t *n_shared);

int fdapde_tune(fdapde_ctx *ctx, const char *key, int32_t value);
void *fdapde_stream(fdapde_ctx *ctx);
int fdapde_synchronize(fdapde_ctx *ctx);

#ifdef __cplusplus
}
#endif
#endif
```

Baseline: 117.4 million.

## Keep head of streamed matrix blocks resident in spare LDS for persistent CG

Adds a residency plan that places the first records of each wave's streamed symmetric ELL values and codes into unused LDS (holes and spare capacity) of the persistent CG kernel. Those records are loaded once and reused across CG iterations instead of being re-streamed from HBM every SpMV. The kernel skips the resident depth when prefetching and streaming. The cost is larger dynamic LDS per workgroup, which may lower occupancy; the launcher falls back to the base layout if the grid no longer fits co-resident. A query API and a tune knob are added, with the feature on by default.

```diff
diff --git a/fdapde-core_amd/capi.py b/fdapde-core_amd/capi.py
--- a/fdapde-core_amd/capi.py
+++ b/fdapde-core_amd/capi.py
@@ -40,7 +40,7 @@
     "fdapde_info_get", "fdapde_spmv", "fdapde_bench_spmv", "fdapde_tune", "fdapde_stream", "fdapde_synchronize",
     "fdapde_comm_unique_id", "fdapde_comm_init", "fdapde_halo_setup", "fdapde_solve_parabolic",
     "fdapde_lin_compute", "fdapde_lin_solve", "fdapde_eval_pointwise", "fdapde_cell_integrals", "fdapde_comm_init_callback", "fdapde_comm_set_exchange_callback", "fdapde_halo_setup_peers",
-    "fdapde_solver_layout", "fdapde_topology_build", "fdapde_topology_get", "fdapde_comm_allreduce", "fdapde_comm_library", "fdapde_solver_layout_kind", "fdapde_solver_layout_partition", "fdapde_rowdist_setup", "fdapde_ctx_clone", "fdapde_comm_count",
+    "fdapde_solver_layout", "fdapde_topology_build", "fdapde_topology_get", "fdapde_comm_allreduce", "fdapde_comm_library", "fdapde_solver_layout_kind", "fdapde_solver_layout_partition", "fdapde_solver_layout_resident", "fdapde_rowdist_setup", "fdapde_ctx_clone", "fdapde_comm_count",
     "fdapde_ctx_create_multi", "fdapde_ctx_devices", "fdapde_partition_build", "fdapde_partition_sizes", "fdapde_partition_get", "fdapde_partition_whole",
     "fdapde_partition_peers",
 ]
@@ -456,6 +456,11 @@
         self._check(self.lib.fdapde_solver_layout_partition(self._ctx, 1 if with_dirichlet else 0, C.byref(p)))
         return p.value
 
+    def solver_layout_resident(self, with_dirichlet=True):
+        by, lo, hi = C.c_double(), C.c_int32(), C.c_int32()
+        self._check(self.lib.fdapde_solver_layout_resident(self._ctx, 1 if with_dirichlet else 0, C.byref(by), C.byref(lo), C.byref(hi)))
+        return dict(bytes=by.value, min_records=lo.value, max_records=hi.value)
+
     @staticmethod
     def comm_unique_id() -> bytes:
         buf = C.create_string_buffer(128)
diff --git a/fdapde-core_amd/csrc/capi.hip b/fdapde-core_amd/csrc/capi.hip
--- a/fdapde-core_amd/csrc/capi.hip
+++ b/fdapde-core_amd/csrc/capi.hip
@@ -107,7 +107,7 @@
               bk.ell_code.release(), bk.ell_val.release();
         for (auto& ps : c->ps)
             ps.slot_dof.release(), ps.sl_off.release(), ps.ell_src.release(), ps.exp_off.release(), ps.imp_off.release(),
-              ps.imp_pos.release(), ps.ell_off.release(), ps.ell_code.release(), ps.exp_slot.release(), ps.ell_val.release(), ps.board.release(), ps.board_cols.release(), ps.amax.release(), ps.wg_late.release(), ps.ell_col.release();
+              ps.imp_pos.release(), ps.ell_off.release(), ps.ell_code.release(), ps.exp_slot.release(), ps.ell_val.release(), ps.board.release(), ps.board_cols.release(), ps.amax.release(), ps.wg_late.release(), ps.ell_col.release(), ps.res_plan.release(), ps.res_depth.release();
         for (int v = 0; v < 2; ++v)
             c->sp_rowptr[v].release(), c->sp_colidx[v].release(), c->sp_map[v].release(), c->sp_tbase[v].release(), c->sp_col16[v].release(),
               c->sp_vrow[v].release();
@@ -258,6 +258,16 @@
     if (!c) return FDAPDE_EINVAL;
     if (c->group) return fdapde_engine::g_layout_kind(c, with_dirichlet, kind, symmetric_storage, workgroups, rows_per_thread);
     return fdapde_engine::e_solver_layout_kind(c, with_dirichlet, kind, symmetric_storage, workgroups, rows_per_thread);
+}
+int fdapde_solver_layout_resident(fdapde_ctx* c, int32_t with_dirichlet, double* resident_bytes, int32_t* min_records, int32_t* max_records) {
+    int32_t kind = 0;
+    if (int rc = fdapde_solver_layout_kind(c, with_dirichlet, &kind, nullptr, nullptr, nullptr)) return rc;
+    const fdapde_ctx::Persist& ps = c->ps[with_dirichlet ? 1 : 0];
+    const bool on = kind == 2 && ps.ok && ps.res_lds_bytes != 0;
+    if (resident_bytes) *resident_bytes = on ? (double)ps.res_bytes : 0.0;
+    if (min_records) *min_records = on ? ps.res_min : 0;
+    if (max_records) *max_records = on ? ps.res_max : 0;
+    return FDAPDE_OK;
 }
 int fdapde_solver_layout_partition(fdapde_ctx* c, int32_t with_dirichlet, int32_t* partition) {
     int32_t kind = 0;
@@ -485,6 +495,10 @@
         c->persist_partition = value;
         for (auto& ps : c->ps) ps.tried = ps.ok = ps.filled = false;
     }
+    else if (k == "persist_resident" && (value == 0 || value == 1)) {
+        c->persist_resident = value;
+        for (auto& ps : c->ps) ps.tried = ps.ok = ps.filled = false;
+    }
     else if (k == "persist_late" && (value == 0 || value == 1)) {
         c->persist_late = value;
         for (auto& ps : c->ps) ps.tried = ps.ok = ps.filled = false;
diff --git a/fdapde-core_amd/csrc/context.h b/fdapde-core_amd/csrc/context.h
--- a/fdapde-core_amd/csrc/context.h
+++ b/fdapde-core_amd/csrc/context.h
@@ -191,6 +191,7 @@
     DBuf<uint8_t> mesh_nbnd;
     bool mesh_on_dev = false;
     DBuf<double> gm_V, gm_b, gm_s, gm_part;
+    int persist_resident = 1;
     int persist_exp_lds = 1;
     int gmres_m = 50;
     int auto_gmres = 1;
@@ -321,6 +322,12 @@
         DBuf<uint16_t> ell_code, exp_slot;
         DBuf<double> ell_val;
         DBuf<unsigned long long> amax;
+        DBuf<uint32_t> res_plan;
+        DBuf<int32_t> res_depth;
+        size_t res_lds_bytes = 0;
+        int64_t res_bytes = 0;
+        int32_t res_min = 0, res_max = 0;
+        int per_cu_base = 0;
         DBuf<uint8_t> wg_late;
         DBuf<unsigned long long> board;
         DBuf<unsigned long long> board_cols;
diff --git a/fdapde-core_amd/csrc/eng_solve.hip b/fdapde-core_amd/csrc/eng_solve.hip
--- a/fdapde-core_amd/csrc/eng_solve.hip
+++ b/fdapde-core_amd/csrc/eng_solve.hip
@@ -900,7 +900,8 @@
     if (streamed_bytes) {
         if (persist) {
             *streamed_bytes = 10.0 * (double)c->ps[v].meta.n_entries + 32.0 * (double)c->ps[v].meta.n_board +
-                              (c->ps[v].meta.R > kPersistRmax ? 16.0 * (double)c->ps[v].meta.n_int : 0.0);
+                              (c->ps[v].meta.R > kPersistRmax ? 16.0 * (double)c->ps[v].meta.n_int : 0.0) -
+                              (c->ps[v].res_lds_bytes != 0 ? (double)c->ps[v].res_bytes : 0.0);
         } else if (blocked) {
             *streamed_bytes = 10.0 * (double)c->bk[v].meta.n_entries + 8.0 * (double)(c->bk[v].meta.n_int + c->bk[v].meta.n_imp) + 8.0 * (double)c->bk[v].meta.n_int;
         } else if (c->spmv_variant == 2 && c->sp_built[v]) {
@@ -1503,7 +1504,8 @@
         !c->lin_state->ss.use_bnd) {
         fdapde_ctx::Persist& ps = c->ps[0];
         const int G = ps.meta.G;
-        const int cap = (ps.per_cu > 0 ? ps.per_cu : 1) * c->n_cu / (G > 0 ? G : 1);
+        const int per_cu = std::max(ps.per_cu, ps.per_cu_base);
+        const int cap = (per_cu > 0 ? per_cu : 1) * c->n_cu / (G > 0 ? G : 1);
         const double tol2 = rtol * rtol;
         const int np = c->vec_grid;
         while (n_rhs - j0 >= 1 && cap >= 1) {
diff --git a/fdapde-core_amd/csrc/host_persist.cpp b/fdapde-core_amd/csrc/host_persist.cpp
--- a/fdapde-core_amd/csrc/host_persist.cpp
+++ b/fdapde-core_amd/csrc/host_persist.cpp
@@ -283,4 +283,120 @@
     return FDAPDE_OK;
 }
 
+int host_persist_resident_plan(const PersistLayout& pl, const uint8_t* hole_in, int imp_cap, size_t lds_used, size_t lds_budget, PersistResidentPlan& plan) {
+    constexpr int T = kPersistT, W = T / 64, REC = kPersistResRecord, VB = 1024, CB = 256;
+    plan = PersistResidentPlan{};
+    const int G = pl.G, R = pl.R, nsl = pl.nsl, S = R * T;
+    if (!pl.sym || G < 1 || R < 2 || R > kPersistRmax || nsl != R * W || pl.sl_off.size() != (size_t)G * (nsl + 1)) return FDAPDE_EINVAL;
+    if (hole_in == nullptr && pl.slot_dof.size() != (size_t)G * S) return FDAPDE_EINVAL;
+    plan.G = G, plan.R = R;
+    plan.words.assign((size_t)G * kPersistResWords, 0u);
+    plan.depth.assign((size_t)G * nsl, 0);
+    plan.rec_first.assign((size_t)G * W + 1, 0);
+    plan.hole.assign((size_t)G * nsl, 0);
+    const size_t spare0 = (lds_used + 255) & ~(size_t)255;
+    const size_t spare_bytes = lds_budget > spare0 ? ((lds_budget - spare0) / CB) * CB : 0;
+    plan.lds_bytes = spare_bytes > 0 ? spare0 + spare_bytes : lds_used;
+    const int64_t tab[2] = {0, 8 * (int64_t)(S + imp_cap)};
+    struct Range {
+        int64_t base, bytes;
+    };
+    for (int g = 0; g < G; ++g) {
+        uint8_t* hole = &plan.hole[(size_t)g * nsl];
+        for (int q = 0; q < nsl; ++q) {
+            if (hole_in) hole[q] = hole_in[(size_t)g * nsl + q] != 0;
+            else {
+                bool any = false;
+                for (int l = 0; l < 64 && !any; ++l) any = pl.slot_dof[(size_t)g * S + q * 64 + l] >= 0;
+                hole[q] = !any;
+            }
+        }
+        const int32_t* slo = &pl.sl_off[(size_t)g * (nsl + 1)];
+        for (int q = 0; q < nsl; ++q)
+            if (hole[q] && slo[q + 1] != slo[q]) return FDAPDE_EINVAL;
+        uint32_t* wd = &plan.words[(size_t)g * kPersistResWords];
+        for (int q = 0; q < nsl; ++q)
+            if (hole[q]) wd[q >> 5] |= 1u << (q & 31);
+        std::vector<Range> reg;
+        for (int t = 0; t < 2; ++t)
+            for (int q = 0; q < nsl;) {
+                if (!hole[q]) {
+                    ++q;
+                    continue;
+                }
+                int q1 = q;
+                while (q1 < nsl && hole[q1]) ++q1;
+                reg.push_back({tab[t] + (int64_t)512 * q, (int64_t)512 * (q1 - q)});
+                q = q1;
+            }
+        if (spare_bytes > 0) reg.push_back({(int64_t)spare0, (int64_t)spare_bytes});
+        int64_t rows_w[W], rows_all = 0, bytes_all = 0, vcap = 0;
+        for (int wv = 0; wv < W; ++wv) {
+            rows_w[wv] = 0;
+            for (int j = 0; j < R; ++j) rows_w[wv] += slo[j * W + wv + 1] - slo[j * W + wv];
+            rows_all += rows_w[wv];
+        }
+        for (const Range& r : reg) bytes_all += r.bytes, vcap += r.bytes / VB;
+        const int n_rec = (int)std::min<int64_t>(std::min<int64_t>(vcap, bytes_all / REC), rows_all);
+        std::vector<Range> vpieces, cpieces;
+        {
+            int left = n_rec;
+            for (const Range& r : reg) {
+                const int n = (int)std::min<int64_t>(left, r.bytes / VB);
+                if (n > 0) vpieces.push_back({r.base, (int64_t)n * VB});
+                if (r.bytes - (int64_t)n * VB > 0) cpieces.push_back({r.base + (int64_t)n * VB, r.bytes - (int64_t)n * VB});
+                left -= n;
+            }
+            std::stable_sort(cpieces.begin(), cpieces.end(), [](const Range& a, const Range& b) { return a.bytes > b.bytes; });
+        }
+        struct Deal {
+            const std::vector<Range>* pieces;
+            int64_t unit;
+            size_t at = 0;
+            int64_t used = 0;
+            int take(int want, int64_t& base) {
+                while (at < pieces->size() && used >= (*pieces)[at].bytes) ++at, used = 0;
+                if (at >= pieces->size() || want <= 0) return 0;
+                const int n = (int)std::min<int64_t>(want, ((*pieces)[at].bytes - used) / unit);
+                base = (*pieces)[at].base + used;
+                used += (int64_t)n * unit;
+                return n;
+            }
+        } dv{&vpieces, VB}, dc{&cpieces, CB};
+        int used = 0;
+        for (int wv = 0; wv < W; ++wv) {
+            const int share = (int)std::min<int64_t>(std::min<int64_t>(n_rec / W + (wv < n_rec % W ? 1 : 0), rows_w[wv]), 255);
+            int64_t va = 0, vb = 0, ca = 0, cb = 0;
+            int n_va = dv.take(share, va), n_vb = dv.take(share - n_va, vb);
+            int n_ca = dc.take(share, ca), n_cb = dc.take(share - n_ca, cb);
+            const int nres = std::min(n_va + n_vb, n_ca + n_cb);
+            n_va = std::min(n_va, nres), n_ca = std::min(n_ca, nres);
+            uint32_t* ww = wd + 4 + 3 * wv;
+            ww[0] = (uint32_t)nres | (uint32_t)n_va << 8 | (uint32_t)n_ca << 16;
+            ww[1] = (uint32_t)(va / 16) | (uint32_t)(vb / 16) << 16;
+            ww[2] = (uint32_t)(ca / 16) | (uint32_t)(cb / 16) << 16;
+            plan.rec_first[(size_t)g * W + wv + 1] = nres;
+            for (int k = 0; k < nres; ++k) {
+                plan.val_off.push_back((int32_t)(k < n_va ? va + (int64_t)k * VB : vb + (int64_t)(k - n_va) * VB));
+                plan.code_off.push_back((int32_t)(k < n_ca ? ca + (int64_t)k * CB : cb + (int64_t)(k - n_ca) * CB));
+            }
+            int k = 0;
+            for (int ph = 0; ph < 2 && k < nres; ++ph) {
+                const int J0 = ph ? R / 2 : 0, J1 = ph ? R : R / 2;
+                int mw = 0;
+                for (int j = J0; j < J1; ++j) mw = std::max(mw, slo[j * W + wv + 1] - slo[j * W + wv]);
+                for (int e = 0; e < mw && k < nres; ++e)
+                    for (int j = J0; j < J1 && k < nres; ++j)
+                        if (e < slo[j * W + wv + 1] - slo[j * W + wv]) ++plan.depth[(size_t)g * nsl + j * W + wv], ++k;
+            }
+            used += nres;
+        }
+        plan.resident_bytes += (int64_t)used * REC;
+        plan.min_records = g == 0 ? used : std::min(plan.min_records, used);
+        plan.max_records = std::max(plan.max_records, used);
+    }
+    for (size_t i = 0; i < (size_t)G * W; ++i) plan.rec_first[i + 1] += plan.rec_first[i];
+    return FDAPDE_OK;
 }
+
+}
diff --git a/fdapde-core_amd/csrc/internal.h b/fdapde-core_amd/csrc/internal.h
--- a/fdapde-core_amd/csrc/internal.h
+++ b/fdapde-core_amd/csrc/internal.h
@@ -170,6 +170,21 @@
 int host_build_persist_layout(const HostSpace& hs, bool use_bnd, int n_wg, int lds_entries, PersistLayout& pl, const int32_t* block_rows = nullptr,
                               int sym_mode = 0, bool balance = false, const int32_t* ghost_order = nullptr, bool allow_late = false);
 
+constexpr int kPersistResRecord = 1280;
+constexpr int kPersistResWords = 28;
+struct PersistResidentPlan {
+    int G = 0, R = 0;
+    size_t lds_bytes = 0;
+    int64_t resident_bytes = 0;
+    int32_t min_records = 0, max_records = 0;
+    std::vector<uint32_t> words;
+    std::vector<uint8_t> hole;
+    std::vector<int32_t> rec_first;
+    std::vector<int32_t> val_off, code_off;
+    std::vector<int32_t> depth;
+};
+int host_persist_resident_plan(const PersistLayout& pl, const uint8_t* hole, int imp_cap, size_t lds_used, size_t lds_budget, PersistResidentPlan& plan);
+
 inline double persist_bisect_span(int M, int N, int64_t n) {
     const double key_span = (double)((uint64_t(1) << (N == 3 ? 21 : 31)) - 1);
     double levels = std::floor(std::pow((double)(n > 1 ? n : 1), 1.0 / (double)(M >= 1 ? M : 1)) + 0.5) - 1.0;
diff --git a/fdapde-core_amd/csrc/kernels_persist.h b/fdapde-core_amd/csrc/kernels_persist.h
--- a/fdapde-core_amd/csrc/kernels_persist.h
+++ b/fdapde-core_amd/csrc/kernels_persist.h
@@ -53,6 +53,8 @@
     const int32_t* i2e;
     const double* scale;
     int32_t pf_steps;
+    const uint32_t* res_plan;
+    const int32_t* res_depth;
     double tol2;
     const int32_t* slot_dof;
     const int64_t* ell_off;
@@ -158,7 +160,7 @@
     asm volatile("s_mov_b32 %0, m0\n\ts_mov_b32 m0, %2\n\tglobal_load_lds_dword %1, off\n\ts_mov_b32 m0, %0" : "=&s"(m0_saved) : "v"(p), "s"(lds_dump) : "memory");
 }
 template <int RI, int W>
-__device__ __forceinline__ void touch_first_step(const int32_t* slo, const void* gv, const void* gc, int wave, int lane, unsigned lds_dump) {
+__device__ __forceinline__ void touch_first_step(const int32_t* slo, const int32_t* dep, const void* gv, const void* gc, int wave, int lane, unsigned lds_dump) {
     constexpr int per_wave = RI * 10, total = 2 * per_wave;
     if (wave < W / 2) return;
 #pragma unroll
@@ -168,10 +170,15 @@
         const int half = idx / per_wave, rem = idx - half * per_wave;
         const int j = rem / 10, k = rem - j * 10;
         const int tw = (wave - W / 2) + half * (W / 2);
-        const int o = slo[j * W + tw], wj = slo[j * W + tw + 1] - o;
+        const int d = dep != nullptr ? dep[j * W + tw] : 0;
+        const int o = slo[j * W + tw] + d, wj = slo[j * W + tw + 1] - o;
         const char* line = k < 8 ? static_cast<const char*>(gv) + (size_t)o * 1024 + k * 128 : static_cast<const char*>(gc) + (size_t)o * 256 + (k - 8) * 128;
         if (t * 64 + lane < total && wj > 0) touch_line(line, lds_dump);
     }
+}
+template <int RI, int W>
+__device__ __forceinline__ void touch_first_step(const int32_t* slo, const void* gv, const void* gc, int wave, int lane, unsigned lds_dump) {
+    touch_first_step<RI, W>(slo, nullptr, gv, gc, wave, lane, lds_dump);
 }
 template <int CTRL> __device__ __forceinline__ double persist_dpp_f64(double v) {
     const long long b = __double_as_longlong(v);
@@ -258,6 +265,35 @@
     const __amdgpu_buffer_rsrc_t rs_v = __builtin_amdgcn_make_buffer_rsrc(const_cast<double2*>(gv), 0, (int)min(e_left * 8, (int64_t)0x7fffffff), 0x00020000);
     const __amdgpu_buffer_rsrc_t rs_c = __builtin_amdgcn_make_buffer_rsrc(const_cast<uint32_t*>(gc), 0, (int)min(e_left * 2, (int64_t)0x7fffffff), 0x00020000);
     const int lane16 = lane * 16, lane4 = lane * 4;
+    constexpr bool RES = SYM && STREAM && !DIST && !WIDE;
+    unsigned hmask = 0;
+    int nres = 0;
+    unsigned res_n = 0, res_v = 0, res_c = 0;
+    const int wave_s = __builtin_amdgcn_readfirstlane(wave);
+    if constexpr (RES) {
+        if (a.res_plan != nullptr) {
+            const uint32_t* wd = a.res_plan + (size_t)g * kPersistResWords;
+#pragma unroll
+            for (int j = 0; j < R; ++j) hmask |= ((wd[(j * W) >> 5] >> (((j * W) & 31) + wave_s)) & 1u) << j;
+            hmask = __builtin_amdgcn_readfirstlane(hmask);
+            res_n = __builtin_amdgcn_readfirstlane(wd[4 + 3 * wave_s]), res_v = __builtin_amdgcn_readfirstlane(wd[5 + 3 * wave_s]);
+            res_c = __builtin_amdgcn_readfirstlane(wd[6 + 3 * wave_s]);
+            nres = (int)(res_n & 0xffu);
+        }
+    }
+    [[maybe_unused]] auto hole = [&](int j) -> bool {
+        if constexpr (RES) return ((hmask >> j) & 1u) != 0;
+        else return false;
+    };
+    [[maybe_unused]] auto res_val_at = [&](int k) -> int {
+        const int na = (int)((res_n >> 8) & 0xffu);
+        return (int)(k < na ? (res_v & 0xffffu) + 64u * (unsigned)k : (res_v >> 16) + 64u * (unsigned)(k - na)) * 16;
+    };
+    [[maybe_unused]] auto res_code_at = [&](int k) -> int {
+        const int na = (int)((res_n >> 16) & 0xffu);
+        return (int)(k < na ? (res_c & 0xffffu) + 16u * (unsigned)k : (res_c >> 16) + 16u * (unsigned)(k - na)) * 16;
+    };
+    char* const lds_c = reinterpret_cast<char*>(lds);
     const int32_t* impl = PLDS ? a.imp_pos + a.imp_off[g] : impl_l;
     const uint16_t* expl = PLDS ? a.exp_slot + a.exp_off[g] : expl_l;
     bool expl_in_lds = !PLDS;
@@ -274,7 +310,8 @@
         for (int i = tid; i < E; i += T) expl_l[i] = a.exp_slot[a.exp_off[g] + i];
     } else if constexpr (SYM) {
 #pragma unroll
-        for (int j = 0; j < R; ++j) y_tab[j * T + tid] = 0;
+        for (int j = 0; j < R; ++j)
+            if (!hole(j)) y_tab[j * T + tid] = 0;
     }
     int bexp = 0;
     if constexpr (SYM) {
@@ -292,6 +329,29 @@
     for (int j = 0; j < R; ++j) {
         o0[j] = __builtin_amdgcn_readfirstlane(slo[j * W + wave]);
         w[j] = __builtin_amdgcn_readfirstlane(slo[j * W + wave + 1]) - o0[j];
+    }
+    if constexpr (RES) {
+        if (nres > 0) {
+            int k = 0;
+            auto stage = [&](auto phase) {
+                constexpr int J0 = decltype(phase)::value ? RI : 0, J1 = decltype(phase)::value ? R : RI;
+                int mw = 0;
+#pragma unroll
+                for (int j = J0; j < J1; ++j) mw = max(mw, w[j]);
+                for (int e = 0; e < mw && k < nres; ++e) {
+#pragma unroll
+                    for (int j = J0; j < J1; ++j)
+                        if (e < w[j] && k < nres) {
+                            const int row = o0[j] + e;
+                            *reinterpret_cast<double2*>(lds_c + res_val_at(k) + lane16) = gv[row * 64 + lane];
+                            *reinterpret_cast<uint32_t*>(lds_c + res_code_at(k) + lane4) = gc[row * 64 + lane];
+                            ++k;
+                        }
+                }
+            };
+            stage(std::integral_constant<int, 0>{});
+            stage(std::integral_constant<int, 1>{});
+        }
     }
     double xv[WIDE ? 1 : R], rv[R], pv[PLDS ? 1 : R];
     int32_t dof[PLDS ? 1 : R];
@@ -310,8 +370,9 @@
         const double x0 = on && a.x != nullptr ? a.x[d] : 0.0;
         if constexpr (WIDE) xs[j * T] = x0;
         else xv[j] = x0;
-        if constexpr (PLDS) p_tab[j * T + tid] = rv[j];
-        else pv[j] = rv[j], dof[j] = d;
+        if constexpr (PLDS) {
+            if (!hole(j)) p_tab[j * T + tid] = rv[j];
+        } else pv[j] = rv[j], dof[j] = d;
         rr_part += rv[j] * rv[j];
     }
     double bb = (!DIST && a.direct) ? 0.0 : a.sc[0];
@@ -322,7 +383,7 @@
     __shared__ unsigned pf_dump[64];
     [[maybe_unused]] auto prefetch_next = [&]() {
         if constexpr (STREAM)
-            if (a.pf_steps != 0) touch_first_step<RI, W>(slo, gv, gc, wave, lane, (unsigned)(size_t)(__attribute__((address_space(3))) unsigned*)pf_dump);
+            if (a.pf_steps != 0) touch_first_step<RI, W>(slo, RES && a.res_plan != nullptr ? a.res_depth + (size_t)g * nsl : nullptr, gv, gc, wave, lane, (unsigned)(size_t)(__attribute__((address_space(3))) unsigned*)pf_dump);
     };
     __syncthreads();
     for (;;) {
@@ -342,7 +403,8 @@
         if constexpr (SYM) {
             double m = 0;
 #pragma unroll
-            for (int j = 0; j < R; ++j) m = fmax(m, fabs(P(j)));
+            for (int j = 0; j < R; ++j)
+                if (!hole(j)) m = fmax(m, fabs(P(j)));
             m = wave_max64(m);
             if (lane == 0) pmax_w[wave] = m;
         }
@@ -358,7 +420,7 @@
         double psj[PS_REG ? R : 1];
         if constexpr (PS_REG) {
 #pragma unroll
-            for (int j = 0; j < R; ++j) psj[j] = P(j) * tscale;
+            for (int j = 0; j < R; ++j) psj[j] = hole(j) ? 0.0 : P(j) * tscale;
         }
         [[maybe_unused]] long long c_exp = 0, c_first = 0;
         {
@@ -390,7 +452,8 @@
         }
         double yv[R];
 #pragma unroll
-        for (int j = 0; j < R; ++j) yv[j] = P(j);
+        for (int j = 0; j < R; ++j) yv[j] = hole(j) ? 0.0 : P(j);
+        [[maybe_unused]] int kres = 0;
         auto product = [&](auto phase) {
             constexpr int J0 = decltype(phase)::value ? RI : 0, J1 = decltype(phase)::value ? R : RI, NJ = J1 - J0;
             int mw = 0;
@@ -462,7 +525,16 @@
                     for (int j = jg; j < jg + GS; ++j) {
                         if (e < w[j]) {
                             const int row = o0[j] + e;
-                            if constexpr (STREAM) {
+                            if constexpr (RES) {
+                                if (kres < nres) {
+                                    v[j - jg] = *reinterpret_cast<const pg_u32x4*>(lds_c + res_val_at(kres) + lane16);
+                                    c[j - jg] = *reinterpret_cast<const uint32_t*>(lds_c + res_code_at(kres) + lane4);
+                                } else {
+                                    v[j - jg] = __builtin_amdgcn_raw_buffer_load_b128(rs_v, lane16, row * 1024, FDAPDE_SYM_NT_V);
+                                    c[j - jg] = __builtin_amdgcn_raw_buffer_load_b32(rs_c, lane4, row * 256, FDAPDE_SYM_NT_C);
+                                }
+                                ++kres;
+                            } else if constexpr (STREAM) {
                                 v[j - jg] = __builtin_amdgcn_raw_buffer_load_b128(rs_v, lane16, row * 1024, FDAPDE_SYM_NT_V);
                                 c[j - jg] = __builtin_amdgcn_raw_buffer_load_b32(rs_c, lane4, row * 256, FDAPDE_SYM_NT_C);
                             } else v[j - jg] = reinterpret_cast<const pg_u32x4*>(ev)[row * 64 + lane], c[j - jg] = ec[row * 64 + lane];
@@ -581,6 +653,7 @@
             __syncthreads();
 #pragma unroll
             for (int j = 0; j < R; ++j) {
+                if (hole(j)) continue;
                 yv[j] += (double)y_tab[j * T + tid] * tinv;
                 y_tab[j * T + tid] = 0;
             }
@@ -588,7 +661,8 @@
         if (stamper) c1 = wall_clock64();
         double s0 = 0, s1 = 0;
 #pragma unroll
-        for (int j = 0; j < R; ++j) s0 += P(j) * yv[j], s1 += yv[j] * yv[j];
+        for (int j = 0; j < R; ++j)
+            if (!hole(j)) s0 += P(j) * yv[j], s1 += yv[j] * yv[j];
         s0 = wave_sum64(s0), s1 = wave_sum64(s1);
         const double s2 = wave_sum64(rr_part);
         if (lane == 0) red[wave][0] = s0, red[wave][1] = s1, red[wave][2] = s2;
@@ -794,6 +868,7 @@
         } else {
 #pragma unroll
         for (int j = 0; j < R; ++j) {
+            if (hole(j)) continue;
             const double pj = P(j);
             xv[j] += alpha * pj;
             rv[j] -= alpha * yv[j];
@@ -853,6 +928,13 @@
         st[0] = (double)n_stamped, st[1] = (double)t_spmv, st[2] = (double)t_gather, st[3] = (double)t_update;
     }
     if (status == 3 && tid == 0 && !(!DIST && a.direct)) atomicExch(a.ctl + 3, 1);
+}
+
+static __global__ void k_persist_hole_slices(const int32_t* slot_dof, int64_t n_slices, uint8_t* hole) {
+    const int64_t q = (int64_t)blockIdx.x * (blockDim.x / 64) + (threadIdx.x >> 6);
+    if (q >= n_slices) return;
+    const bool any = __any(slot_dof[q * 64 + (threadIdx.x & 63)] >= 0) != 0;
+    if ((threadIdx.x & 63) == 0) hole[q] = any ? 0 : 1;
 }
 
 struct BlockedSpmvArgs {
diff --git a/fdapde-core_amd/csrc/persist_engine.hip b/fdapde-core_amd/csrc/persist_engine.hip
--- a/fdapde-core_amd/csrc/persist_engine.hip
+++ b/fdapde-core_amd/csrc/persist_engine.hip
@@ -81,6 +81,45 @@
     for (int g = 0; g < pl.G && host_built; ++g) n.need = std::max<int64_t>(n.need, pl.ell_off[(size_t)g + 1] - pl.ell_off[(size_t)g]);
     n.need += 128;
     return n;
+}
+
+static size_t persist_lds_used(const fdapde_ctx* c, const PersistLayout& pl, const PersistNeeds& pn, bool stream, bool* exp_lds) {
+    const bool e = pl.sym && stream && pl.R <= kPersistRmax && pn.fixed + 2 * (size_t)pn.exp_cap + 1024 <= 160 * 1024 && c->persist_exp_lds;
+    if (exp_lds) *exp_lds = e;
+    return pn.fixed + (e ? 2 * (size_t)pn.exp_cap : 0);
+}
+static int persist_plan_resident(fdapde_ctx* c, const PersistLayout& pl, const DevPersist* dp, const PersistNeeds& pn, size_t lds_used, size_t lds_budget, bool check,
+                                 PersistResidentPlan& plan) {
+    if (dp == nullptr) {
+        if (host_persist_resident_plan(pl, nullptr, pn.imp_cap, lds_used, lds_budget, plan) != FDAPDE_OK) return fail(c, FDAPDE_EHIP, "residency plan of the single launch failed");
+        return FDAPDE_OK;
+    }
+    const size_t nq = (size_t)pl.G * pl.nsl;
+    DBuf<uint8_t> dh;
+    HIPCHK(c, dh.alloc(nq));
+    hipLaunchKernelGGL(k_persist_hole_slices, dim3((unsigned)((nq + 3) / 4)), dim3(256), 0, c->stream, dp->slot_dof, (int64_t)nq, dh.p);
+    HIPCHK(c, hipGetLastError());
+    std::vector<uint8_t> hole(nq);
+    PersistLayout t;
+    t.sym = pl.sym, t.G = pl.G, t.R = pl.R, t.nsl = pl.nsl;
+    t.sl_off.resize((size_t)pl.G * (pl.nsl + 1));
+    HIPCHK(c, hipMemcpyAsync(hole.data(), dh.p, nq, hipMemcpyDeviceToHost, c->stream));
+    HIPCHK(c, hipMemcpyAsync(t.sl_off.data(), dp->sl_off, sizeof(int32_t) * t.sl_off.size(), hipMemcpyDeviceToHost, c->stream));
+    HIPCHK(c, hipStreamSynchronize(c->stream));
+    if (check) {
+        std::vector<int32_t> sd(nq * 64);
+        HIPCHK(c, hipMemcpy(sd.data(), dp->slot_dof, sizeof(int32_t) * sd.size(), hipMemcpyDeviceToHost));
+        size_t bad = 0;
+        for (size_t q = 0; q < nq; ++q) {
+            bool any = false;
+            for (int l = 0; l < 64; ++l) any = any || sd[q * 64 + l] >= 0;
+            bad += (hole[q] != 0) == any;
+        }
+        std::fprintf(stderr, "persist check %-9s: %s (%zu elements)\n", "holes", bad ? "MISMATCH" : "ok", nq);
+        if (bad) return fail(c, FDAPDE_EHIP, "FDAPDE_SETUP_CHECK: the empty slices found on the device differ from the layout's slot_dof (see stderr)");
+    }
+    if (host_persist_resident_plan(t, hole.data(), pn.imp_cap, lds_used, lds_budget, plan) != FDAPDE_OK) return fail(c, FDAPDE_EHIP, "residency plan of the single launch failed");
+    return FDAPDE_OK;
 }
 
 int build_persist_once(fdapde_ctx* c, int v, const std::vector<int32_t>* block_rows, bool balance) {
@@ -220,16 +259,25 @@
         if (rc2 == FDAPDE_OK) {
             pn2 = persist_needs(pl2, !on_device);
             stream2 = pn2.fixed + 10 * (size_t)pn2.need > lds_total;
-            auto bytes = [](const PersistLayout& l) {
-                return 10.0 * (double)l.n_entries + 32.0 * (double)l.n_board + (l.R > kPersistRmax ? 16.0 * (double)l.n_int : 0.0);
+            auto bytes = [&](const PersistLayout& l, const DevPersist& d, const PersistNeeds& n, bool streams) {
+                double b = 10.0 * (double)l.n_entries + 32.0 * (double)l.n_board + (l.R > kPersistRmax ? 16.0 * (double)l.n_int : 0.0);
+                if (c->persist_resident && l.sym && streams && l.R <= kPersistRmax) {
+                    PersistResidentPlan rp;
+                    if (persist_plan_resident(c, l, on_device ? &d : nullptr, n, persist_lds_used(c, l, n, streams, nullptr), lds_total, false, rp) == FDAPDE_OK)
+                        b -= (double)rp.resident_bytes;
+                    else
+                        (void)hipGetLastError(), c->err.clear();
+                }
+                return b;
             };
+            const double bytes2 = bytes(pl2, dp2, pn2, stream2), bytes1 = bytes(pl, dp, persist_needs(pl, !on_device), ps.stream);
             const bool fits = 10.0 * (double)pl2.n_entries <= max_mb * 1e6 && pn2.fixed <= lds_total && !(pl2.R >= 16 && !stream2) &&
                               !(pl2.R > kPersistRmax && (c->persist_plain || !c->persist_wide));
             const bool same_form = pl2.sym == pl.sym && pl2.R <= pl.R && (!stream2 || ps.stream);
-            take = fits && same_form && (part == 1 || bytes(pl2) < bytes(pl));
+            take = fits && same_form && (part == 1 || bytes2 < bytes1);
             if (std::getenv("FDAPDE_DEBUG_SETUP"))
                 std::fprintf(stderr, "persistent CG layout %d: bisection %s: %.0f bytes per iteration against %.0f (entries %lld / %lld, board %lld / %lld, imports <= %d / %d, R %d / %d)\n",
-                             v, take ? "taken" : "not taken", bytes(pl2), bytes(pl), (long long)pl2.n_entries, (long long)pl.n_entries, (long long)pl2.n_board,
+                             v, take ? "taken" : "not taken", bytes2, bytes1, (long long)pl2.n_entries, (long long)pl.n_entries, (long long)pl2.n_board,
                              (long long)pl.n_board, pl2.max_imp, pl.max_imp, pl2.R, pl.R);
         }
         if (take) {
@@ -246,6 +294,24 @@
     ps.exp_lds = pl.sym && ps.stream && pl.R <= kPersistRmax && ps.lds_bytes + 2 * (size_t)exp_cap + 1024 <= 160 * 1024 && c->persist_exp_lds;
     if (ps.exp_lds) ps.lds_bytes += 2 * (size_t)exp_cap;
     hipStream_t st = c->stream;
+    ps.res_lds_bytes = 0, ps.res_bytes = 0, ps.res_min = ps.res_max = 0;
+    ps.res_plan.release(), ps.res_depth.release();
+    if (c->persist_resident && pl.sym && ps.stream && pl.R <= kPersistRmax) {
+        PersistResidentPlan rp;
+        PersistNeeds pn;
+        pn.S = S, pn.imp_cap = imp_cap, pn.exp_cap = exp_cap, pn.fixed = fixed, pn.need = need;
+        if (int rc = persist_plan_resident(c, pl, on_device ? &dp : nullptr, pn, ps.lds_bytes, lds_total, check, rp)) {
+            dev_persist_release(&dp);
+            return rc;
+        }
+        if (rp.resident_bytes > 0) {
+            HIPCHK(c, ps.res_plan.upload(rp.words.data(), rp.words.size(), st));
+            HIPCHK(c, ps.res_depth.upload(rp.depth.data(), rp.depth.size(), st));
+            HIPCHK(c, hipStreamSynchronize(st));
+            ps.res_lds_bytes = rp.lds_bytes, ps.res_bytes = rp.resident_bytes, ps.res_min = rp.min_records, ps.res_max = rp.max_records;
+        }
+        clk.mark("build_persist: residency plan");
+    }
     if (on_device) {
         const size_t GS = (size_t)pl.G * S, n_alloc = (size_t)pl.n_entries + 256;
         adopt(ps.slot_dof, dp.slot_dof, GS), adopt(ps.ell_off, dp.ell_off, (size_t)pl.G + 1), adopt(ps.sl_off, dp.sl_off, (size_t)pl.G * (pl.nsl + 1));
@@ -282,7 +348,7 @@
                      "LDS %zu B (%s%s, largest block %lld), imports <= %d, exports <= %d, board %lld\n", v, on_device ? "device" : "host", pl.G, pl.R,
                      (long long)pl.n_int, (long long)pl.n_entries, (long long)pl.nnz,
                      100.0 * (double)(pl.n_entries - pl.nnz) / (double)(pl.n_entries > 0 ? pl.n_entries : 1), ps.lds_bytes,
-                     ps.stream ? "blocks stream" : "blocks resident", pl.sym ? (pl.bisect ? ", symmetric storage, bisection blocks" : ", symmetric storage") : (pl.bisect ? ", bisection blocks" : ""), (long long)need, pl.max_imp, pl.max_exp, (long long)pl.n_board);
+                     ps.stream ? (ps.res_lds_bytes ? "blocks stream behind a resident head" : "blocks stream") : "blocks resident", pl.sym ? (pl.bisect ? ", symmetric storage, bisection blocks" : ", symmetric storage") : (pl.bisect ? ", bisection blocks" : ""), (long long)need, pl.max_imp, pl.max_exp, (long long)pl.n_board);
     pl.slot_dof = {}, pl.ell_code = {}, pl.ell_src = {}, pl.exp_slot = {}, pl.imp_pos = {}, pl.sl_off = {}, pl.ell_off = {};
     ps.meta = std::move(pl);
     ps.filled = false, ps.ok = true;
@@ -313,20 +379,33 @@
 #define PERSIST_GO_D(R_, ST_, SY_, DI_)                                                                                         \
     do {                                                                                                                        \
         const void* fn = reinterpret_cast<const void*>(&k_cg_persist<R_, ST_, SY_, DI_>);                                       \
+         \
+        const bool res_form = SY_ && ST_ && !DI_;                                                                               \
         if (ps.attr_set != fn) {                                                                                                \
             DebugClock clk2;                                                                                                    \
-            HIPCHK(c, hipFuncSetAttribute(fn, hipFuncAttributeMaxDynamicSharedMemorySize, (int)ps.lds_bytes));                  \
-            clk2.mark("launch_persist: hipFuncSetAttribute");                                                                   \
-            int per_cu = 0;                                                                                                     \
-            HIPCHK(c, hipOccupancyMaxActiveBlocksPerMultiprocessor(&per_cu, fn, kPersistT, ps.lds_bytes));                      \
+            int per_cu = 0, per_cu_base = 0;                                                                                    \
+            if (res_form && ps.res_lds_bytes != 0) {                                                                            \
+                HIPCHK(c, hipFuncSetAttribute(fn, hipFuncAttributeMaxDynamicSharedMemorySize, (int)ps.res_lds_bytes));          \
+                HIPCHK(c, hipOccupancyMaxActiveBlocksPerMultiprocessor(&per_cu, fn, kPersistT, ps.res_lds_bytes));              \
+                HIPCHK(c, hipOccupancyMaxActiveBlocksPerMultiprocessor(&per_cu_base, fn, kPersistT, ps.lds_bytes));             \
+                if ((int64_t)per_cu * c->n_cu < (int64_t)a.G) ps.res_lds_bytes = 0, per_cu = per_cu_base;                       \
+            } else {                                                                                                            \
+                HIPCHK(c, hipFuncSetAttribute(fn, hipFuncAttributeMaxDynamicSharedMemorySize, (int)ps.lds_bytes));              \
+                clk2.mark("launch_persist: hipFuncSetAttribute");                                                               \
+                HIPCHK(c, hipOccupancyMaxActiveBlocksPerMultiprocessor(&per_cu, fn, kPersistT, ps.lds_bytes));                  \
+                per_cu_base = per_cu;                                                                                           \
+            }                                                                                                                   \
             clk2.mark("launch_persist: occupancy query");                                                                       \
             if ((int64_t)per_cu * c->n_cu < (int64_t)a.G) return FDAPDE_EUNSUPPORTED;    \
-            ps.attr_set = fn, ps.per_cu = per_cu;                                                                               \
+            ps.attr_set = fn, ps.per_cu = per_cu, ps.per_cu_base = per_cu_base;                                                 \
         }                                                                                                                       \
         const unsigned ncol = a.n_cols > 1 ? (unsigned)a.n_cols : 1u;                                                           \
-        if ((int64_t)ps.per_cu * c->n_cu < (int64_t)a.G * ncol) return FDAPDE_EUNSUPPORTED;                                     \
-        if (c->persist_coop) HIPCHK(c, hipLaunchCooperativeKernel(fn, dim3(a.G, ncol), dim3(kPersistT), kargs, (unsigned)ps.lds_bytes, st)); \
-        else hipLaunchKernelGGL((k_cg_persist<R_, ST_, SY_, DI_>), dim3(a.G, ncol), dim3(kPersistT), ps.lds_bytes, st, a);      \
+        const bool res_go = res_form && ps.res_lds_bytes != 0 && (int64_t)ps.per_cu * c->n_cu >= (int64_t)a.G * ncol;           \
+        if ((int64_t)(res_go ? ps.per_cu : ps.per_cu_base) * c->n_cu < (int64_t)a.G * ncol) return FDAPDE_EUNSUPPORTED;         \
+        const size_t lds_go = res_go ? ps.res_lds_bytes : ps.lds_bytes;                                                         \
+        a.res_plan = res_go ? ps.res_plan.p : nullptr, a.res_depth = res_go ? ps.res_depth.p : nullptr;                         \
+        if (c->persist_coop) HIPCHK(c, hipLaunchCooperativeKernel(fn, dim3(a.G, ncol), dim3(kPersistT), kargs, (unsigned)lds_go, st)); \
+        else hipLaunchKernelGGL((k_cg_persist<R_, ST_, SY_, DI_>), dim3(a.G, ncol), dim3(kPersistT), lds_go, st, a);            \
     } while (0)
 #define PERSIST_GO2(R_, ST_)                                                                                                    \
     do {                                                                                                                        \
diff --git a/include/fdapde_hip.h b/include/fdapde_hip.h
--- a/include/fdapde_hip.h
+++ b/include/fdapde_hip.h
@@ -126,6 +126,7 @@
 int fdapde_solver_layout_kind(fdapde_ctx *ctx, int32_t with_dirichlet, int32_t *kind, int32_t *symmetric_storage,
                               int32_t *workgroups, int32_t *rows_per_thread);
 int fdapde_solver_layout_partition(fdapde_ctx *ctx, int32_t with_dirichlet, int32_t *partition);
+int fdapde_solver_layout_resident(fdapde_ctx *ctx, int32_t with_dirichlet, double *resident_bytes, int32_t *min_records, int32_t *max_records);
 typedef int (*fdapde_allreduce_fn)(void *user, double *host_buf, int64_t count);
 int fdapde_comm_init_callback(fdapde_ctx *ctx, int32_t world, int32_t rank, fdapde_allreduce_fn fn, void *user);
 int fdapde_comm_unique_id(void *out128);
```

Measured after the change: 112.4 million. 4.2% lower.
